# jcasal-homer/HomerHEVC

Hardware: AMD Instinct MI355X
Metric: encoded frames/sec, 1080p & 2160p YUV420 fixed-QP IPPP, 1/2/4/8 MI355X (higher is better)
Workload: dtype int16; 1 GPU; cfg2-1080p-encode; sequences_per_gpu=256, width=1920, height=1080, wfpp_num_threads=17, qp=32, gop=IPPP intra_period=100

## Files before the change

homerhevc_amd/csrc/enc/enc_platform.h:

```cpp
#pragma once
#include <stdint.h>
#include <string.h>
#include <math.h>

#if defined(__HIPCC__)
#include <hip/hip_runtime.h>
#define HENC_HD __device__
#if defined(HENC_PRIM_NOINLINE)
#define HENC_PRIM __device__ __attribute__((noinline))
#else
#define HENC_PRIM __device__
#endif
#define HENC_INLINE __host__ __device__ __forceinline__
#define HENC_TU_TABLES_IN_LDS 0
#define HENC_FT(e) ((const FastTables *)nullptr)
#else
#define HENC_HD
#define HENC_PRIM
#define HENC_INLINE inline
#define HENC_TU_TABLES_IN_LDS 1
#define HENC_FT(e) ((e).ft)
#endif

#if defined(__HIPCC__) && !defined(HENC_WALK_OUTLINE)
#define HENC_WALK_FN __attribute__((always_inline))
#else
#define HENC_WALK_FN
#endif

namespace henc {

#if defined(__HIPCC__)
struct WaveGrp {
	int tid;
	static constexpr int n = 64;
	static constexpr bool bg = false;
#if defined(HENC_NO_RDFULL)
	static constexpr bool rdfull = false;
#else
	static constexpr bool rdfull = true;
#endif
	__device__ __forceinline__ void sync() const
	{
		__builtin_amdgcn_fence(__ATOMIC_RELEASE, "wavefront");
		__builtin_amdgcn_wave_barrier();
		__builtin_amdgcn_fence(__ATOMIC_ACQUIRE, "wavefront");
	}
	__device__ __forceinline__ uint32_t sum(uint32_t v) const
	{
		int x = (int)v;
		x += __builtin_amdgcn_update_dpp(0, x, 0x111, 0xf, 0xf, true);
		x += __builtin_amdgcn_update_dpp(0, x, 0x112, 0xf, 0xf, true);
		x += __builtin_amdgcn_update_dpp(0, x, 0x114, 0xf, 0xf, true);
		x += __builtin_amdgcn_update_dpp(0, x, 0x118, 0xf, 0xf, true);
		return (uint32_t)(__builtin_amdgcn_readlane(x, 15) + __builtin_amdgcn_readlane(x, 31) + __builtin_amdgcn_readlane(x, 47) + __builtin_amdgcn_readlane(x, 63));
	}
	__device__ __forceinline__ int64_t sum64(int64_t v) const
	{
#pragma unroll
		for (int m = 32; m >= 1; m >>= 1) v += __shfl_xor(v, m, 64);
		return v;
	}
	__device__ __forceinline__ uint32_t any(bool p) const { return __ballot(p) != 0; }
	__device__ __forceinline__ uint64_t ballot(bool p) const { return __ballot(p); }
	__device__ __forceinline__ uint64_t min64(uint64_t v) const
	{
#pragma unroll
		for (int m = 32; m >= 1; m >>= 1) {
			const uint64_t o = __shfl_xor(v, m, 64);
			v = o < v ? o : v;
		}
		return v;
	}
};
struct WaveGrpLat : WaveGrp {
	static constexpr bool bg = true;
};
struct WaveGrpLean : WaveGrp {
	static constexpr bool rdfull = false;
};

template <class P>
struct PairGrpOf {
	int tid, half;
	static constexpr int n = 32;
	static constexpr bool bg = false;
	static constexpr bool rdfull = P::rdfull;
	__device__ __forceinline__ void sync() const
	{
		__builtin_amdgcn_fence(__ATOMIC_RELEASE, "wavefront");
		__builtin_amdgcn_wave_barrier();
		__builtin_amdgcn_fence(__ATOMIC_ACQUIRE, "wavefront");
	}
	__device__ __forceinline__ uint32_t sum(uint32_t v) const
	{
		int x = (int)v;
		x += __builtin_amdgcn_update_dpp(0, x, 0x111, 0xf, 0xf, true);
		x += __builtin_amdgcn_update_dpp(0, x, 0x112, 0xf, 0xf, true);
		x += __builtin_amdgcn_update_dpp(0, x, 0x114, 0xf, 0xf, true);
		x += __builtin_amdgcn_update_dpp(0, x, 0x118, 0xf, 0xf, true);
		const int lo = __builtin_amdgcn_readlane(x, 15) + __builtin_amdgcn_readlane(x, 31), hi = __builtin_amdgcn_readlane(x, 47) + __builtin_amdgcn_readlane(x, 63);
		return (uint32_t)(half ? hi : lo);
	}
	__device__ __forceinline__ uint64_t ballot(bool p) const { const uint64_t m = __ballot(p); return half ? m >> 32 : m & 0xffffffffull; }
	__device__ __forceinline__ uint32_t any(bool p) const { return ballot(p) != 0; }
};
using PairGrp = PairGrpOf<WaveGrp>;

#endif

template <class T>
HENC_INLINE T uni(T x)
{
#if defined(__HIP_DEVICE_COMPILE__)
	static_assert(sizeof(T) <= 4, "one scalar register");
	return (T)__builtin_amdgcn_readfirstlane((int)x);
#else
	return x;
#endif
}
template <class T>
HENC_INLINE T *uni_ptr(T *p)
{
#if defined(__HIP_DEVICE_COMPILE__)
	const uintptr_t v = (uintptr_t)p;
	const uint32_t lo = (uint32_t)__builtin_amdgcn_readfirstlane((int)(uint32_t)v), hi = (uint32_t)__builtin_amdgcn_readfirstlane((int)(uint32_t)(v >> 32));
	return (T *)(((uintptr_t)hi << 32) | (uintptr_t)lo);
#else
	return p;
#endif
}
template <class T>
HENC_INLINE T *in_fast_memory(T *p)
{
#if defined(__HIP_DEVICE_COMPILE__) && defined(HENC_CHECK_ADDRSPACE)
	if (p && !__builtin_amdgcn_is_shared((const void *)p)) __builtin_trap();
	return p;
#elif defined(__HIP_DEVICE_COMPILE__)
	__builtin_assume(__builtin_amdgcn_is_shared((const void *)p));
	return p;
#else
	return p;
#endif
}
#if defined(__HIP_DEVICE_COMPILE__) && defined(HENC_CHECK_ADDRSPACE)
#define HENC_ENC_IN_LDS(e) do { if (!__builtin_amdgcn_is_shared((const void *)&(e))) __builtin_trap(); } while (0)
#elif defined(__HIP_DEVICE_COMPILE__)
#define HENC_ENC_IN_LDS(e) __builtin_assume(__builtin_amdgcn_is_shared((const void *)&(e)))
#else
#define HENC_ENC_IN_LDS(e) do { } while (0)
#endif
#if defined(__HIP_DEVICE_COMPILE__) && defined(HENC_TU_OPERANDS_IN_LDS) && defined(HENC_CHECK_ADDRSPACE)
#define HENC_OP_IN_LDS(p) do { if (!__builtin_amdgcn_is_shared((const void *)(p))) __builtin_trap(); } while (0)
#elif defined(__HIP_DEVICE_COMPILE__) && defined(HENC_TU_OPERANDS_IN_LDS)
#define HENC_OP_IN_LDS(p) __builtin_assume(__builtin_amdgcn_is_shared((const void *)(p)))
#else
#define HENC_OP_IN_LDS(p) do { } while (0)
#endif
#if defined(__HIP_DEVICE_COMPILE__)
#define HENC_GLOBAL_PTR(T) __attribute__((address_space(1))) T *
#else
#define HENC_GLOBAL_PTR(T) T *
#endif
template <class T>
struct FastPtr {
	T *p;
	HENC_INLINE T *get() const { return in_fast_memory(p); }
	HENC_INLINE T *operator->() const { return get(); }
	HENC_INLINE T &operator*() const { return *get(); }
	HENC_INLINE T &operator[](int i) const { return get()[i]; }
	HENC_INLINE operator T *() const { return get(); }
	HENC_INLINE explicit operator bool() const { return p != nullptr; }
	HENC_INLINE FastPtr &operator=(T *q) { p = q; return *this; }
};

#if defined(__HIP_DEVICE_COMPILE__)
extern __shared__ __align__(16) unsigned char henc_lds_base[];
template <class T, int OFFSET>
struct LdsAt {
	HENC_INLINE T *get() const { return (T *)(henc_lds_base + OFFSET); }
	HENC_INLINE T *operator->() const { return get(); }
	HENC_INLINE T &operator*() const { return *get(); }
	HENC_INLINE T &operator[](int i) const { return get()[i]; }
	HENC_INLINE operator T *() const { return get(); }
	HENC_INLINE explicit operator bool() const { return true; }
	HENC_INLINE LdsAt &operator=(T *) { return *this; }
	HENC_INLINE LdsAt &operator=(decltype(nullptr)) { return *this; }
};
#endif

struct CpuGrp {
	static constexpr int tid = 0;
	static constexpr int n = 1;
	static constexpr bool bg = false;
	static constexpr bool rdfull = true;
	void sync() const {}
	uint32_t sum(uint32_t v) const { return v; }
	int64_t sum64(int64_t v) const { return v; }
	uint32_t any(bool p) const { return p; }
	uint64_t ballot(bool p) const { return p ? 1 : 0; }
	uint64_t min64(uint64_t v) const { return v; }
};

template <class T> HENC_INLINE T hmin(T a, T b) { return a < b ? a : b; }
template <class T> HENC_INLINE T hmax(T a, T b) { return a > b ? a : b; }
template <class T> HENC_INLINE T hclip(T v, T lo, T hi) { return v < lo ? lo : (v > hi ? hi : v); }
HENC_INLINE int habs(int v) { return v < 0 ? -v : v; }
HENC_INLINE double hsqrt(double v) { return ::sqrt(v); }
HENC_INLINE int16_t sat16(int v) { return (int16_t)hclip(v, -32768, 32767); }

}
```

homerhevc_amd/csrc/enc/enc_sched.h:

```cpp
#pragma once
#include "enc_ctu.h"

#if !defined(__HIPCC__) && defined(HENC_SCHED_CAUSES)
extern "C" int henc_sched_causes[8];
#define SCHED_CAUSE(k) (henc_sched_causes[k]++)
#else
#define SCHED_CAUSE(k) ((void)0)
#endif

namespace henc {

constexpr int MODE_STATE_BYTES = 2 * NDEPTH * NPART;

HENC_INLINE void sched_chain_step(uint8_t st[2][NDEPTH], const uint8_t *out_tokens, int k)
{
	uint8_t nx[2][NDEPTH];
	for (int comp = 0; comp < 2; comp++)
		for (int d = 0; d < NDEPTH; d++) {
			const uint8_t v = out_tokens[(comp * NDEPTH + d) * NPART + k];
			nx[comp][d] = (v & MODE_TOKEN) ? st[comp][v & 7] : v;
		}
	for (int comp = 0; comp < 2; comp++)
		for (int d = 0; d < NDEPTH; d++) st[comp][d] = nx[comp][d];
}

HENC_INLINE int sched_replay_search(const SearchLog &lg, const uint8_t *true_in, double sqrt_lambda, int *mode_g, int *bits_g, int *mode_t, int *bits_t)
{
	int td[2], pg[3], pt[3];
	double cg = 0, ct = 0;
	for (int k = 0; k < 2; k++) td[k] = (lg.src[k] & 0x8000) ? true_in[((lg.src[k] >> 8) & 7) * NPART + (lg.src[k] & 255)] : lg.used[k];
	mpm_from_dirs(lg.used[0], lg.used[1], pg);
	mpm_from_dirs(td[0], td[1], pt);
	auto table = [&](int mode) -> int64_t {
		for (int k = 0; k < lg.n; k++)
			if (lg.mode[k] == mode) return (int64_t)lg.sad[k];
		return -1;
	};
	*bits_g = intra_search_walk(pg, 1, sqrt_lambda, table, mode_g, &cg);
	*bits_t = intra_search_walk(pt, 1, sqrt_lambda, table, mode_t, &ct);
	return *bits_t >= 0;
}

template <class G>
HENC_HD int sched_guesses_hold(const G g, const CtuInfo &c, const FrameCtx &f, const uint8_t *true_in, const uint8_t *used_in, uint32_t intra_before,
			       uint32_t parts_before, uint32_t used_intra, uint32_t used_parts, int uses_ratio)
{
	int bad = 0;
	if (c.walk_intra != ctu_takes_intra_walk(f, c.ctu_number)) return 0;
	if (c.walk_intra) uses_ratio = 0;
	if (c.n_spec_reads > MAX_SEARCH_LOGS || c.n_ratio_cmp > MAX_RATIO_CMP) {
		for (int i = g.tid; i < NDEPTH * NPART; i += g.n) bad |= true_in[i] != used_in[i];
		if (uses_ratio) bad |= intra_ratio(intra_before, parts_before) != intra_ratio(used_intra, used_parts);
		return !g.any(bad);
	}
	for (int i = g.tid; i < c.n_spec_reads; i += g.n) {
		const SearchLog &lg = c.slog[i];
		if (lg.has_cmp) continue;
		int mg, bg, mt, bt;
		bad |= !sched_replay_search(lg, true_in, f.sqrt_lambda, &mg, &bg, &mt, &bt) || mg != mt || bg != bt;
	}
	if (uses_ratio) {
		const double ratio = intra_ratio(intra_before, parts_before), used_ratio = intra_ratio(used_intra, used_parts);
		const double correction = calc_mv_correction((uint32_t)f.qp, f.avg_dist);
		for (int i = g.tid; i < c.n_ratio_cmp; i += g.n) {
			const double *lg = c.ratio_cmp + 4 * i;
			double intra_dist = lg[0];
			int same_bits = 1;
			if (c.ratio_slog[i] >= 0) {
				const SearchLog &sl = c.slog[c.ratio_slog[i]];
				int mg, bg, mt, bt;
				if (!sched_replay_search(sl, true_in, f.sqrt_lambda, &mg, &bg, &mt, &bt) || mg != mt) { bad = 1; SCHED_CAUSE(bt < 0 ? 0 : 1); continue; }
				same_bits = bg == bt;
				intra_dist = (double)((uint32_t)lg[0] - intra_luma_cost(sl.tu_cost, bg, correction) + intra_luma_cost(sl.tu_cost, bt, correction));
			}
			const double ic = intra_cost_with_ratio(intra_dist, ratio, lg[1], lg[2]), ic_used = intra_cost_with_ratio(lg[0], used_ratio, lg[1], lg[2]);
			const int take = ic < lg[3];
			if (take != (c.ratio_out[i] != 0)) SCHED_CAUSE(c.ratio_slog[i] >= 0 && !same_bits ? 2 : 3);
			else if (take && (!same_bits || (uint32_t)ic != (uint32_t)ic_used)) SCHED_CAUSE(4);
			bad |= take != (c.ratio_out[i] != 0) || (take && (!same_bits || (uint32_t)ic != (uint32_t)ic_used));
		}
	}
	return !g.any(bad);
}

template <class G>
HENC_HD uint64_t sched_output_hash(const G g, const Seq &S, const FrameCtx &f, const CtuInfo &c)
{
	uint32_t h1 = 0, h2 = 0;
	const uint32_t *p = (const uint32_t *)(const CtuPublic *)&c;
	const int words = (int)(offsetof(CtuPublic, sao_recon) / 4);
	for (int i = g.tid; i < words; i += g.n) {
		h1 += p[i] * (2654435761u + 2u * (uint32_t)i);
		h2 += (p[i] ^ 0x9e3779b9u) * (40503u + 2u * (uint32_t)i + 1u);
	}
	for (int comp = 0; comp < 3; comp++) {
		const int sz = comp ? 32 : 64, px = comp ? c.x >> 1 : c.x, py = comp ? c.y >> 1 : c.y;
		const int pw = comp ? S.width >> 1 : S.width, ph = comp ? S.height >> 1 : S.height, rs = comp ? S.stride_c : S.stride_y;
		const int ww = (px + sz) < pw ? sz : pw - px, hh = (py + sz) < ph ? sz : ph - py;
		const int16_t *r = f.rec[comp] + py * rs + px;
		for (int i = g.tid; i < ww * hh; i += g.n) {
			const uint32_t v = (uint16_t)r[(i / ww) * rs + (i % ww)];
			h1 += v * (2246822519u + 2u * (uint32_t)(i + comp * 4096));
			h2 += (v + 0x632be5abu) * (3266489917u + 2u * (uint32_t)(i + comp * 4096));
		}
	}
	h1 = g.sum(h1);
	h2 = g.sum(h2);
	return ((uint64_t)h1 << 32) | h2;
}

HENC_INLINE void sched_known_intra(const uint32_t *prefix, int W, int row, int col, uint32_t *intra, uint32_t *parts)
{
	uint32_t ti = prefix[(size_t)row * (W + 1) + col], tp = (uint32_t)col;
	for (int k = 1; k <= row; k++) {
		const int have = col + 2 * k < W ? col + 2 * k : W;
		ti += prefix[(size_t)(row - k) * (W + 1) + have];
		tp += (uint32_t)have;
	}
	*intra = ti;
	*parts = tp * NPART;
}

}
```

homerhevc_amd/csrc/k_encode.hip:

```cpp
#define HENC_TU_OPERANDS_IN_LDS 1
#include <stddef.h>
#include <stdlib.h>
#include <algorithm>
#include <chrono>
#include <mutex>
#include <condition_variable>
#include <new>
#include <string>
#include <thread>
#include <vector>

#include <type_traits>
#include "common.h"
#include "enc/enc_sched.h"
#include "enc/enc_host.h"
#include "enc/enc_post.h"
#include "picture_io.h"

using namespace henc;

int hmr_subpel_plane_on(hipStream_t stream, int comp, const int16_t *pic, int stride, int rows, uint8_t *out);
int hmr_subpel_planes_on(hipStream_t stream, const int16_t *pic_y, const int16_t *pic_u, const int16_t *pic_v, int stride_y, int rows_y, int stride_c, int rows_c, uint8_t *out_y,
			 uint8_t *out_u, uint8_t *out_v);

struct EncDev {
	const Seq *seq;
	const FrameCtx *frame;
	const DevTables *tables;
	const Geo *geo;
	CtuInfo *ctus, *ctus_start;
	WorkSlow *work_slow;
	int16_t *coeff;
	int *progress;
	uint32_t *prefix;
	unsigned long long *prof;
	uint8_t *guess, *truth, *outtok;
	uint8_t *chain_start, *chain_end;
	int *valid, *dirty;
	unsigned long long *hash;
	uint32_t *intra_before, *used_intra, *used_parts;
	uint8_t *rowstate;
	int *thread_seen;
	int *row0_checked;
	int *counters;
	int threads;
	int dep, dep_full;
	int after, raster;
	FrameCtx *next_frame;
	double *fin;
	RcFrame *rc_dyn;
	const int *rd_src;
	const uint8_t *rd_init, *rd_ring;
	PostPic post;
};

__device__ __forceinline__ void wave_copy_words(void *dst, const void *src, int bytes, int tid)
{
	uint32_t *d = (uint32_t *)dst;
	const uint32_t *s = (const uint32_t *)src;
	for (int i = tid; i < bytes / 4; i += 64) d[i] = s[i];
}
__device__ __forceinline__ void wave_copy_quads(void *dst, const void *src, int bytes, int tid)
{
	uint4 *d = (uint4 *)dst;
	const uint4 *s = (const uint4 *)src;
#pragma unroll 4
	for (int i = tid; i < bytes / 16; i += 64) d[i] = s[i];
}
constexpr int PRED_STATE_BYTES = (64 * 64 + 2 * 32 * 32) * (int)sizeof(pred_t), ROW_STATE_BYTES = MODE_STATE_BYTES + PRED_STATE_BYTES;
static_assert(offsetof(Work, pred_c) == offsetof(Work, pred_y) + 64 * 64 * sizeof(pred_t) && sizeof(((Work *)nullptr)->pred_c) == 2 * 32 * 32 * sizeof(pred_t), "the prediction windows are one block of Work");
static_assert(MODE_STATE_BYTES % 16 == 0 && offsetof(Work, pred_y) % 16 == 0, "wave_copy_quads alignment");

constexpr size_t LDS_WORK = (sizeof(Work) + 15) & ~(size_t)15, LDS_NODES = (sizeof(Node) * NODE_SLOTS + 15) & ~(size_t)15,
		 LDS_GEO = NHELP * HSCRATCH_ELEMS * 2;
namespace henc { __constant__ Geo henc_geo_table[NNODES]; }
constexpr bool LDS_KEEPS_CTU_RECORD = false, LDS_KEEPS_TU_TABLES = false;
static_assert(LDS_KEEPS_TU_TABLES == (HENC_TU_TABLES_IN_LDS != 0), "enc_platform.h: HENC_FT");
constexpr size_t LDS_SEQ = (sizeof(Seq) + sizeof(FrameCtx) + 31) & ~(size_t)15, LDS_CTU = LDS_KEEPS_CTU_RECORD ? (sizeof(CtuPublic) + 15) & ~(size_t)15 : 0,
		 LDS_FT = LDS_KEEPS_TU_TABLES ? (sizeof(FastTables) + 15) & ~(size_t)15 : 0;
#if defined(HENC_PROFILE)
constexpr size_t LDS_BOX = LDS_BOX_BYTES + (1 + NHELP) * LDS_ENC_BYTES, LDS_HSCRATCH = 0, LDS_RD = (sizeof(WorkRd) + 15) & ~(size_t)15;
constexpr size_t LDS_BYTES = HENC_LDS_PROF_OFFSET + 2 * PP_COUNT * 8;
constexpr size_t LDS_FT_OFFSET = LDS_WORK + LDS_NODES + LDS_GEO + LDS_SEQ + LDS_CTU + LDS_BOX + LDS_HSCRATCH;
static_assert(LDS_WORK + LDS_NODES + LDS_GEO + LDS_SEQ + LDS_CTU + LDS_BOX + LDS_HSCRATCH + LDS_FT + LDS_RD <= HENC_LDS_PROF_OFFSET, "profile table overlaps the worker state");
#else
constexpr size_t LDS_BOX = LDS_BOX_BYTES + (1 + NHELP) * LDS_ENC_BYTES, LDS_HSCRATCH = 0, LDS_RD = (sizeof(WorkRd) + 15) & ~(size_t)15;
constexpr size_t LDS_BYTES = LDS_WORK + LDS_NODES + LDS_GEO + LDS_SEQ + LDS_CTU + LDS_BOX + LDS_HSCRATCH + LDS_FT + LDS_RD;
constexpr size_t LDS_FT_OFFSET = LDS_WORK + LDS_NODES + LDS_GEO + LDS_SEQ + LDS_CTU + LDS_BOX + LDS_HSCRATCH;
#endif
static_assert(sizeof(SubpelScratch) <= LDS_WORK + LDS_NODES + LDS_GEO, "task S works where the post stage does");
static_assert(sizeof(PostScratch) <= LDS_WORK + LDS_NODES + LDS_GEO, "the post stage works in what is idle between two CTUs: the worker's Work area, the CTU's partition nodes, the helpers' scratch");
#if !defined(HENC_PROFILE)
static_assert(LDS_OFF_RD == (int)(LDS_BYTES - LDS_RD), "the RD_FULL arrays are the tail of a worker's LDS");
#endif
static_assert(LDS_OFF_ENC == (int)(LDS_WORK + LDS_NODES + LDS_GEO + LDS_SEQ + LDS_CTU + LDS_BOX_BYTES) || LDS_FT != 0 || LDS_CTU != 0, "the RD_FULL arrays are the tail of a worker's LDS: launches without RD_FULL pictures leave them out");
static_assert(LDS_OFF_NODES == (int)LDS_WORK && LDS_OFF_SEQ == (int)(LDS_WORK + LDS_NODES + LDS_GEO) && LDS_OFF_BOX == (int)(LDS_WORK + LDS_NODES + LDS_GEO + LDS_SEQ + LDS_CTU),
	      "enc_common.h: the fixed places of Enc's LDS members");
#if !defined(HENC_WAVES_PER_EU)
#define HENC_WAVES_PER_EU 2
#endif
constexpr int ENC_THREADS = 64 * (1 + NHELP);
static_assert(LDS_BYTES <= 160 * 1024, "a workgroup has 160 KiB of LDS on gfx950");
constexpr int workers_per_cu(size_t lds_bytes)
{
	const int by_lds = (int)((160 * 1024) / ((lds_bytes + 1279) / 1280 * 1280)), by_waves = 4 * HENC_WAVES_PER_EU / (1 + NHELP);
	return by_lds < by_waves ? by_lds : by_waves;
}
constexpr int WORKERS_PER_CU = workers_per_cu(LDS_BYTES - LDS_RD);
#if !defined(HENC_PROFILE) && HENC_WAVES_PER_EU == 2 && HENC_NHELP == 1
static_assert(WORKERS_PER_CU == 4, "a worker's LDS (without the RD_FULL arrays) has to stay within a quarter of the CU's: 32 granules of 1280 bytes");
#endif
#if defined(HENC_PRINT_LDS)
static_assert(LDS_BYTES - LDS_RD == 0 && LDS_WORK == 0 && LDS_NODES == 0 && LDS_BOX == 0 && sizeof(PostScratch) == 0 && WORKERS_PER_CU == 0, "sizes");
#endif

template <class G>
__device__ __forceinline__ bool helper_serve(HelperBox *box, int h, int16_t *scratch, const G g, int seq)
{
	extern __shared__ __align__(16) uint8_t lds[];
	Enc &e = *(Enc *)(lds + LDS_OFF_ENC + (1 + h) * LDS_ENC_BYTES);
	HENC_ENC_IN_LDS(e);
	const Enc &worker = *(const Enc *)(lds + LDS_OFF_ENC);
	{
		const int job = box->job[h];
		if (job == HJOB_QUIT) return false;
		if (job == HJOB_NEW_CTU) {
			wave_copy_words(&e, &worker, (int)sizeof(Enc), g.tid);
			g.sync();
			e.box = nullptr;
			e.on_helper = 1 + h;
			e.scratch_a = scratch;
			e.scratch_b = scratch + 1024;
			e.adi_c = scratch + 2048;
			e.prof = nullptr;
		}
		const int *a = box->a[h];
		uint32_t r0 = 0, r1 = 0, r2 = 0, r3 = 0, r4 = 0, r5 = 0;
		switch (job) {
		case HJOB_INTER_TU: {
			int sum = 0;
			uint32_t raw = 0;
			if (NHELP == 1 && a[1] == COMP_UV && e.geo[a[0]].size_chroma <= 8) {
				const PairGrpOf<G> pg{g.tid & 31, g.tid >> 5};
				const uint32_t d = encode_inter_tu(pg, e, a[0], COMP_U + pg.half, a[2], a[3], &sum, &raw, pg.half * 512);
				r0 = (uint32_t)__builtin_amdgcn_readlane((int)d, 0); r1 = (uint32_t)__builtin_amdgcn_readlane(sum, 0); r2 = (uint32_t)__builtin_amdgcn_readlane((int)raw, 0);
				r3 = (uint32_t)__builtin_amdgcn_readlane((int)d, 32); r4 = (uint32_t)__builtin_amdgcn_readlane(sum, 32); r5 = (uint32_t)__builtin_amdgcn_readlane((int)raw, 32);
				break;
			}
			r0 = encode_inter_tu(g, e, a[0], a[1] == COMP_UV ? COMP_U : a[1], a[2], a[3], &sum, &raw);
			r1 = (uint32_t)sum;
			r2 = raw;
			if (a[1] == COMP_UV) {
				r3 = encode_inter_tu(g, e, a[0], COMP_V, a[2], a[3], &sum, &raw);
				r4 = (uint32_t)sum;
				r5 = raw;
			}
			break;
		}
		case HJOB_SYNC_CU:
			if (a[1] == COMP_UV) sync_cu_chroma_both(g, e, a[0], a[2], a[3], a[4], a[5]);
			else sync_cu_comp(g, e, a[0], a[2], a[3], a[4], a[5], a[1]);
			break;
		case HJOB_SSD: {
			const Geo &q = e.geo[a[0]];
			if (a[1] == COMP_UV) {
				const int n = q.size_chroma, l = ilog2i(n);
				uint32_t acc[2] = {0, 0};
				for (int i = g.tid * 4; i < n * n; i += 64 * 4) {
					const int o = q.yc * 32 + q.xc + (i >> l) * 32 + (i & (n - 1));
#pragma unroll
					for (int c = 0; c < 2; c++) {
						const S4 va = ld4(e.w->curr_c[c] + o), vb = ld4(e.w->pred_c[c] + o);
#pragma unroll
						for (int k = 0; k < 4; k++) { const int32_t dd = (int16_t)(va.v[k] - vb.v[k]); acc[c] += (uint32_t)(dd * dd); }
					}
				}
				r0 = g.sum(acc[0]);
				r1 = g.sum(acc[1]);
			} else {
				const int c = a[1] - 1;
				r0 = blk_ssd(g, e.w->curr_c[c] + q.yc * 32 + q.xc, 32, e.w->pred_c[c] + q.yc * 32 + q.xc, 32, q.size_chroma);
			}
			break;
		}
		case HJOB_CHROMA_SEARCH: {
			const int cand[5] = {a[2] & 255, (a[2] >> 8) & 255, (a[2] >> 16) & 255, (a[2] >> 24) & 255, a[3]};
			uint32_t sads[5];
			chroma_search_comp(g, e, a[0], a[1], cand, sads);
			g.sync();
			if (g.tid == 0)
				for (int k = 0; k < 5; k++) box->r[h][k] = sads[k];
			break;
		}
		case HJOB_CHROMA_TU: {
			int cs = 0;
			r0 = (uint32_t)chroma_tu_comp(g, e, a[0], a[1], a[2], a[3], a[4], a[5] & 255, a[5] >> 8, &cs);
			r1 = (uint32_t)cs;
			break;
		}
#if defined(HENC_QUAD)
// ... 89 lines not shown
	HelperBox *box = (HelperBox *)(lds + LDS_WORK + LDS_NODES + LDS_GEO + LDS_SEQ + LDS_CTU);
	const int wave = (int)(threadIdx.x >> 6);
	for (int i = (int)threadIdx.x; i < (int)(lds_bytes / 4); i += ENC_THREADS) ((uint32_t *)lds)[i] = 0;
	__syncthreads();
	if (wave > 0) {
		helper_loop<LAT, G>(box, wave - 1, (int16_t *)(lds + LDS_WORK + LDS_NODES) + (wave - 1) * HSCRATCH_ELEMS);
		return false;
	}
	return true;
}
__device__ __forceinline__ void release_helpers(int *hseq)
{
	extern __shared__ __align__(16) uint8_t lds[];
	HelperBox *box = (HelperBox *)(lds + LDS_WORK + LDS_NODES + LDS_GEO + LDS_SEQ + LDS_CTU);
	if ((threadIdx.x & 63) == 0)
		for (int h = 0; h < NHELP; h++) {
			box->job[h] = HJOB_QUIT;
			__hip_atomic_store(&box->cmd[h], ++hseq[h], __ATOMIC_RELEASE, __HIP_MEMORY_SCOPE_WORKGROUP);
		}
}
__device__ __forceinline__ void encode_row(const EncDev &d, int pass, int row, int *hseq)
{
	extern __shared__ __align__(16) uint8_t lds[];
	const Seq &S = *d.seq;
	const int W = S.wctu, H = S.hctu;
	WaveGrp g{(int)(threadIdx.x & 63)};
	Work *lw = (Work *)lds;
	HelperBox *box = (HelperBox *)(lds + LDS_WORK + LDS_NODES + LDS_GEO + LDS_SEQ + LDS_CTU);
	for (int i = g.tid; i < (int)(LDS_WORK / 4); i += 64) ((uint32_t *)lds)[i] = 0;
	g.sync();
	Seq *lseq = (Seq *)(lds + LDS_WORK + LDS_NODES + LDS_GEO);
	FrameCtx *lframe = (FrameCtx *)((uint8_t *)lseq + ((sizeof(Seq) + 15) & ~(size_t)15));
	for (int i = g.tid; i < (int)(sizeof(Seq) / 4); i += 64) ((uint32_t *)lseq)[i] = ((const uint32_t *)d.seq)[i];
	for (int i = g.tid; i < (int)(sizeof(FrameCtx) / 4); i += 64) ((uint32_t *)lframe)[i] = ((const uint32_t *)d.frame)[i];
	if (g.tid == 0) lw->slow = (HENC_GLOBAL_PTR(WorkSlow))(d.work_slow + row);
	g.sync();
	if (g.tid == 0) lframe->scene_cut_ctu = d.counters[2];
	FastTables *lft = LDS_KEEPS_TU_TABLES ? (FastTables *)(lds + LDS_FT_OFFSET) : nullptr;
	if (lft) fast_tables_fill(g, *lft, d.tables, lframe->qp % 6, chroma_qp_table(lframe->qp + S.chroma_qp_offset) % 6);
#if defined(HENC_PROFILE)
	if (g.tid < 2 * PP_COUNT) ((unsigned long long *)(lds + HENC_LDS_PROF_OFFSET))[g.tid] = 0;
#endif
	g.sync();
	Enc &e = *(Enc *)(lds + LDS_OFF_ENC);
	HENC_ENC_IN_LDS(e);
	e.seq = lseq;
	e.f = lframe;
	e.T = d.tables;
	e.ft = lft;
	e.geo.p = nullptr;
	e.ctus = d.ctus;
	e.ctu = nullptr;
	e.w = lw;
	e.nodes = nullptr;
	e.nodes_fast = (Node *)(lds + LDS_WORK);
	e.node_quad = -1;
	e.on_helper = 0;
	e.ctu_g = nullptr;
	e.ctu_fast = LDS_KEEPS_CTU_RECORD ? (CtuPublic *)(lds + LDS_WORK + LDS_NODES + LDS_GEO + LDS_SEQ) : nullptr;
	e.box = box;
	for (int h = 0; h < NHELP; h++) e.hseq[h] = hseq[h];
	e.bgseq = 0;
	e.bg_node = -1;
	e.prof = d.prof ? d.prof + (size_t)row * PF_COUNT : nullptr;
	e.timeline = nullptr;
	uint32_t *my_prefix = d.prefix + (size_t)row * (W + 1);
	if (pass <= 0 && g.tid == 0) my_prefix[0] = 0;
	int encodes = 0;
	if (g.tid == 0) lw->thread_seen_intra = 1;
	g.sync();
	for (int c = 0; c < W; c++) {
		if (row > 0) {
			HENC_PROF_T0();
			const int need = c + 2 < W ? c + 2 : W;
			while (__hip_atomic_load(&d.progress[row - 1], __ATOMIC_RELAXED, __HIP_MEMORY_SCOPE_AGENT) < need) __builtin_amdgcn_s_sleep(32);
			__builtin_amdgcn_fence(__ATOMIC_ACQUIRE, "agent");
			HENC_PROF_ADD(e, PF_WAIT);
		}
		const int n = row * W + c;
		const int redo = pass == 0 || !__hip_atomic_load(&d.valid[n], __ATOMIC_RELAXED, __HIP_MEMORY_SCOPE_AGENT) ||
				 __hip_atomic_load(&d.dirty[n], __ATOMIC_RELAXED, __HIP_MEMORY_SCOPE_AGENT);
		if (redo) {
			HENC_PROF_T0();
			uint8_t *gs = d.guess + (size_t)n * MODE_STATE_BYTES;
			uint32_t ui, up;
			if (pass > 0) {
				wave_copy_words(&d.ctus[n], &d.ctus_start[n], (int)offsetof(CtuInfo, n_spec_reads), g.tid);
				wave_copy_words(d.ctus[n].nodes, d.ctus_start[n].nodes, (int)sizeof(d.ctus[n].nodes), g.tid);
				wave_copy_words(gs, d.truth + (size_t)n * MODE_STATE_BYTES, MODE_STATE_BYTES, g.tid);
				ui = d.intra_before[n];
				up = (uint32_t)n * NPART;
			} else {
				if (n == 0) wave_copy_words(gs, d.chain_start, MODE_STATE_BYTES, g.tid);
				sched_known_intra(d.prefix, W, row, c, &ui, &up);
			}
			g.sync();
			if (g.tid == 0) e.w->mode_in = (const uint8_t (*)[NDEPTH][NPART])gs;
			if (g.tid == 0) { d.used_intra[n] = ui; d.used_parts[n] = up; }
			const unsigned long long old_hash = d.hash[n];
			e.total_intra_partitions = ui;
			e.total_partitions = up;
			e.coeff = d.coeff + (size_t)n * 6144;
			e.ctu_qp = lframe->qp;
			g.sync();
			encode_ctu(g, e, n);
			encodes++;
			wave_copy_words(d.outtok + (size_t)n * MODE_STATE_BYTES, e.w->intra_mode_buffs, MODE_STATE_BYTES, g.tid);
			const unsigned long long h = sched_output_hash(g, S, *lframe, d.ctus[n]);
			if (g.tid == 0) { d.hash[n] = h; d.dirty[n] = 0; }
			if (pass == 0) {
				const int snap = row + 1 < H && c == (W > 1 ? 1 : 0);
				if (c + 1 < W || snap) {
					const uint8_t *tok = &e.w->intra_mode_buffs[0][0][0];
					uint8_t *nx = gs + MODE_STATE_BYTES, *rs = d.guess + (size_t)(row + 1) * W * MODE_STATE_BYTES;
					for (int i = g.tid; i < MODE_STATE_BYTES; i += 64) {
						const uint8_t v = tok[i];
						const uint8_t r = (v & MODE_TOKEN) ? gs[(i / (NDEPTH * NPART)) * NDEPTH * NPART + (v & 7) * NPART + i % NPART] : v;
						if (c + 1 < W) nx[i] = r;
						if (snap) rs[i] = r;
					}
				}
				if (g.tid == 0) my_prefix[c + 1] = my_prefix[c] + d.ctus[n].intra_parts;
			} else if (h != old_hash && g.tid == 0) {
				if (c + 1 < W) d.dirty[n + 1] = 1;
				if (row + 1 < H) {
					if (c > 0) d.dirty[n + W - 1] = 1;
					d.dirty[n + W] = 1;
					if (c + 1 < W) d.dirty[n + W + 1] = 1;
				}
			}
			HENC_PROF_ADD(e, PF_TOTAL);
		}
		g.sync();
		if (g.tid == 0) __hip_atomic_store(&d.progress[row], c + 1, __ATOMIC_RELEASE, __HIP_MEMORY_SCOPE_AGENT);
	}
	for (int h = 0; h < NHELP; h++) hseq[h] = e.hseq[h];
	if (g.tid == 0 && encodes) atomicAdd(&d.counters[1], encodes);
#if defined(HENC_PROFILE)
	if (g.tid == 0 && e.prof) {
		const unsigned long long *pp = (const unsigned long long *)(lds + HENC_LDS_PROF_OFFSET);
		for (int k = 0; k < 2 * PP_COUNT; k++) e.prof[PF_PRIM0 + k] += pp[k];
	}
#endif
}

struct PoolSeq {
	int *cur_step;
	int *ticket;
	int *done;
};
constexpr int POOL_MAX_STEPS = HENC_MAX_STEPS;
constexpr int POOL_STRIDE = 1 + 2 * POOL_MAX_STEPS;
constexpr int BATCH_MAX = 512;

__device__ __forceinline__ void pool_step_rows(int t, int W, int H, int *r_lo, int *r_hi)
{
	const int lo = t - W + 1;
	*r_lo = lo <= 0 ? 0 : (lo + 1) >> 1;
	*r_hi = (t >> 1) < H - 1 ? (t >> 1) : H - 1;
}

template <class G>
__device__ void pool_encode_ctu(const EncDev &d, Enc &__restrict__ e, const G g, Seq *lseq, FrameCtx *lframe, FastTables *lft, int t, int row, int *cached_rem, const int *abort_flag)
{
	HENC_ENC_IN_LDS(e);
	const Seq &S = *lseq;
	const int W = S.wctu, H = S.hctu;
	const int raster = d.raster;
	const int T = d.threads, me = row % T, c = raster ? t - row * W : t - 2 * row, n = row * W + c;
	uint32_t ti = 0, tc = 0;
	for (int r2 = g.tid; r2 < H; r2 += 64) {
		const int have = raster ? (r2 < row ? W : (r2 == row ? c : 0)) : (t - 2 * r2 < 0 ? 0 : (t - 2 * r2 < W ? t - 2 * r2 : W));
		ti += d.prefix[(size_t)r2 * (W + 1) + have];
		tc += (uint32_t)have;
	}
	ti = g.sum(ti);
	tc = g.sum(tc);
	wave_copy_words(&e.w->intra_mode_buffs[0][0][0], d.rowstate + (size_t)me * ROW_STATE_BYTES, MODE_STATE_BYTES, g.tid);
	wave_copy_quads(e.w->pred_y, d.rowstate + (size_t)me * ROW_STATE_BYTES + MODE_STATE_BYTES, PRED_STATE_BYTES, g.tid);
	if (g.tid == 0) e.w->thread_seen_intra = d.thread_seen[me];
	if (rd_full(g, S)) {
		const int seen = d.thread_seen[me];
		for (int i = g.tid; i < NPART; i += 64) e.wrd->rd_pred_mode[i] = seen ? PM_INTRA : PM_INTER;
	}
	const int rem_y = lframe->qp % 6, rem_c = chroma_qp_table(lframe->qp + S.chroma_qp_offset) % 6;
	if (lft && (cached_rem[0] != rem_y || cached_rem[1] != rem_c)) {
		fast_tables_fill(g, *lft, d.tables, rem_y, rem_c);
		cached_rem[0] = rem_y; cached_rem[1] = rem_c;
	}
	g.sync();
	const int hrow = raster ? row : t / (2 * T) * T;
	uint32_t rc_bits = 0;
	int rc_ctus = 0;
	if (rd_full(g, S)) {
		const int code = d.rd_src[n], kind = code >> 28, slot = (code >> 24) & 15;
		const size_t off = (size_t)(code & 0x00ffffff) * RD_CTX_BYTES;
		e.rd_ctx = kind == 3 ? d.rd_ring + ((size_t)slot * S.nctu) * RD_CTX_BYTES + off : d.rd_init + (size_t)(kind ? 1 + slot : 0) * RD_CTX_BYTES;
	}
	if (lframe->rc.on) rc_consumed(g, d.post, W, H, t, &rc_bits, &rc_ctus);
	if (row == hrow) {
		if (g.tid == 0) {
			if (d.counters[2] < 0 && lframe->slice_type == SLICE_P && scene_cut_fires(S, *lframe, ti, tc * NPART)) {
				if (lframe->rc.on) {
					RcFrame nrc = lframe->rc;
					rc_change_pic_mode(nrc, S.reinit_gop, S.intra_period, S.nctu, nrc.sqrt_clipped_intra_period, rc_bits, rc_ctus);
					*d.rc_dyn = nrc;
				}
				d.counters[2] = n;
			}
			__hip_atomic_store(d.row0_checked, t + 1, __ATOMIC_RELEASE, __HIP_MEMORY_SCOPE_AGENT);
		}
	} else if (hrow < H && t - 2 * hrow < W) {
		while (__hip_atomic_load(d.row0_checked, __ATOMIC_RELAXED, __HIP_MEMORY_SCOPE_AGENT) < t + 1 && !__hip_atomic_load(abort_flag, __ATOMIC_RELAXED, __HIP_MEMORY_SCOPE_AGENT)) __builtin_amdgcn_s_sleep(8);
		__builtin_amdgcn_fence(__ATOMIC_ACQUIRE, "agent");
	}
	g.sync();
	if (g.tid == 0) lframe->scene_cut_ctu = __hip_atomic_load(&d.counters[2], __ATOMIC_RELAXED, __HIP_MEMORY_SCOPE_AGENT);
	g.sync();
	e.ctu_qp = lframe->qp;
	if (lframe->rc.on) {
		const int cut = lframe->scene_cut_ctu;
		const int is_sc = cut >= 0 && (raster ? n >= cut : t >= cut % W + 2 * (cut / W));
		if (is_sc) {
			wave_copy_words(&lframe->rc, d.rc_dyn, (int)sizeof(RcFrame), g.tid);
			g.sync();
		}
		e.ctu_qp = rc_calc_cu_qp(lframe->rc, (double)rc_bits, rc_ctus, lframe->slice_type, is_sc, S.reinit_gop, S.intra_period, lframe->avg_dist, lframe->num_encoded_frames);
	}
	if (g.tid == 0) e.w->mode_in = (const uint8_t (*)[NDEPTH][NPART])(d.rowstate + (size_t)me * ROW_STATE_BYTES);
	e.total_intra_partitions = ti;
	e.total_partitions = tc * NPART;
	e.coeff = d.coeff + (size_t)n * 6144;
	g.sync();
#if defined(HENC_PROFILE)
	e.prof = d.prof ? d.prof + (size_t)row * PF_COUNT : nullptr;
	{
		HENC_PROF_T0();
		encode_ctu(g, e, n);
		HENC_PROF_ADD(e, PF_TOTAL);
	}
	if (g.tid == 0 && e.prof) {
		unsigned long long *pp = (unsigned long long *)(henc_lds + HENC_LDS_PROF_OFFSET);
		for (int k = 0; k < 2 * PP_COUNT; k++) { e.prof[PF_PRIM0 + k] += pp[k]; pp[k] = 0; }
	}
#else
	encode_ctu(g, e, n);
#endif
	resolve_mode_tokens(g, *e.w, d.ctus[n]);
	wave_copy_words(d.outtok + (size_t)n * MODE_STATE_BYTES, e.w->intra_mode_buffs, MODE_STATE_BYTES, g.tid);
	wave_copy_words(d.rowstate + (size_t)me * ROW_STATE_BYTES, &e.w->intra_mode_buffs[0][0][0], MODE_STATE_BYTES, g.tid);
	wave_copy_quads(d.rowstate + (size_t)me * ROW_STATE_BYTES + MODE_STATE_BYTES, e.w->pred_y, PRED_STATE_BYTES, g.tid);
	if (g.tid == 0) {
		d.thread_seen[me] = e.w->thread_seen_intra;
		uint32_t *my_prefix = d.prefix + (size_t)row * (W + 1);
		my_prefix[c + 1] = my_prefix[c] + d.ctus[n].intra_parts;
		atomicAdd(&d.counters[1], 1);
	}
	g.sync();
	__builtin_amdgcn_fence(__ATOMIC_RELEASE, "agent");
	if (g.tid == 0) post_st_fenced(&d.post.rows[row].dec, c + 1);
}

__device__ __attribute__((noinline)) int pool_post_drain_run(const EncDev &d, const WaveGrp g, const Seq *lseq, const FrameCtx *lframe, Work *lw, WorkSlow *my_slow, int *finished);
__device__ __forceinline__ int pool_post_drain(const EncDev &d, const WaveGrp g, const Seq *lseq, const FrameCtx *lframe, Work *lw, WorkSlow *my_slow, int *finished)
{
	if (post_finished(*lseq, d.post)) return 0;
	PostCtx x;
	x.seq = lseq; x.f = lframe; x.T = d.tables; x.geo.p = nullptr; x.ctus = d.ctus; x.coeff = d.coeff; x.pic = &d.post;
	int r, c, k;
	if (!post_scan(g, x, r, c, k)) return 0;
	return pool_post_drain_run(d, g, lseq, lframe, lw, my_slow, finished);
}
__device__ __attribute__((noinline)) int pool_post_drain_run(const EncDev &d, const WaveGrp g, const Seq *lseq, const FrameCtx *lframe, Work *lw, WorkSlow *my_slow, int *finished)
{
	PostCtx x;
	x.seq = lseq; x.f = lframe; x.T = d.tables; x.geo.p = nullptr; x.ctus = d.ctus; x.coeff = d.coeff; x.pic = &d.post;
	PostScratch &sc = *(PostScratch *)in_fast_memory((uint8_t *)lw);
	const int ran = post_drain(g, x, sc);
	if (ran) {
		if (g.tid == 0) lw->slow = (HENC_GLOBAL_PTR(WorkSlow))my_slow;
		g.sync();
		if (post_finished(*lseq, d.post)) {
			int won = 0;
			if (g.tid == 0) won = atomicCAS(&d.post.errors[1], 0, 2) == 0;
			if (__builtin_amdgcn_readfirstlane(won)) {
				__builtin_amdgcn_fence(__ATOMIC_ACQUIRE, "agent");
				const int W = lseq->wctu, H = lseq->hctu, T = d.threads < 1 ? 1 : d.threads;
				int64_t part = 0;
				for (int t = g.tid; t < T && t < H; t += 64) {
					uint32_t acc = 0;
					for (int r = t; r < H; r += T)
						for (int c = 0; c < W; c++) acc += d.ctus[r * W + c].distortion;
					part += acc;
				}
				const double total = (double)g.sum64(part);
				if (g.tid == 0) {
					d.fin[0] = total;
					if (d.next_frame) {
						double a = total;
						a /= lseq->nctu * NPART;
						a = a < .1 ? .1 : a;
						if (lframe->slice_type == SLICE_I) a *= 1.5;
						else if (__hip_atomic_load(&d.counters[2], __ATOMIC_RELAXED, __HIP_MEMORY_SCOPE_AGENT) >= 0) a *= 1.375;
						d.next_frame->avg_dist = a;
					}
					__builtin_amdgcn_fence(__ATOMIC_RELEASE, "agent");
					post_st_release(&d.post.errors[1], 1);
					atomicAdd(finished, 1);
				}
			}
		}
	}
	return ran;
}

template <class G>
__device__ __forceinline__ void encode_pool_body(const EncDev *devs, int nseq, int *state, int *finished, WorkSlow *slow, unsigned long long watchdog_ticks, unsigned lds_bytes)
{
	unsigned long long t_start = wall_clock64();
	constexpr bool LAT = G::bg;
	if (!rows_enter<LAT, typename std::conditional<LAT, WaveGrp, G>::type>(lds_bytes)) return;
	extern __shared__ __align__(16) uint8_t lds[];
	G g{(int)(threadIdx.x & 63)};
	Work *lw = (Work *)lds;
	HelperBox *box = (HelperBox *)(lds + LDS_WORK + LDS_NODES + LDS_GEO + LDS_SEQ + LDS_CTU);
	Seq *lseq = (Seq *)(lds + LDS_WORK + LDS_NODES + LDS_GEO);
	FrameCtx *lframe = (FrameCtx *)((uint8_t *)lseq + ((sizeof(Seq) + 15) & ~(size_t)15));
	FastTables *lft = LDS_KEEPS_TU_TABLES ? (FastTables *)(lds + LDS_FT_OFFSET) : nullptr;
	if (g.tid == 0) lw->slow = (HENC_GLOBAL_PTR(WorkSlow))(slow + blockIdx.x);
#if defined(HENC_PROFILE)
	if (g.tid < 2 * PP_COUNT) ((unsigned long long *)(lds + HENC_LDS_PROF_OFFSET))[g.tid] = 0;
#endif
	g.sync();
	Enc &e = *(Enc *)(lds + LDS_OFF_ENC);
	HENC_ENC_IN_LDS(e);
	e.seq = lseq;
	e.f = lframe;
	e.ft = lft;
	e.geo.p = nullptr;
	e.ctu = nullptr;
	e.w = lw;
	e.nodes = nullptr;
	e.nodes_fast = (Node *)(lds + LDS_WORK);
	e.node_quad = -1;
	e.on_helper = 0;
	e.ctu_g = nullptr;
	e.ctu_fast = LDS_KEEPS_CTU_RECORD ? (CtuPublic *)(lds + LDS_WORK + LDS_NODES + LDS_GEO + LDS_SEQ) : nullptr;
	e.box = box;
	for (int h = 0; h < NHELP; h++) e.hseq[h] = 0;
	e.bgseq = 0;
	e.bg_node = -1;
	e.prof = nullptr;
	e.timeline = nullptr;
	int cached_rem[2] = {-1, -1}, cached_q = -1, idle_rounds = 0;
	int start = (int)(blockIdx.x % (unsigned)nseq);
	for (;;) {
		int q = -1, t = 0, k = 0;
		bool all_finished = true;
		for (int base = 0; base < nseq && q < 0; base += 64) {
			const int i = base + g.tid, cand = i < nseq ? (start + i) % nseq : -1;
			int ct = -1;
			bool open = false;
			if (cand >= 0) {
				const int *st = state + (size_t)cand * POOL_STRIDE;
				const EncDev &dd = devs[cand];
				const int W = dd.seq->wctu, H = dd.seq->hctu, steps = dd.raster ? W * H : W + 2 * (H - 1);
				ct = __hip_atomic_load(&st[0], __ATOMIC_RELAXED, __HIP_MEMORY_SCOPE_AGENT);
				if (ct < steps) {
					all_finished = false;
					if (dd.raster) open = __hip_atomic_load(&st[1], __ATOMIC_RELAXED, __HIP_MEMORY_SCOPE_AGENT) == ct;
					else {
						int r_lo, r_hi;
						pool_step_rows(ct, W, H, &r_lo, &r_hi);
						open = __hip_atomic_load(&st[1 + ct], __ATOMIC_RELAXED, __HIP_MEMORY_SCOPE_AGENT) < r_hi - r_lo + 1;
					}
				}
			}
			if (g.any(!all_finished)) all_finished = false;
			uint64_t m = g.ballot(open);
			while (m) {
				const int lane0 = __builtin_ctzll(m);
				const int q0 = __builtin_amdgcn_readlane(cand, lane0), t0 = __builtin_amdgcn_readlane(ct, lane0);
				const EncDev &d0 = devs[q0];
				bool ready = !d0.post.rc_need || rc_ready(g, d0.post, d0.seq->hctu, t0);
				if (ready && d0.dep >= 0) {
					const EncDev &dd = devs[d0.dep];
					const int H0 = dd.seq->hctu, W0 = dd.seq->wctu;
					for (int base2 = 0; base2 < H0 && ready; base2 += 64) {
						const int r2 = base2 + g.tid;
						bool miss = false;
						if (r2 < H0) {
							int need = t0 - 2 * r2 + 8;
							need = need < 0 ? 0 : (need > W0 ? W0 : need);
							if (d0.dep_full) need = W0;
							miss = post_ld(&dd.post.rows[r2].s_done) < need;
						}
						if (g.any(miss)) ready = false;
					}
				}
				if (ready && d0.after >= 0) ready = post_ld(&devs[d0.after].post.errors[1]) == 1;
				if (ready) break;
				m &= m - 1;
			}
			if (m) {
				const int lane = __builtin_ctzll(m);
				const int qq = __builtin_amdgcn_readlane(cand, lane), tt = __builtin_amdgcn_readlane(ct, lane);
				int kk = 0;
				const EncDev &dd = devs[qq];
				if (dd.raster) {
					if (g.tid == 0) kk = atomicCAS(&state[(size_t)qq * POOL_STRIDE + 1], tt, tt + 1) == tt ? 0 : 1;
					kk = __builtin_amdgcn_readfirstlane(kk);
					if (kk == 0) { q = qq; t = tt; k = 0; }
					else base -= 64;
					continue;
				}
				if (g.tid == 0) kk = atomicAdd(&state[(size_t)qq * POOL_STRIDE + 1 + tt], 1);
				kk = __builtin_amdgcn_readfirstlane(kk);
				int r_lo, r_hi;
				pool_step_rows(tt, dd.seq->wctu, dd.seq->hctu, &r_lo, &r_hi);
				if (kk < r_hi - r_lo + 1) { q = qq; t = tt; k = kk; }
				else base -= 64;
			}
		}
		if (q < 0) {
			if (__hip_atomic_load(finished, __ATOMIC_RELAXED, __HIP_MEMORY_SCOPE_AGENT) >= nseq) break;
			if (__hip_atomic_load(finished + 1, __ATOMIC_RELAXED, __HIP_MEMORY_SCOPE_AGENT)) break;
			if (wall_clock64() - t_start > watchdog_ticks) { if (g.tid == 0) __hip_atomic_store(finished + 1, 1, __ATOMIC_RELAXED, __HIP_MEMORY_SCOPE_AGENT); break; }
			int ran = 0;
			for (int i = 0; i < nseq; i++) {
				const int cand = (start + i) % nseq;
				const EncDev &dd = devs[cand];
				ran += pool_post_drain(dd, g, dd.seq, dd.frame, lw, slow + blockIdx.x, finished);
				if (ran) { start = cand; break; }
			}
			if (!ran) {
				idle_rounds = idle_rounds < 16 ? idle_rounds + 1 : 16;
				for (int i = 0; i < idle_rounds; i++) __builtin_amdgcn_s_sleep(127);
			} else {
				idle_rounds = 0;
				t_start = wall_clock64();
			}
			continue;
		}
		__builtin_amdgcn_fence(__ATOMIC_ACQUIRE, "agent");
		const EncDev &d = devs[q];
		if (q != cached_q) {
			for (int i = g.tid; i < (int)(sizeof(Seq) / 4); i += 64) ((uint32_t *)lseq)[i] = ((const uint32_t *)d.seq)[i];
			for (int i = g.tid; i < (int)(sizeof(FrameCtx) / 4); i += 64) ((uint32_t *)lframe)[i] = ((const uint32_t *)d.frame)[i];
			cached_q = q;
			g.sync();
		}
		e.T = d.tables;
		e.ctus = d.ctus;
		const int W = lseq->wctu, H = lseq->hctu;
		int r_lo, r_hi;
		pool_step_rows(t, W, H, &r_lo, &r_hi);
		const int hrow = t / (2 * d.threads) * d.threads;
		const bool hvalid = hrow >= r_lo && hrow <= r_hi;
		int row;
		if (d.raster) row = t / W;
		else if (hvalid) row = k == 0 ? hrow : (r_lo + k - 1 < hrow ? r_lo + k - 1 : r_lo + k);
		else row = r_lo + k;
		pool_encode_ctu(d, e, g, lseq, lframe, lft, t, row, cached_rem, finished + 1);
		if (g.tid == 0) {
			int *st = state + (size_t)q * POOL_STRIDE;
			const int dn = d.raster ? 1 : atomicAdd(&st[1 + POOL_MAX_STEPS + t], 1) + 1;
			if (dn == (d.raster ? 1 : r_hi - r_lo + 1)) {
				__builtin_amdgcn_fence(__ATOMIC_ACQUIRE, "agent");
				__hip_atomic_store(&st[0], t + 1, __ATOMIC_RELEASE, __HIP_MEMORY_SCOPE_AGENT);
			}
		}
		pool_post_drain(d, g, lseq, lframe, lw, slow + blockIdx.x, finished);
		idle_rounds = 0;
		t_start = wall_clock64();
		start = (q + 1) % nseq;
	}
	int hseq[NHELP];
	for (int h = 0; h < NHELP; h++) hseq[h] = e.hseq[h];
	release_helpers(hseq);
}
__global__ __launch_bounds__(ENC_THREADS) __attribute__((amdgpu_waves_per_eu(HENC_WAVES_PER_EU))) void k_encode_pool(const EncDev *devs, int nseq, int *state, int *finished, WorkSlow *slow, unsigned long long watchdog_ticks, unsigned lds_bytes)
{
	encode_pool_body<WaveGrpLean>(devs, nseq, state, finished, slow, watchdog_ticks, lds_bytes);
}
__global__ __launch_bounds__(ENC_THREADS) __attribute__((amdgpu_waves_per_eu(HENC_WAVES_PER_EU))) void k_encode_full(const EncDev *devs, int nseq, int *state, int *finished, WorkSlow *slow, unsigned long long watchdog_ticks, unsigned lds_bytes)
{
	encode_pool_body<WaveGrp>(devs, nseq, state, finished, slow, watchdog_ticks, lds_bytes);
}
__global__ __launch_bounds__(ENC_THREADS) __attribute__((amdgpu_waves_per_eu(HENC_WAVES_PER_EU))) void k_encode_pool_lat(const EncDev *devs, int nseq, int *state, int *finished, WorkSlow *slow, unsigned long long watchdog_ticks, unsigned lds_bytes)
{
	encode_pool_body<WaveGrpLat>(devs, nseq, state, finished, slow, watchdog_ticks, lds_bytes);
}

__global__ __launch_bounds__(320) void k_sched_scan(EncDev d)
{
	const int nctu = d.seq->nctu, k = threadIdx.x;
	if (k < NPART) {
		uint8_t st[2][NDEPTH];
		for (int comp = 0; comp < 2; comp++)
			for (int dd = 0; dd < NDEPTH; dd++) st[comp][dd] = d.chain_start[(comp * NDEPTH + dd) * NPART + k];
		for (int n = 0; n < nctu; n++) {
			uint8_t *t = d.truth + (size_t)n * MODE_STATE_BYTES;
			for (int comp = 0; comp < 2; comp++)
				for (int dd = 0; dd < NDEPTH; dd++) t[(comp * NDEPTH + dd) * NPART + k] = st[comp][dd];
			sched_chain_step(st, d.outtok + (size_t)n * MODE_STATE_BYTES, k);
		}
		for (int comp = 0; comp < 2; comp++)
			for (int dd = 0; dd < NDEPTH; dd++) d.chain_end[(comp * NDEPTH + dd) * NPART + k] = st[comp][dd];
	} else if (k == NPART) {
		uint32_t ib = 0;
		int cut = -1;
		const FrameCtx &f = *d.frame;
		for (int n = 0; n < nctu; n++) {
			d.intra_before[n] = ib;
			if (cut < 0 && f.slice_type == SLICE_P && scene_cut_fires(*d.seq, f, ib, (uint32_t)n * NPART)) cut = n;
			ib += d.ctus[n].intra_parts;
		}
		d.counters[0] = 0;
		d.counters[2] = cut;
	}
}

__global__ __launch_bounds__(64) void k_sched_check(EncDev d)
{
	const int n = blockIdx.x;
	WaveGrp g{(int)threadIdx.x};
	FrameCtx f = *d.frame;
	f.scene_cut_ctu = d.counters[2];
	const int uses_ratio = f.slice_type != SLICE_I;
	const int ok = sched_guesses_hold(g, d.ctus[n], f, d.truth + (size_t)n * MODE_STATE_BYTES, d.guess + (size_t)n * MODE_STATE_BYTES, d.intra_before[n], (uint32_t)n * NPART,
					  d.used_intra[n], d.used_parts[n], uses_ratio);
	if (g.tid == 0) {
		d.valid[n] = ok;
		if (!ok) atomicAdd(&d.counters[0], 1);
	}
}

__global__ __launch_bounds__(64) void k_sched_finish(EncDev d)
{
	const int n = blockIdx.x, tid = threadIdx.x;
	CtuInfo &c = d.ctus[n];
	const uint8_t *t = d.truth + (size_t)n * MODE_STATE_BYTES;
	for (int i = tid; i < 2 * NPART; i += 64) {
		uint8_t &v = (&c.intra_mode[0][0])[i];
		if (v & MODE_TOKEN) v = t[((i / NPART) * NDEPTH + (v & 7)) * NPART + i % NPART];
	}
}

struct SrcSlot {
	int16_t *p[3];
};

__global__ __launch_bounds__(ENC_THREADS) __attribute__((amdgpu_waves_per_eu(2))) void k_encode_ctus(EncDev d, int pass)
{
	if (!rows_enter((unsigned)LDS_BYTES)) return;
	int hseq[NHELP_MAX] = {0, 0, 0};
	encode_row(d, pass, (int)blockIdx.x, hseq);
	release_helpers(hseq);
}
__global__ __launch_bounds__(64) __attribute__((amdgpu_waves_per_eu(2))) void k_post_frame(EncDev d)
{
	extern __shared__ __align__(16) uint8_t lds[];
	WaveGrp g{(int)threadIdx.x};
	for (int r = (int)blockIdx.x * 64 + g.tid; r < d.seq->hctu; r += (int)gridDim.x * 64) d.post.rows[r].dec = d.seq->wctu;
	__builtin_amdgcn_fence(__ATOMIC_RELEASE, "agent");
	PostCtx x;
	x.seq = d.seq; x.f = d.frame; x.T = d.tables; x.geo.p = nullptr; x.ctus = d.ctus; x.coeff = d.coeff; x.pic = &d.post;
	PostScratch &sc = *(PostScratch *)in_fast_memory((uint8_t *)lds);
	const unsigned long long t_start = wall_clock64();
	while (!post_finished(*d.seq, d.post)) {
		if (!post_drain(g, x, sc)) {
			if (wall_clock64() - t_start > 3000000000ull) { if (g.tid == 0) d.post.errors[2] = 1; break; }
			__builtin_amdgcn_s_sleep(16);
		}
	}
}

#include "k_encode_object.inc"
#include "k_encode_batch.inc"
#include "k_encode_picture_io.inc"
#include "k_encode_walktest.inc"
```

homerhevc_amd/csrc/k_encode_batch.inc:

```
namespace {
__global__ __launch_bounds__(256) void k_pack_streams(const EncDev *devs, uint8_t *out, const size_t *offs)
{
	__shared__ uint32_t start[POST_MAX_ROWS + 1];
	const EncDev &d = devs[blockIdx.x];
	const int rows = d.seq->wpp ? d.seq->hctu : 1;
	if (threadIdx.x == 0) {
		uint32_t o = 0;
		for (int r = 0; r < rows; r++) { start[r] = o; o += (uint32_t)d.post.ent[r].bytecnt; }
		start[rows] = o;
	}
	__syncthreads();
	uint8_t *dst = out + offs[blockIdx.x];
	for (int r = 0; r < rows; r++) {
		const uint8_t *src = d.post.bs + (size_t)r * d.post.row_cap;
		const uint32_t n = start[r + 1] - start[r];
		for (uint32_t i = threadIdx.x; i < n; i += blockDim.x) dst[start[r] + i] = src[i];
	}
}

__global__ void k_batch_stage(const EncDev *h_devs, const FrameCtx *h_frames, EncDev *d_devs, FrameCtx *d_frames)
{
	const int i = blockIdx.x, t = threadIdx.x;
	for (int k = t; k < (int)(sizeof(EncDev) / 4); k += blockDim.x) ((uint32_t *)(d_devs + i))[k] = ((const uint32_t *)(h_devs + i))[k];
	for (int k = t; k < (int)(sizeof(FrameCtx) / 4); k += blockDim.x) ((uint32_t *)(d_frames + i))[k] = ((const uint32_t *)(h_frames + i))[k];
	const EncDev d = h_devs[i];
	const int H = d.seq->hctu, W = d.seq->wctu;
	if (t < 3) d.counters[t] = t == 2 ? -1 : 0;
	if (t == 3) *d.row0_checked = 0;
	if (t >= 4 && t < 8) d.post.errors[t - 4] = 0;
	for (int k = t; k < H * (int)(sizeof(PostRow) / 4); k += blockDim.x) ((int *)d.post.rows)[k] = 0;
	for (int k = t; k < H; k += blockDim.x) d.progress[k] = 0;
	for (int k = t; k < H * (W + 1); k += blockDim.x) d.prefix[k] = 0;
}

struct BatchTimes {
	std::chrono::steady_clock::time_point t[8];
	double ms(int a, int b) const { return std::chrono::duration<double, std::milli>(t[b] - t[a]).count(); }
};

template <class F>
void parallel_for(int n, int threads, F fn)
{
	const int T = n < threads ? n : threads;
	std::vector<std::thread> th;
	for (int t = 0; t < T; t++)
		th.emplace_back([=]() {
			for (int i = t; i < n; i += T) fn(i);
		});
	for (auto &x : th) x.join();
}
constexpr int QUEUE_THREADS = 16;
constexpr int CODING_THREADS = 32;

int batch_check(hmr_gpu_enc **encs, int n, const int *slots, uint8_t **streams, const long *caps, long *stream_bytes)
{
	if (!encs || n <= 0 || n > BATCH_MAX || !streams || !caps || !stream_bytes) return HMR_GPU_ERR_ARG;
	for (int i = 0; i < n; i++) {
		hmr_gpu_enc *e = encs[i];
		if (!e || !e->lockstep || e->ctx->device != encs[0]->ctx->device || (slots && (slots[i] < 0 || slots[i] >= (int)e->src.size())) || !streams[i]) {
			hmr_set_error("hmr_gpu_enc_encode_batch: encoder %d: needs the row-per-thread schedule (wfpp_num_threads > 1), the batch's device and a loaded picture slot", i);
			return HMR_GPU_ERR_ARG;
		}
		for (int j = 0; j < i; j++)
			if (encs[j] == e) return HMR_GPU_ERR_ARG;
	}
	return HMR_GPU_OK;
}

int batch_launch(hmr_gpu_enc **encs, int n, const int *slots, const int *image_types, int *pitch_out)
{
	hmr_gpu_enc *lead = encs[0];
	hipStream_t bst = lead->ctx->stream;
	int rc, rows_total = 0, max_ctus = 0;
	bool needs_rd = false;
	if (!lead->d_frames) {
		HIP_TRY(hipMalloc((void **)&lead->d_frames, BATCH_MAX * sizeof(FrameCtx)));
		HIP_TRY(hipHostMalloc((void **)&lead->h_frames, BATCH_MAX * sizeof(FrameCtx), hipHostMallocDefault));
		HIP_TRY(hipHostMalloc((void **)&lead->h_devs, BATCH_MAX * sizeof(EncDev), hipHostMallocDefault));
	}
	for (int i = 0; i < n; i++) {
		hmr_gpu_enc *e = encs[i];
		if ((rc = set_frame(e, slots[i], image_types ? image_types[i] : 0, -1.0, false))) return rc;
		e->pic_stream = bst;
		HIP_TRY(hipEventRecord(e->ev_ready, e->ctx->stream));
		if (i) HIP_TRY(hipStreamWaitEvent(bst, e->ev_ready, 0));
		lead->h_frames[i] = e->f;
		lead->h_devs[i] = e->d;
		lead->h_devs[i].frame = lead->d_frames + i;
		rows_total += pool_inflight(e->seq, e->raster);
		needs_rd = needs_rd || e->seq.rd_mode == RDM_FULL;
		if (e->seq.nctu > max_ctus) max_ctus = e->seq.nctu;
	}
	if (!lead->plane_stream[0]) {
		for (int k = 0; k < 2; k++) {
			HIP_TRY(hipStreamCreateWithFlags(&lead->plane_stream[k], hipStreamNonBlocking));
			HIP_TRY(hipEventCreateWithFlags(&lead->ev_plane[k], hipEventDisableTiming));
		}
		HIP_TRY(hipEventCreateWithFlags(&lead->ev_plane[2], hipEventDisableTiming));
	}
	HIP_TRY(hipEventRecord(lead->ev_plane[2], bst));
	for (int k = 0; k < 2; k++) HIP_TRY(hipStreamWaitEvent(lead->plane_stream[k], lead->ev_plane[2], 0));
	for (int i = 0; i < n; i++) {
		hmr_gpu_enc *e = encs[i];
		const Seq &s = e->seq;
		if (e->f.slice_type == SLICE_I) continue;
		if ((rc = hmr_subpel_plane_on(bst, 0, e->d_pic[e->cur ^ 1][0], s.stride_y, s.height + 2 * s.margin_y, e->planes.y))) return rc;
		for (int k = 0; k < 2; k++)
			if ((rc = hmr_subpel_plane_on(lead->plane_stream[k], 1 + k, e->d_pic[e->cur ^ 1][1 + k], s.stride_c, s.height / 2 + 2 * s.margin_c, e->planes.c[k]))) return rc;
	}
	for (int k = 0; k < 2; k++) {
		HIP_TRY(hipEventRecord(lead->ev_plane[k], lead->plane_stream[k]));
		HIP_TRY(hipStreamWaitEvent(bst, lead->ev_plane[k], 0));
	}
	if (!lead->d_batch) {
		HIP_TRY(hipMalloc((void **)&lead->d_batch, BATCH_MAX * sizeof(EncDev)));
		HIP_TRY(hipDeviceGetAttribute(&lead->n_cus, hipDeviceAttributeMultiprocessorCount, lead->ctx->device));
	}
	const int pitch = GATHER_HEAD + max_ctus + POST_MAX_ROWS;
	if ((size_t)pitch * n > lead->gather_words) {
		if (lead->d_gather) (void)hipFree(lead->d_gather);
		if (lead->h_gather) (void)hipHostFree(lead->h_gather);
		lead->d_gather = lead->h_gather = nullptr;
		lead->gather_words = 0;
		HIP_TRY(hipMalloc((void **)&lead->d_gather, (size_t)pitch * BATCH_MAX * 4));
		HIP_TRY(hipHostMalloc((void **)&lead->h_gather, (size_t)pitch * BATCH_MAX * 4, hipHostMallocDefault));
		lead->gather_words = (size_t)pitch * BATCH_MAX;
	}
	hipLaunchKernelGGL(k_batch_stage, dim3(n), dim3(256), 0, bst, (const EncDev *)lead->h_devs, (const FrameCtx *)lead->h_frames, (EncDev *)lead->d_batch, lead->d_frames);
	HIP_TRY(hipGetLastError());
	HIP_TRY(hipEventRecord(lead->ev_batch0, bst));
	if ((rc = launch_pool(lead, lead->h_devs, n, rows_total, needs_rd, bst))) return rc;
	(void)hipEventRecord(lead->ev_batch1, bst);
	hipLaunchKernelGGL(k_gather_results, dim3(n), dim3(256), 0, bst, (const EncDev *)lead->d_batch, lead->d_gather, pitch, (const int *)(lead->d_pool_state + BATCH_MAX * POOL_STRIDE));
	HIP_TRY(hipGetLastError());
	HIP_TRY(hipMemcpyAsync(lead->h_gather, lead->d_gather, (size_t)pitch * n * 4, hipMemcpyDeviceToHost, bst));
	*pitch_out = pitch;
	return HMR_GPU_OK;
}

int batch_finish(hmr_gpu_enc **encs, int n, const int *slots, int pitch, BatchTimes &bt)
{
	(void)slots;
	hmr_gpu_enc *lead = encs[0];
	hipStream_t bst = lead->ctx->stream;
	const hipError_t waited = hipStreamSynchronize(bst);
	if (waited != hipSuccess) {
		hmr_set_error("k_encode_pool: %s", hipGetErrorString(waited));
		return HMR_GPU_ERR_HIP;
	}
	bt.t[2] = std::chrono::steady_clock::now();
	float ms = 0;
	HIP_TRY(hipEventElapsedTime(&ms, lead->ev_batch0, lead->ev_batch1));
	if (!lead->h_offs) HIP_TRY(hipHostMalloc((void **)&lead->h_offs, BATCH_MAX * sizeof(size_t), hipHostMallocDefault));
	lead->pend_off.resize(n);
	lead->pend_rows.assign(n, std::vector<uint32_t>());
	size_t total = 0;
	for (int i = 0; i < n; i++) {
		hmr_gpu_enc *e = encs[i];
		const uint32_t *g = lead->h_gather + (size_t)i * pitch;
		if (g[3] & 2) {
			hmr_set_error("k_encode_pool: the launch was abandoned by its watchdog (a worker found nothing to do for too long: HENC_WATCHDOG_S)");
			return HMR_GPU_ERR_HIP;
		}
		if (g[3] & 1) {
			hmr_set_error("hmr_gpu_enc_encode_batch: sequence %d: a CTU row's sub-stream outgrew its buffer (%d bytes)", i, e->row_cap);
			return HMR_GPU_ERR_HIP;
		}
		e->note_stale_predictions(g[3] >> 8);
		const int rows = e->seq.wpp ? e->seq.hctu : 1;
		lead->pend_off[i] = total;
		lead->h_offs[i] = total;
		lead->pend_rows[i].assign(g + pitch - POST_MAX_ROWS, g + pitch - POST_MAX_ROWS + rows);
		for (int r = 0; r < rows; r++) total += lead->pend_rows[i][r];
		total = (total + 255) & ~(size_t)255;
		e->last_ms = e->last_total_ms = ms;
		e->last_encodes = (int)g[1];
		e->f.scene_cut_ctu = (int)g[2];
		e->last_passes = 1;
		release_planes(e);
		e->f_pending = e->f;
		e->awaiting_delivery = true;
		FrameRcOut ro;
		ro.sum_qp = (int)g[4]; ro.consumed_bits = (double)g[5];
		memcpy(&ro.target_pict_size, &g[6], 8);
		end_frame(e->seq, e->st, e->f, frame_acc_dist(e->seq, e->cfg.wfpp_num_threads, [&](int c) { return g[GATHER_HEAD + c]; }), &ro);
	}
	if (total > lead->stage_bytes) {
		if (lead->d_stage) (void)hipFree(lead->d_stage);
		if (lead->h_stage) (void)hipHostFree(lead->h_stage);
		lead->d_stage = lead->h_stage = nullptr;
		lead->stage_bytes = 0;
		const size_t want = total * 2 + (1 << 20);
		HIP_TRY(hipMalloc((void **)&lead->d_stage, want));
		HIP_TRY(hipHostMalloc((void **)&lead->h_stage, want, hipHostMallocDefault));
		lead->stage_bytes = want;
	}
	if (!lead->copy_stream) HIP_TRY(hipStreamCreateWithFlags(&lead->copy_stream, hipStreamNonBlocking));
	hipLaunchKernelGGL(k_pack_streams, dim3(n), dim3(256), 0, bst, (const EncDev *)lead->d_batch, lead->d_stage, (const size_t *)lead->h_offs);
	HIP_TRY(hipGetLastError());
	HIP_TRY(hipEventRecord(lead->ev_decided, bst));
	HIP_TRY(hipStreamWaitEvent(lead->copy_stream, lead->ev_decided, 0));
	if (total) HIP_TRY(hipMemcpyAsync(lead->h_stage, lead->d_stage, total, hipMemcpyDeviceToHost, lead->copy_stream));
	bt.t[3] = std::chrono::steady_clock::now();
	lead->pend_encs.assign(encs, encs + n);
	lead->pend_total = total;
	lead->pending = true;
	return HMR_GPU_OK;
}

int batch_deliver(hmr_gpu_enc *lead, uint8_t **streams, const long *caps, long *stream_bytes, BatchTimes &bt)
{
	const int n = (int)lead->pend_encs.size();
	bt.t[4] = std::chrono::steady_clock::now();
	lead->pending = false;
	for (int i = 0; i < n; i++) lead->pend_encs[i]->awaiting_delivery = false;
	HIP_TRY(hipStreamSynchronize(lead->copy_stream));
	bt.t[5] = std::chrono::steady_clock::now();
	std::vector<int> rcs(n, 0);
	std::vector<std::string> errs(n);
	parallel_for(n, CODING_THREADS, [&](int i) {
		hmr_gpu_enc *e = lead->pend_encs[i];
		rcs[i] = frame_assemble(e, e->f_pending, lead->h_stage + lead->pend_off[i], lead->pend_rows[i].data(), streams[i], caps[i], &stream_bytes[i]);
		if (rcs[i] < 0) errs[i] = hmr_gpu_last_error();
	});
	bt.t[6] = std::chrono::steady_clock::now();
	for (int i = 0; i < n; i++)
		if (rcs[i] < 0) { hmr_set_error("hmr_gpu_enc_encode_batch: sequence %d: %s", i, errs[i].c_str()); return rcs[i]; }
	return HMR_GPU_OK;
}

void batch_report(const BatchTimes &bt, hmr_gpu_enc *lead, bool pipelined)
{
	if (!getenv("HENC_BATCH_TIMING")) return;
	static std::chrono::steady_clock::time_point last_end;
	const auto now = std::chrono::steady_clock::now();
	fprintf(stderr, "batch step%s: launch %.1f ms, wait for the pool %.1f, queue device parts %.1f, download wait %.1f (%.0f MB), entropy coding %.1f; the call %.1f, since the last call %.1f\n",
		pipelined ? " (pipelined)" : "", bt.ms(0, 1), pipelined ? bt.ms(6, 2) : bt.ms(1, 2), bt.ms(2, 3), bt.ms(4, 5), lead->pend_total / 1e6, bt.ms(5, 6),
		std::chrono::duration<double, std::milli>(now - bt.t[0]).count(), std::chrono::duration<double, std::milli>(bt.t[0] - last_end).count());
	last_end = now;
}
}

extern "C" int hmr_gpu_enc_encode_batch(hmr_gpu_enc **encs, int n, const int *slots, const int *image_types, uint8_t **streams, const long *caps, long *stream_bytes)
{
	int rc = batch_check(encs, n, slots, streams, caps, stream_bytes);
	if (rc) return rc;
	if (!slots) return HMR_GPU_ERR_ARG;
	for (int i = 0; i < n; i++)
		if (encs[i]->awaiting_delivery || encs[i]->pending) {
			hmr_set_error("hmr_gpu_enc_encode_batch: encoder %d has an access unit outstanding from a pipelined call: flush first", i);
			return HMR_GPU_ERR_ARG;
		}
	hmr_gpu_enc *lead = encs[0];
	HIP_TRY(hipSetDevice(lead->ctx->device));
	BatchTimes bt;
	int pitch = 0;
	bt.t[0] = std::chrono::steady_clock::now();
	if ((rc = batch_launch(encs, n, slots, image_types, &pitch))) return rc;
	bt.t[1] = std::chrono::steady_clock::now();
	if ((rc = batch_finish(encs, n, slots, pitch, bt))) return rc;
	if ((rc = batch_deliver(lead, streams, caps, stream_bytes, bt))) return rc;
	batch_report(bt, lead, false);
	return HMR_GPU_OK;
}

extern "C" int hmr_gpu_enc_encode_batch_pipelined(hmr_gpu_enc **encs, int n, const int *slots, const int *image_types, uint8_t **streams, const long *caps, long *stream_bytes)
{
	int rc = batch_check(encs, n, slots, streams, caps, stream_bytes);
	if (rc) return rc;
	hmr_gpu_enc *lead = encs[0];
	HIP_TRY(hipSetDevice(lead->ctx->device));
	if (lead->pending) {
		if ((int)lead->pend_encs.size() != n || memcmp(lead->pend_encs.data(), encs, n * sizeof(hmr_gpu_enc *))) {
			hmr_set_error("hmr_gpu_enc_encode_batch_pipelined: the encoder list changed while access units are outstanding: flush (slots = NULL) with the previous list first");
			return HMR_GPU_ERR_ARG;
		}
	} else {
		for (int i = 0; i < n; i++)
			if (encs[i]->awaiting_delivery) {
				hmr_set_error("hmr_gpu_enc_encode_batch_pipelined: encoder %d has an access unit outstanding in another batch", i);
				return HMR_GPU_ERR_ARG;
			}
	}
	BatchTimes bt;
	for (auto &t : bt.t) t = std::chrono::steady_clock::now();
	int pitch = 0;
	if (slots && (rc = batch_launch(encs, n, slots, image_types, &pitch))) return rc;
	bt.t[1] = std::chrono::steady_clock::now();
	if (lead->pending) {
		if ((rc = batch_deliver(lead, streams, caps, stream_bytes, bt))) return rc;
	} else {
		for (int i = 0; i < n; i++) stream_bytes[i] = 0;
		bt.t[6] = bt.t[1];
	}
	if (slots && (rc = batch_finish(encs, n, slots, pitch, bt))) return rc;
	if (slots) batch_report(bt, lead, true);
	return HMR_GPU_OK;
}

extern "C" int hmr_gpu_enc_encode_chain(hmr_gpu_enc **encs, int n, hmr_gpu_enc *prev, const int *slots, const int *image_types, uint8_t **streams, const long *caps, long *stream_bytes)
{
	if (!encs || n <= 0 || n > CHAIN_MAX_FRAMES || !slots || !streams || !caps || !stream_bytes) return HMR_GPU_ERR_ARG;
	for (int j = 0; j < n; j++) {
		hmr_gpu_enc *e = encs[j];
		if (!e || !e->lockstep || e->ctx->device != encs[0]->ctx->device || slots[j] < 0 || slots[j] >= (int)e->src.size() || !streams[j] || e->awaiting_delivery || e->engine_index < 0 ||
		    e->seq.width != encs[0]->seq.width || e->seq.height != encs[0]->seq.height) {
			hmr_set_error("hmr_gpu_enc_encode_chain: frame %d: needs an engine object (hmr_gpu_enc_create_engine) of the chain's sequence on the chain's device with a loaded picture slot", j);
			return HMR_GPU_ERR_ARG;
		}
		if (n > 1 && (e->seq.bitrate_mode != 0 || e->seq.rd_mode == RDM_FULL)) {
			hmr_set_error("hmr_gpu_enc_encode_chain: frame %d: rate control and RD_FULL need the frames one at a time (a chain of %d frames starts them from a predicted state)", j, n);
			return HMR_GPU_ERR_ARG;
		}
		if (j >= e->st.engines && e->d_ctus_eng[0] != encs[j - e->st.engines]->d_ctus_eng[0]) {
			hmr_set_error("hmr_gpu_enc_encode_chain: frame %d: the object has to be a twin (hmr_gpu_enc_create_engine_twin) of the one that encodes frame %d, the engine's frame before it", j, j - e->st.engines);
			return HMR_GPU_ERR_ARG;
		}
		for (int i = 0; i < j; i++)
			if (encs[i] == e) return HMR_GPU_ERR_ARG;
	}
	hmr_gpu_enc *lead = encs[0];
	hipStream_t bst = lead->ctx->stream;
	HIP_TRY(hipSetDevice(lead->ctx->device));
	int rc, rows_total = 0;
	bool needs_rd = false;
	if (!lead->d_frames) {
		HIP_TRY(hipMalloc((void **)&lead->d_frames, BATCH_MAX * sizeof(FrameCtx)));
		HIP_TRY(hipHostMalloc((void **)&lead->h_frames, BATCH_MAX * sizeof(FrameCtx), hipHostMallocDefault));
		HIP_TRY(hipHostMalloc((void **)&lead->h_devs, BATCH_MAX * sizeof(EncDev), hipHostMallocDefault));
	}
	if (!lead->d_batch) HIP_TRY(hipMalloc((void **)&lead->d_batch, BATCH_MAX * sizeof(EncDev)));
	HostState st = prev ? prev->st : lead->st;
	const HostState start_state = st;
	struct Undo { hmr_gpu_enc *e; int cur; HostState st; FrameCtx f; PlaneSet planes, planes2; EncDev d; bool has_picture; hipStream_t pic_stream; };
	std::vector<Undo> undo;
	auto refuse = [&](int code) {
		for (size_t k = undo.size(); k-- > 0;) {
			Undo &u = undo[k];
			u.e->cur = u.cur; u.e->st = u.st; u.e->f = u.f; u.e->chain_planes = u.planes; u.e->chain_planes2 = u.planes2; u.e->d = u.d;
			u.e->has_picture = u.has_picture; u.e->pic_stream = u.pic_stream;
		}
		return code;
	};
	for (int j = 0; j < n; j++) {
		hmr_gpu_enc *e = encs[j];
		const Seq &s = e->seq;
		if (st.num_encoded_frames % e->st.engines != e->engine_index) {
			hmr_set_error("hmr_gpu_enc_encode_chain: frame %d of the sequence belongs to engine %d, not %d", st.num_encoded_frames, st.num_encoded_frames % e->st.engines, e->engine_index);
			return refuse(HMR_GPU_ERR_ARG);
		}
		for (int k = 0; k < 2; k++) {
			PlaneSet &ps = k ? e->chain_planes2 : e->chain_planes;
			if (ps.y) continue;
			PlaneSet p;
			p.device = e->ctx->device; p.bytes_y = (size_t)16 * s.plane_elems_y; p.bytes_c = (size_t)64 * s.plane_elems_c;
			HIP_TRY(hipMalloc((void **)&p.y, p.bytes_y));
			HIP_TRY(hipMalloc((void **)&p.c[0], p.bytes_c));
			HIP_TRY(hipMalloc((void **)&p.c[1], p.bytes_c));
			ps = p;
		}
		undo.push_back(Undo{e, e->cur, e->st, e->f, e->chain_planes, e->chain_planes2, e->d, e->has_picture, e->pic_stream});
		e->st = st;
		const hmr_gpu_enc *r = j ? encs[j - 1] : prev;
		const int16_t *ref_planes[3] = {nullptr, nullptr, nullptr};
		PlaneSet ref_set;
		if (r) {
			for (int c = 0; c < 3; c++) ref_planes[c] = plane0(const_cast<hmr_gpu_enc *>(r), r->cur, c);
			ref_set = r->chain_planes;
		}
		std::swap(e->chain_planes, e->chain_planes2);
		if (j == 0 && e == prev) ref_set = e->chain_planes2;
		if ((rc = set_frame(e, slots[j], image_types ? image_types[j] : 0, -1.0, false, true))) return refuse(rc);
		e->pic_stream = bst;
		st = e->st;
		st.num_encoded_frames++;
		if (e->f.slice_type != SLICE_I) {
			if (!r || !ref_set.y) {
				hmr_set_error("hmr_gpu_enc_encode_chain: frame %d is a P frame and there is no object that holds the picture before it with its phase planes", j);
				return refuse(HMR_GPU_ERR_ARG);
			}
			for (int c = 0; c < 3; c++) e->f.ref[c] = ref_planes[c];
			e->f.sub_y = ref_set.y + (size_t)s.margin_y * 16 * s.stride_y + s.margin_y;
			e->f.sub_c[0] = ref_set.c[0] + (size_t)s.margin_c * 64 * s.stride_c + s.margin_c;
			e->f.sub_c[1] = ref_set.c[1] + (size_t)s.margin_c * 64 * s.stride_c + s.margin_c;
			e->d.dep = j ? j - 1 : -1;
			e->d.dep_full = getenv("HENC_CHAIN_SERIAL") ? 1 : 0;
		}
		if (j >= e->st.engines) {
			const hmr_gpu_enc *b = encs[j - e->st.engines];
			if (b->f.slice_type == SLICE_I && b->f.num_encoded_frames != 0 && s.intra_period != 1) {
				hmr_set_error("hmr_gpu_enc_encode_chain: frame %d is an I frame inside the sequence and the same engine's next frame is in the chain: end the chain before frame %d", j - e->st.engines, j);
				return refuse(HMR_GPU_ERR_ARG);
			}
			e->d.after = j - e->st.engines;
			e->f.avg_dist = 0.0;
			lead->h_devs[j - e->st.engines].next_frame = lead->d_frames + j;
		}
		e->d.post.planes[0] = e->chain_planes.y; e->d.post.planes[1] = e->chain_planes.c[0]; e->d.post.planes[2] = e->chain_planes.c[1];
		HIP_TRY(hipEventRecord(e->ev_ready, e->ctx->stream));
		if (j) HIP_TRY(hipStreamWaitEvent(bst, e->ev_ready, 0));
		lead->h_frames[j] = e->f;
		lead->h_devs[j] = e->d;
		lead->h_devs[j].frame = lead->d_frames + j;
		rows_total += s.hctu;
		needs_rd = needs_rd || s.rd_mode == RDM_FULL;
	}
	const int nctu = lead->seq.nctu, pitch = GATHER_HEAD + nctu + POST_MAX_ROWS;
	if ((size_t)pitch * n > lead->gather_words) {
		if (lead->d_gather) (void)hipFree(lead->d_gather);
		if (lead->h_gather) (void)hipHostFree(lead->h_gather);
		lead->d_gather = lead->h_gather = nullptr;
		lead->gather_words = 0;
		HIP_TRY(hipMalloc((void **)&lead->d_gather, (size_t)pitch * BATCH_MAX * 4));
		HIP_TRY(hipHostMalloc((void **)&lead->h_gather, (size_t)pitch * BATCH_MAX * 4, hipHostMallocDefault));
		lead->gather_words = (size_t)pitch * BATCH_MAX;
	}
	hipLaunchKernelGGL(k_batch_stage, dim3(n), dim3(256), 0, bst, (const EncDev *)lead->h_devs, (const FrameCtx *)lead->h_frames, (EncDev *)lead->d_batch, lead->d_frames);
	HIP_TRY(hipGetLastError());
	HIP_TRY(hipEventRecord(lead->ev_batch0, bst));
	if ((rc = launch_pool(lead, lead->h_devs, n, rows_total, needs_rd, bst))) return rc;
	(void)hipEventRecord(lead->ev_batch1, bst);
	hipLaunchKernelGGL(k_gather_results, dim3(n), dim3(256), 0, bst, (const EncDev *)lead->d_batch, lead->d_gather, pitch, (const int *)(lead->d_pool_state + BATCH_MAX * POOL_STRIDE));
	HIP_TRY(hipGetLastError());
	HIP_TRY(hipMemcpyAsync(lead->h_gather, lead->d_gather, (size_t)pitch * n * 4, hipMemcpyDeviceToHost, bst));
	{
		const hipError_t waited = hipStreamSynchronize(bst);
		if (waited != hipSuccess) { hmr_set_error("k_encode_pool: %s", hipGetErrorString(waited)); return HMR_GPU_ERR_HIP; }
	}
	float ms = 0;
	HIP_TRY(hipEventElapsedTime(&ms, lead->ev_batch0, lead->ev_batch1));
	HostState seq_state = start_state;
	bool cut_before = false;
	for (int j = 0; j < n; j++) {
		hmr_gpu_enc *e = encs[j];
		const Seq &s = e->seq;
		const uint32_t *g = lead->h_gather + (size_t)j * pitch;
		if (g[3] & 2) { hmr_set_error("k_encode_pool: the launch was abandoned by its watchdog (HENC_WATCHDOG_S)"); return HMR_GPU_ERR_HIP; }
		if (g[3] & 1) { hmr_set_error("hmr_gpu_enc_encode_chain: frame %d: a CTU row's sub-stream outgrew its buffer (%d bytes)", j, e->row_cap); return HMR_GPU_ERR_HIP; }
		e->note_stale_predictions(g[3] >> 8);
		e->last_ms = e->last_total_ms = ms;
		e->last_encodes = (int)g[1];
		e->f.scene_cut_ctu = (int)g[2];
		e->last_passes = 1;
		const bool fired = (int)g[2] >= 0;
		if (fired && cut_before) {
			hmr_set_error("hmr_gpu_enc_encode_chain: two frames of the chain detected a scene change: in the sequential order the first one switches the detection off for the second; repeat the chain frame by frame");
			return HMR_GPU_ERR_ARG;
		}
		cut_before = cut_before || fired;
		FrameCtx replay;
		e->st = seq_state;
		begin_frame(s, e->st, image_types ? image_types[j] : 0, replay);
		double acc_dist;
		memcpy(&acc_dist, &g[8], 8);
		memcpy(&e->f.avg_dist, &g[10], 8);
		if (replay.slice_type != e->f.slice_type || replay.poc != e->f.poc || replay.avg_dist != e->f.avg_dist) {
			hmr_set_error("hmr_gpu_enc_encode_chain: frame %d started from a state the frames before it changed", j);
			return HMR_GPU_ERR_ARG;
		}
		FrameRcOut ro;
		ro.sum_qp = (int)g[4]; ro.consumed_bits = (double)g[5];
		memcpy(&ro.target_pict_size, &g[6], 8);
		end_frame(s, e->st, e->f, acc_dist, &ro);
		seq_state = e->st;
		const int rows = s.wpp ? s.hctu : 1;
		std::vector<uint32_t> row_bytes(g + pitch - POST_MAX_ROWS, g + pitch - POST_MAX_ROWS + rows);
		size_t total = 0;
		for (int r = 0; r < rows; r++) total += row_bytes[r];
		if (e->h_bs.size() < total) e->h_bs.resize(total);
		total = 0;
		for (int r = 0; r < rows; r++) {
			HIP_TRY(hipMemcpyAsync(e->h_bs.data() + total, e->d_bs + (size_t)r * e->row_cap, row_bytes[r], hipMemcpyDeviceToHost, bst));
			total += row_bytes[r];
		}
		HIP_TRY(hipStreamSynchronize(bst));
		if ((rc = frame_assemble(e, e->f, e->h_bs.data(), row_bytes.data(), streams[j], caps[j], &stream_bytes[j])) < 0) return rc;
	}
	return HMR_GPU_OK;
}

extern "C" int hmr_gpu_enc_encode(hmr_gpu_enc *e, const uint8_t *y, const uint8_t *u, const uint8_t *v, int image_type, uint8_t *stream, long cap, long *stream_bytes,
				  uint8_t *recon)
{
	const int rc = hmr_gpu_enc_load_source(e, 0, y, u, v);
	if (rc) return rc;
	return hmr_gpu_enc_encode_source(e, 0, image_type, stream, cap, stream_bytes, recon);
}
```

homerhevc_amd/csrc/k_encode_object.inc:

```
template <class T>
struct PinnedAlloc {
	typedef T value_type;
	PinnedAlloc() = default;
	template <class U> PinnedAlloc(const PinnedAlloc<U> &) {}
	T *allocate(size_t n)
	{
		void *p = nullptr;
		if (hipHostMalloc(&p, n * sizeof(T), hipHostMallocDefault) != hipSuccess) throw std::bad_alloc();
		return (T *)p;
	}
	void deallocate(T *p, size_t) { (void)hipHostFree(p); }
	template <class U> bool operator==(const PinnedAlloc<U> &) const { return true; }
	template <class U> bool operator!=(const PinnedAlloc<U> &) const { return false; }
};

struct PlaneSet { uint8_t *y = nullptr, *c[2] = {nullptr, nullptr}; size_t bytes_y = 0, bytes_c = 0; int device = 0; };
struct PlanePool {
	std::mutex m;
	std::vector<PlaneSet> free_sets;
	int acquire(int device, size_t by, size_t bc, PlaneSet *out)
	{
		{
			std::lock_guard<std::mutex> lk(m);
			for (size_t i = 0; i < free_sets.size(); i++)
				if (free_sets[i].device == device && free_sets[i].bytes_y == by && free_sets[i].bytes_c == bc) {
					*out = free_sets[i];
					free_sets.erase(free_sets.begin() + (long)i);
					return HMR_GPU_OK;
				}
		}
		PlaneSet p;
		p.device = device; p.bytes_y = by; p.bytes_c = bc;
		if (hipMalloc((void **)&p.y, by) != hipSuccess || hipMalloc((void **)&p.c[0], bc) != hipSuccess || hipMalloc((void **)&p.c[1], bc) != hipSuccess) {
			(void)hipGetLastError();
			if (p.y) (void)hipFree(p.y);
			if (p.c[0]) (void)hipFree(p.c[0]);
			if (p.c[1]) (void)hipFree(p.c[1]);
			hmr_set_error("phase planes: out of device memory (%zu bytes per picture)", by + 2 * bc);
			return HMR_GPU_ERR_HIP;
		}
		*out = p;
		return HMR_GPU_OK;
	}
	void release(const PlaneSet &p)
	{
		std::lock_guard<std::mutex> lk(m);
		free_sets.push_back(p);
	}
	int live = 0;
	void encoder_created() { std::lock_guard<std::mutex> lk(m); live++; }
	void encoder_destroyed()
	{
		std::lock_guard<std::mutex> lk(m);
		if (--live > 0) return;
		for (PlaneSet &p : free_sets) {
			(void)hipSetDevice(p.device);
			(void)hipFree(p.y); (void)hipFree(p.c[0]); (void)hipFree(p.c[1]);
		}
		free_sets.clear();
	}
};
PlanePool g_plane_pool;
struct hmr_gpu_enc {
	hmr_gpu_ctx *ctx;
	HostCfg cfg;
	long stale_last = -1, stale_total = 0;
	void note_stale_predictions(uint32_t n) { stale_last = (long)n; stale_total += (long)n; }
	Seq seq;
	HostState st;
	FrameCtx f;
	EncDev d;
	Seq *d_seq;
	FrameCtx *d_frame;
	Geo *d_geo;
	std::vector<Geo> geo;
	std::vector<SrcSlot> src;
	int16_t *d_pic[2][3], *d_pre[3], *d_rec[3];
	PostRow *d_rows = nullptr;
	RowEnt *d_ent = nullptr;
	uint8_t *d_bs = nullptr;
	uint32_t *d_cumbits = nullptr;
	double *d_sao_tab = nullptr;
	int *d_post_err = nullptr;
	RdCtxSim rdsim[MAX_ENGINES];
	uint8_t *d_ctx_ring = nullptr, *d_rd_init = nullptr;
	int *d_rd_src = nullptr;
	uint8_t h_rd_init[(1 + RD_RING) * RD_CTX_BYTES] = {0};
	uint16_t *d_rc_need = nullptr;
	RcFrame *d_rc_dyn = nullptr;
	int row_cap = 0;
	std::vector<RowEnt> h_ent;
	std::vector<uint8_t, PinnedAlloc<uint8_t>> h_bs;
	PlaneSet chain_planes2;
	PlaneSet chain_planes;
	PlaneSet planes;
	size_t src_elems[3], pic_elems[3];
	uint8_t *d_bytes;
	int units_stride, units_rows;
	int16_t *d_mvx, *d_mvy;
	int8_t *d_ref;
	uint8_t *d_qp, *d_flags;
	uint8_t *d_public;
	std::vector<uint8_t, PinnedAlloc<uint8_t>> h_public;
	std::vector<int16_t, PinnedAlloc<int16_t>> h_coeff;
	std::vector<int32_t> h_stats, h_params;
	std::vector<double> h_lambdas;
	hipEvent_t ev_frame = nullptr, ev_ready = nullptr, ev_batch0 = nullptr, ev_batch1 = nullptr;
	int n_cus = 0;
	uint8_t *d_stage = nullptr, *h_stage = nullptr;
	size_t stage_bytes = 0;
	void *d_batch = nullptr;
	bool pending = false, download_queued = false;
	std::vector<hmr_gpu_enc *> pend_encs;
	std::vector<size_t> pend_off;
	std::vector<std::vector<uint32_t>> pend_rows;
	size_t *h_offs = nullptr;
	size_t pend_total = 0;
	hipStream_t copy_stream = nullptr;
	uint32_t *d_gather = nullptr, *h_gather = nullptr;
	size_t gather_words = 0;
	bool awaiting_delivery = false;
	FrameCtx f_pending;
	double acc_pending = 0;
	hipEvent_t ev_packed = nullptr;
	hipEvent_t ev_decided = nullptr;
	FrameCtx *d_frames = nullptr, *h_frames = nullptr;
	EncDev *h_devs = nullptr;
	hipStream_t plane_stream[2] = {nullptr, nullptr};
	hipEvent_t ev_plane[3] = {nullptr, nullptr, nullptr};
	int *d_pool_state = nullptr;
	WorkSlow *d_pool_slow = nullptr;
	int pool_workers = 0;
	int last_pool_kernel = -1;
	JobRing<IngestJob> ingest;
	JobRing<RgbIngestJob> ingest_rgb;
	JobRing<ScaleJob> scale;
	JobRing<EgressJob> egress;
	JobRing<SsimJob> ssim;
	JobRing<RgbEgressJob> egress_rgb;
	JobRing<RgbScaleJob> scale_rgb;
	bool has_picture = false;
	hipStream_t pic_stream = nullptr;
	hipEvent_t ev_pic_done = nullptr, ev_own_done = nullptr;
	EntropyState es;
	CtuInfo *d_ctus_eng[MAX_ENGINES] = {nullptr};
	uint8_t *d_rowstate_eng[MAX_ENGINES] = {nullptr};
	int *d_seen_eng[MAX_ENGINES] = {nullptr};
	hmr_gpu_enc *twin_of = nullptr;
	int local_engines = 1, engine_index = -1;
	int cur, lockstep;
	int raster = 0;
	float last_ms, last_total_ms;
	int last_passes, last_encodes;
};

namespace {
void release_planes(hmr_gpu_enc *e);
constexpr int REC_BYTES = 32 + 3 * 256 + 2 * 256 + 9 * 256 + 256 + 256 + 2048 + 2048 + 6144 * 2 + 6144 * 2 + 2 * 5 * 256;

int16_t *plane0(hmr_gpu_enc *e, int which, int comp)
{
	const Seq &s = e->seq;
	const int st = comp ? s.stride_c : s.stride_y, m = comp ? s.margin_c : s.margin_y;
	return e->d_pic[which][comp] + (size_t)m * st + m;
}

template <class T>
int dev_alloc(T **p, size_t n, hipStream_t st)
{
	HIP_TRY(hipMalloc((void **)p, n * sizeof(T)));
	HIP_TRY(hipMemsetAsync(*p, 0, n * sizeof(T), st));
	HIP_TRY(hipStreamSynchronize(st));
	return HMR_GPU_OK;
}
#define DEV_ALLOC(p, n)                           \
	do {                                      \
		const int rc_ = dev_alloc(&(p), (n), e->ctx->stream); \
		if (rc_) return rc_;              \
	} while (0)

IngestJob ingest_job(const hmr_gpu_enc *e, const hmr_gpu_picture &pic, int16_t *const dst[3], int stride_y, int stride_c)
{
	IngestJob j;
	for (int c = 0; c < 3; c++) {
		j.src[c] = pic.plane[c];
		j.pitch[c] = pic.pitch[c];
		j.dst[c] = dst[c];
	}
	j.stride_y = stride_y; j.stride_c = stride_c;
	j.width = e->seq.width; j.height = e->seq.height;
	j.format = pic.format; j.reserved = 0;
	return j;
}
EgressJob egress_job(hmr_gpu_enc *e, const hmr_gpu_picture *pic, int16_t *const src[3], uint64_t *ssd)
{
	const Seq &s = e->seq;
	EgressJob j;
	for (int c = 0; c < 3; c++) {
		j.rec[c] = plane0(e, e->cur, c);
		j.src[c] = src ? src[c] : nullptr;
		j.dst[c] = pic ? const_cast<uint8_t *>(pic->plane[c]) : nullptr;
		j.pitch[c] = pic ? pic->pitch[c] : 0;
	}
	j.ssd = ssd;
	j.stride_y = s.stride_y; j.stride_c = s.stride_c;
	j.src_stride_y = s.src_stride_y; j.src_stride_c = s.src_stride_c;
	j.width = s.width; j.height = s.height;
	j.format = pic ? pic->format : HMR_GPU_PIC_I420; j.reserved = 0;
	return j;
}
hmr_gpu_picture packed_picture(const hmr_gpu_enc *e, const uint8_t *bytes)
{
	const int64_t w = e->seq.width, h = e->seq.height;
	return hmr_gpu_picture{HMR_GPU_PIC_I420, 0, {bytes, bytes + w * h, bytes + w * h + (w / 2) * (h / 2)}, {w, w / 2, w / 2}};
}
int widen_packed(hmr_gpu_enc *e, const uint8_t *bytes, int16_t *const dst[3], int stride_y, int stride_c)
{
	const IngestJob j = ingest_job(e, packed_picture(e, bytes), dst, stride_y, stride_c);
	return run_jobs(e->ingest, hmr_ingest_launch, e->ctx->stream, &j, 1, e->ctx->stream);
}
int narrow_packed(hmr_gpu_enc *e, uint8_t *bytes)
{
	const hmr_gpu_picture pic = packed_picture(e, bytes);
	const EgressJob j = egress_job(e, &pic, nullptr, nullptr);
	return run_jobs(e->egress, hmr_egress_launch, e->ctx->stream, &j, 1, e->ctx->stream);
}

int load_planes(hmr_gpu_enc *e, const uint8_t *y, const uint8_t *u, const uint8_t *v, int16_t *const dst[3], int stride_y, int stride_c)
{
	hipStream_t st = e->ctx->stream;
	const hmr_gpu_picture staged = packed_picture(e, e->d_bytes);
	const uint8_t *in[3] = {y, u, v};
	for (int c = 0; c < 3; c++)
		HIP_TRY(hipMemcpyAsync(const_cast<uint8_t *>(staged.plane[c]), in[c], (size_t)staged.pitch[c] * (c ? e->seq.height / 2 : e->seq.height), hipMemcpyHostToDevice, st));
	const int rc = widen_packed(e, e->d_bytes, dst, stride_y, stride_c);
	if (rc) return rc;
	HIP_TRY(hipStreamSynchronize(st));
	return HMR_GPU_OK;
}


int reference_planes(hmr_gpu_enc *e, hipStream_t st)
{
	const Seq &s = e->seq;
	if (e->f.slice_type == SLICE_I) return HMR_GPU_OK;
	return hmr_subpel_planes_on(st, e->d_pic[e->cur ^ 1][0], e->d_pic[e->cur ^ 1][1], e->d_pic[e->cur ^ 1][2], s.stride_y, s.height + 2 * s.margin_y, s.stride_c,
				    s.height / 2 + 2 * s.margin_c, e->planes.y, e->planes.c[0], e->planes.c[1]);
}
int ctu_stage_prepare(hmr_gpu_enc *e, bool planes_elsewhere = false)
{
	const Seq &s = e->seq;
	hipStream_t st = e->ctx->stream;
	if (!e->lockstep)
		HIP_TRY(hipMemcpyAsync(e->d.ctus_start, e->d.ctus, sizeof(CtuInfo) * s.nctu, hipMemcpyDeviceToDevice, st));
	if (!planes_elsewhere) {
		const int rc = reference_planes(e, st);
		if (rc) return rc;
	}
	{
		static const int zero_counters[3] = {0, 0, -1};
		HIP_TRY(hipMemcpyAsync(e->d.counters, zero_counters, sizeof zero_counters, hipMemcpyHostToDevice, st));
	}
	if (e->lockstep) {
		HIP_TRY(hipMemsetAsync(e->d.progress, 0, sizeof(int) * s.hctu, st));
		HIP_TRY(hipMemsetAsync(e->d.row0_checked, 0, sizeof(int), st));
		HIP_TRY(hipMemsetAsync(e->d.prefix, 0, sizeof(uint32_t) * s.hctu * (s.wctu + 1), st));
	}
	HIP_TRY(hipMemsetAsync(e->d_rows, 0, sizeof(PostRow) * s.hctu, st));
	HIP_TRY(hipMemsetAsync(e->d_post_err, 0, sizeof(int) * 4, st));
	return HMR_GPU_OK;
}
int lockstep_collect(hmr_gpu_enc *e)
{
	hipStream_t st = e->ctx->stream;
	int counters[3], aborted = 0;
	HIP_TRY(hipMemcpyAsync(counters, e->d.counters, sizeof counters, hipMemcpyDeviceToHost, st));
	HIP_TRY(hipMemcpyAsync(&aborted, e->d_pool_state + BATCH_MAX * POOL_STRIDE + 1, sizeof(int), hipMemcpyDeviceToHost, st));
	HIP_TRY(hipStreamSynchronize(st));
	e->last_encodes = counters[1];
	e->f.scene_cut_ctu = counters[2];
	e->last_passes = 1;
	release_planes(e);
	if (aborted) {
		hmr_set_error("k_encode_pool: the launch was abandoned by its watchdog (a worker found nothing to do for too long: HENC_WATCHDOG_S)");
		return HMR_GPU_ERR_HIP;
	}
	return HMR_GPU_OK;
}

static int pool_inflight(const Seq &s, int raster = 0)
{
	if (raster) return 3;
	const int by_step = s.hctu < (s.wctu + 1) / 2 ? s.hctu : (s.wctu + 1) / 2;
	return s.bitrate_mode != 0 ? (by_step + 1) / 2 : by_step;
}
int launch_pool(hmr_gpu_enc *lead, const EncDev *host, int n, int rows_total, bool needs_rd, hipStream_t st)
{
	if (!lead->n_cus) HIP_TRY(hipDeviceGetAttribute(&lead->n_cus, hipDeviceAttributeMultiprocessorCount, lead->ctx->device));
#if defined(HENC_PROFILE)
	const size_t lds_default = LDS_BYTES + (needs_rd ? 0 : 0);
#else
	const size_t lds_default = needs_rd ? LDS_BYTES : LDS_BYTES - LDS_RD;
#endif
	const size_t lds_bytes = getenv("HENC_LDS_BYTES") && (size_t)atoi(getenv("HENC_LDS_BYTES")) > lds_default ? (size_t)atoi(getenv("HENC_LDS_BYTES")) : lds_default;
	if (lds_bytes > 160 * 1024) {
		hmr_set_error("k_encode_pool: a worker's LDS request of %zu bytes (HENC_LDS_BYTES) is more than a CU has", lds_bytes);
		return HMR_GPU_ERR_ARG;
	}
	const int cap = lead->n_cus * workers_per_cu(lds_bytes);
	int workers = rows_total < cap ? rows_total : cap;
	if (workers < 1) workers = 1;
	if (getenv("HENC_POOL_WORKERS") && atoi(getenv("HENC_POOL_WORKERS")) > 0 && atoi(getenv("HENC_POOL_WORKERS")) < workers) workers = atoi(getenv("HENC_POOL_WORKERS"));
	const int kernel = workers <= lead->n_cus ? 0 : (needs_rd ? 2 : 1);
	if (kernel == 1)
		for (int i = 0; i < n; i++)
			if (host[i].rd_src) {
				hmr_set_error("k_encode_pool: picture %d of the launch is RD_FULL, and this kernel's walk is compiled without full RDO (needs_rd was not set)", i);
				return HMR_GPU_ERR_ARG;
			}
	if (!lead->d_pool_state) HIP_TRY(hipMalloc((void **)&lead->d_pool_state, sizeof(int) * (BATCH_MAX * POOL_STRIDE + 4)));
	if (lead->pool_workers < workers) {
		if (lead->d_pool_slow) (void)hipFree(lead->d_pool_slow);
		lead->d_pool_slow = nullptr;
		lead->pool_workers = 0;
		HIP_TRY(hipMalloc((void **)&lead->d_pool_slow, sizeof(WorkSlow) * workers));
		HIP_TRY(hipMemsetAsync(lead->d_pool_slow, 0, sizeof(WorkSlow) * workers, st));
		lead->pool_workers = workers;
	}
	HIP_TRY(hipMemsetAsync(lead->d_pool_state, 0, sizeof(int) * (BATCH_MAX * POOL_STRIDE + 4), st));
	double watchdog_s = getenv("HENC_WATCHDOG_S") ? atof(getenv("HENC_WATCHDOG_S")) : 120.0;
	if (!(watchdog_s > 0)) watchdog_s = 120.0;
	const unsigned long long watchdog = (unsigned long long)(watchdog_s * 1e8);
	auto *const fn = kernel == 0 ? k_encode_pool_lat : (kernel == 1 ? k_encode_pool : k_encode_full);
	hipLaunchKernelGGL(fn, dim3(workers), dim3(ENC_THREADS), lds_bytes, st, (const EncDev *)lead->d_batch, n, lead->d_pool_state, lead->d_pool_state + BATCH_MAX * POOL_STRIDE,
			   lead->d_pool_slow, watchdog, (unsigned)lds_default);
	const hipError_t launched = hipGetLastError();
	if (launched != hipSuccess) {
		hmr_set_error("k_encode_pool: %s", hipGetErrorString(launched));
		return HMR_GPU_ERR_HIP;
	}
	lead->last_pool_kernel = kernel;
	return HMR_GPU_OK;
}

int run_ctu_passes(hmr_gpu_enc *e)
{
	const Seq &s = e->seq;
	hipStream_t st = e->ctx->stream;
	int rc = ctu_stage_prepare(e);
	if (rc) return rc;
	HIP_TRY(hipEventRecord(e->ctx->ev0, st));
	if (e->lockstep) {
		if (!e->d_batch) HIP_TRY(hipMalloc((void **)&e->d_batch, BATCH_MAX * sizeof(EncDev)));
		HIP_TRY(hipMemcpyAsync(e->d_batch, &e->d, sizeof(EncDev), hipMemcpyHostToDevice, st));
		if ((rc = launch_pool(e, &e->d, 1, e->raster ? pool_inflight(s, 1) : s.hctu, s.rd_mode == RDM_FULL, st))) return rc;
		HIP_TRY(hipEventRecord(e->ctx->ev1, st));
		if ((rc = lockstep_collect(e))) return rc;
		HIP_TRY(hipEventElapsedTime(&e->last_ms, e->ctx->ev0, e->ctx->ev1));
		return HMR_GPU_OK;
	}
	int pass = 0;
	for (;; pass++) {
		HIP_TRY(hipMemsetAsync(e->d.progress, 0, sizeof(int) * s.hctu, st));
		{
			EncDev dd = e->d;
			int pp = pass;
			void *args[] = {&dd, &pp};
			const hipError_t launched = hipLaunchCooperativeKernel((const void *)k_encode_ctus, dim3(s.hctu), dim3(ENC_THREADS), args, (unsigned)LDS_BYTES, st);
			if (launched != hipSuccess) {
				hmr_set_error("k_encode_ctus (%d row workers, cooperative): %s", s.hctu, hipGetErrorString(launched));
				return HMR_GPU_ERR_HIP;
			}
		}
		hipLaunchKernelGGL(k_sched_scan, dim3(1), dim3(320), 0, st, e->d);
		hipLaunchKernelGGL(k_sched_check, dim3(s.nctu), dim3(64), 0, st, e->d);
		HIP_TRY(hipGetLastError());
		int counters[3];
		HIP_TRY(hipMemcpyAsync(counters, e->d.counters, sizeof counters, hipMemcpyDeviceToHost, st));
		HIP_TRY(hipStreamSynchronize(st));
		e->last_encodes = counters[1];
		e->f.scene_cut_ctu = counters[2];
		if (counters[0] == 0) break;
		if (pass > s.nctu + 2) {
			hmr_set_error("hmr_gpu_enc: the CTU schedule did not converge");
			return HMR_GPU_ERR_HIP;
		}
	}
	hipLaunchKernelGGL(k_sched_finish, dim3(s.nctu), dim3(64), 0, st, e->d);
	HIP_TRY(hipMemcpyAsync(e->d.chain_start, e->d.chain_end, MODE_STATE_BYTES, hipMemcpyDeviceToDevice, st));
	HIP_TRY(hipMemcpyAsync(e->d_frame, &e->f, sizeof(FrameCtx), hipMemcpyHostToDevice, st));
	HIP_TRY(hipFuncSetAttribute((const void *)k_post_frame, hipFuncAttributeMaxDynamicSharedMemorySize, (int)sizeof(PostScratch)));
	hipLaunchKernelGGL(k_post_frame, dim3(s.hctu < 32 ? s.hctu : 32), dim3(64), sizeof(PostScratch), st, e->d);
	HIP_TRY(hipGetLastError());
	HIP_TRY(hipEventRecord(e->ctx->ev1, st));
	HIP_TRY(hipStreamSynchronize(st));
	HIP_TRY(hipEventElapsedTime(&e->last_ms, e->ctx->ev0, e->ctx->ev1));
	e->last_passes = pass + 1;
	release_planes(e);
	return HMR_GPU_OK;
}

int set_frame(hmr_gpu_enc *e, int slot, int image_type, double avg_dist, bool upload = true, bool chain = false)
{
	const Seq &s = e->seq;
	e->cur ^= 1;
	e->has_picture = true;
	e->pic_stream = e->ctx->stream;
	{
		const int k = e->local_engines > 1 ? e->st.num_encoded_frames % e->local_engines : 0;
		e->d.ctus = e->d_ctus_eng[k];
		e->d.rowstate = e->d_rowstate_eng[k];
		e->d.thread_seen = e->d_seen_eng[k];
	}
	begin_frame(s, e->st, image_type, e->f);
	if (avg_dist >= 0) e->f.avg_dist = avg_dist;
	e->f.lockstep = e->lockstep && !e->raster;
	for (int c = 0; c < 3; c++) {
		e->f.src[c] = e->src[slot].p[c];
		e->f.ref[c] = plane0(e, e->cur ^ 1, c);
		e->f.rec[c] = e->d_rec[c] + (size_t)(c ? s.margin_c : s.margin_y) * (c ? s.stride_c : s.stride_y) + (c ? s.margin_c : s.margin_y);
		e->d.post.fin[c] = plane0(e, e->cur, c);
	}
	e->d.post.sao_lambda = e->d_sao_tab + (e->f.slice_type == SLICE_I ? 104 : 0);
	e->d.post.ctx_after = nullptr;
	if (s.rd_mode == RDM_FULL) {
		std::vector<RdCtxVersion> src;
		e->rdsim[e->local_engines > 1 ? e->f.num_encoded_frames % e->local_engines : 0].frame(e->f.num_encoded_frames, src, e->raster != 0);
		std::vector<int> codes(s.nctu);
		for (int n = 0; n < s.nctu; n++) {
			const RdCtxVersion v = src[n];
			if (v.frame > e->f.num_encoded_frames || (v.frame >= 0 && v.frame <= e->f.num_encoded_frames - RD_RING)) {
				hmr_set_error("RD_FULL: CTU %d copies coder states of frame %d in frame %d (the states of %d frames are kept)", n, v.frame, e->f.num_encoded_frames, RD_RING);
				return HMR_GPU_ERR_ARG;
			}
			const int slot = v.frame < 0 ? 0 : v.frame % RD_RING;
			codes[n] = v.frame < 0 ? 0 : (v.k == 0 ? (1 << 28) | (slot << 24) : (3 << 28) | (slot << 24) | (v.row * s.wctu + v.k - 1));
		}
		const int slot_now = e->f.num_encoded_frames % RD_RING;
		for (int i = 0; i < CTX_TOTAL; i++) e->h_rd_init[(1 + slot_now) * RD_CTX_BYTES + i] = Cabac::init_state(e->f.slice_type, e->f.qp, i);
		HIP_TRY(hipMemcpyAsync(e->d_rd_src, codes.data(), sizeof(int) * s.nctu, hipMemcpyHostToDevice, e->ctx->stream));
		HIP_TRY(hipMemcpyAsync(e->d_rd_init, e->h_rd_init, sizeof e->h_rd_init, hipMemcpyHostToDevice, e->ctx->stream));
		e->d.post.ctx_after = e->d_ctx_ring + (size_t)slot_now * s.nctu * RD_CTX_BYTES;
		e->d.rd_src = e->d_rd_src;
		e->d.rd_init = e->d_rd_init;
		e->d.rd_ring = e->d_ctx_ring;
	}
	e->d.dep = -1;
	e->d.dep_full = 0;
	e->d.after = -1;
	e->d.next_frame = nullptr;
	e->d.post.planes[0] = e->d.post.planes[1] = e->d.post.planes[2] = nullptr;
	if (e->f.slice_type != SLICE_I && !chain) {
		if (!e->planes.y) {
			const int rc = g_plane_pool.acquire(e->ctx->device, (size_t)16 * s.plane_elems_y, (size_t)64 * s.plane_elems_c, &e->planes);
			if (rc) return rc;
		}
		e->f.sub_y = e->planes.y + (size_t)s.margin_y * 16 * s.stride_y + s.margin_y;
		e->f.sub_c[0] = e->planes.c[0] + (size_t)s.margin_c * 64 * s.stride_c + s.margin_c;
		e->f.sub_c[1] = e->planes.c[1] + (size_t)s.margin_c * 64 * s.stride_c + s.margin_c;
	}
	if (upload) HIP_TRY(hipMemcpyAsync(e->d_frame, &e->f, sizeof(FrameCtx), hipMemcpyHostToDevice, e->ctx->stream));
	return HMR_GPU_OK;
}

void release_planes(hmr_gpu_enc *e)
{
	if (e->planes.y) g_plane_pool.release(e->planes);
	e->planes = PlaneSet();
}

__global__ __launch_bounds__(256) void k_copy_planes(const int16_t *s0, const int16_t *s1, const int16_t *s2, int16_t *d0, int16_t *d1, int16_t *d2, size_t n0, size_t n12)
{
	const int c = (int)blockIdx.y;
	const uint4 *s = (const uint4 *)(c == 0 ? s0 : (c == 1 ? s1 : s2));
	uint4 *d = (uint4 *)(c == 0 ? d0 : (c == 1 ? d1 : d2));
	const size_t n = (c == 0 ? n0 : n12) / 8;
	for (size_t i = (size_t)blockIdx.x * blockDim.x + threadIdx.x; i < n; i += (size_t)gridDim.x * blockDim.x) d[i] = s[i];
}

__global__ void k_pack_public(const CtuInfo *ctus, uint32_t *out)
{
	const uint32_t *src = (const uint32_t *)(const CtuPublic *)(ctus + blockIdx.x);
	uint32_t *dst = out + (size_t)blockIdx.x * (sizeof(CtuPublic) / 4);
	for (int i = threadIdx.x; i < (int)(sizeof(CtuPublic) / 4); i += blockDim.x) dst[i] = src[i];
}
__global__ void k_sum_stale(const CtuInfo *ctus, int nctu, int *out)
{
	int n = 0;
	for (int c = threadIdx.x; c < nctu; c += blockDim.x) n += ctus[c].n_stale_pred;
	if (n) atomicAdd(out, n);
}
int download_public(hmr_gpu_enc *e)
{
	const Seq &s = e->seq;
	hipLaunchKernelGGL(k_sum_stale, dim3(1), dim3(256), 0, e->ctx->stream, (const CtuInfo *)e->d.ctus, s.nctu, e->d_post_err + 3);
	hipLaunchKernelGGL(k_pack_public, dim3(s.nctu), dim3(256), 0, e->ctx->stream, e->d.ctus, (uint32_t *)e->d_public);
	HIP_TRY(hipGetLastError());
	HIP_TRY(hipMemcpyAsync(e->h_public.data(), e->d_public, sizeof(CtuPublic) * s.nctu, hipMemcpyDeviceToHost, e->ctx->stream));
	return HMR_GPU_OK;
}
}

extern "C" int hmr_gpu_enc_record_bytes(void) { return REC_BYTES; }

static thread_local int g_serial_pool = 0;
static int enc_create(hmr_gpu_ctx *ctx, const hmr_gpu_enc_cfg *cfg, int engine_index, hmr_gpu_enc **out)
{
	if (!ctx || !cfg || !out) return HMR_GPU_ERR_ARG;
	static_assert(sizeof(hmr_gpu_enc_cfg) == sizeof(HostCfg), "configuration layouts must match");
	static_assert(offsetof(CtuInfo, n_spec_reads) % 4 == 0 && sizeof(Node) % 4 == 0 && sizeof(Geo) % 2 == 0 && sizeof(Seq) % 4 == 0 && sizeof(FrameCtx) % 4 == 0 && sizeof(CtuPublic) % 4 == 0 && MODE_STATE_BYTES % 4 == 0, "word copies");
	hmr_gpu_enc *e = new hmr_gpu_enc();
	e->ctx = ctx;
	memcpy(&e->cfg, cfg, sizeof(HostCfg));
	const char *why = "";
	if (!make_seq(e->cfg, e->seq, &why)) {
		hmr_set_error("hmr_gpu_enc_create: configuration outside the built rows: %s", why);
		delete e;
		return HMR_GPU_ERR_ARG;
	}
	e->st.engines = clampi(e->cfg.num_enc_engines, 1, MAX_ENGINES);
	e->engine_index = engine_index;
	e->local_engines = engine_index >= 0 ? 1 : e->st.engines;
	if (e->st.engines > 1 && e->cfg.wfpp_num_threads < 2 && engine_index >= 0) {
		hmr_set_error("hmr_gpu_enc_create: configuration outside the built rows: num_enc_engines > 1 needs the row-per-thread schedule (wfpp_num_threads > 1)");
		delete e;
		return HMR_GPU_ERR_ARG;
	}
	if (engine_index >= e->st.engines) { delete e; return HMR_GPU_ERR_ARG; }
#if defined(HENC_NO_RDFULL)
	if (e->seq.rd_mode == RDM_FULL) {
		hmr_set_error("hmr_gpu_enc_create: this library was built with -DHENC_NO_RDFULL and cannot encode rd_mode RD_FULL");
		delete e;
		return HMR_GPU_ERR_ARG;
	}
#endif
	if (e->cfg.bitrate_mode != 0) host_rc_init(e->cfg, e->seq, e->st);
	g_plane_pool.encoder_created();
	struct Guard {
		hmr_gpu_enc *e;
		bool ok = false;
		~Guard() { if (!ok) hmr_gpu_enc_destroy(e); }
	} guard{e};
	e->seq.wide_min_n = 0;
	e->raster = e->cfg.wfpp_num_threads <= 1 && (e->cfg.bitrate_mode != 0 || e->seq.rd_mode == RDM_FULL || g_serial_pool || e->st.engines > 1);
	e->lockstep = e->cfg.wfpp_num_threads > 1 || e->raster;
	const Seq &s = e->seq;
	HIP_TRY(hipSetDevice(ctx->device));
	e->geo.resize(NNODES);
	make_geo(e->geo.data());
	DEV_ALLOC(e->d_seq, 1);
	HIP_TRY(hipMemcpy(e->d_seq, &s, sizeof(Seq), hipMemcpyHostToDevice));
	DEV_ALLOC(e->d_frame, 1);
	DEV_ALLOC(e->d_geo, NNODES);
	HIP_TRY(hipMemcpy(e->d_geo, e->geo.data(), sizeof(Geo) * NNODES, hipMemcpyHostToDevice));
	HIP_TRY(hipMemcpyToSymbol(HIP_SYMBOL(henc_geo_table), e->geo.data(), sizeof(Geo) * NNODES));
	DEV_ALLOC(e->d.ctus, s.nctu);
	if (e->cfg.wfpp_num_threads <= 1) DEV_ALLOC(e->d.ctus_start, s.nctu);
	{
		std::vector<CtuInfo> init(s.nctu);
		memset((void *)init.data(), 0, sizeof(CtuInfo) * s.nctu);
		for (auto &c : init) memset(c.mv_ref_idx, -1, sizeof c.mv_ref_idx);
		HIP_TRY(hipMemcpy(e->d.ctus, init.data(), sizeof(CtuInfo) * s.nctu, hipMemcpyHostToDevice));
		e->d_ctus_eng[0] = e->d.ctus;
		for (int k = 1; k < e->local_engines; k++) {
			DEV_ALLOC(e->d_ctus_eng[k], s.nctu);
			HIP_TRY(hipMemcpy(e->d_ctus_eng[k], init.data(), sizeof(CtuInfo) * s.nctu, hipMemcpyHostToDevice));
		}
	}
	if (e->cfg.wfpp_num_threads <= 1) DEV_ALLOC(e->d.work_slow, s.hctu);
	HIP_TRY(hipFuncSetAttribute((const void *)k_encode_ctus, hipFuncAttributeMaxDynamicSharedMemorySize, (int)LDS_BYTES));
	HIP_TRY(hipFuncSetAttribute((const void *)k_encode_pool, hipFuncAttributeMaxDynamicSharedMemorySize, 160 * 1024));
	HIP_TRY(hipFuncSetAttribute((const void *)k_encode_pool_lat, hipFuncAttributeMaxDynamicSharedMemorySize, 160 * 1024));
	HIP_TRY(hipFuncSetAttribute((const void *)k_encode_full, hipFuncAttributeMaxDynamicSharedMemorySize, 160 * 1024));
	HIP_TRY(hipEventCreate(&e->ev_frame));
	HIP_TRY(hipEventCreate(&e->ev_ready));
	HIP_TRY(hipEventCreate(&e->ev_batch0));
	HIP_TRY(hipEventCreate(&e->ev_batch1));
	HIP_TRY(hipEventCreateWithFlags(&e->ev_packed, hipEventDisableTiming));
	HIP_TRY(hipEventCreateWithFlags(&e->ev_decided, hipEventDisableTiming));
	DEV_ALLOC(e->d.coeff, (size_t)6144 * s.nctu);
	DEV_ALLOC(e->d.progress, s.hctu);
	DEV_ALLOC(e->d.prefix, (size_t)s.hctu * (s.wctu + 1));
	DEV_ALLOC(e->d.prof, (size_t)s.hctu * PF_COUNT + (size_t)s.nctu * 4);
	DEV_ALLOC(e->d.guess, (size_t)s.nctu * MODE_STATE_BYTES);
	DEV_ALLOC(e->d.truth, (size_t)s.nctu * MODE_STATE_BYTES);
	DEV_ALLOC(e->d.outtok, (size_t)s.nctu * MODE_STATE_BYTES);
	DEV_ALLOC(e->d.chain_start, MODE_STATE_BYTES);
	DEV_ALLOC(e->d.chain_end, MODE_STATE_BYTES);
	DEV_ALLOC(e->d.valid, s.nctu);
	DEV_ALLOC(e->d.dirty, s.nctu);
	DEV_ALLOC(e->d.hash, s.nctu);
	DEV_ALLOC(e->d.intra_before, s.nctu);
	DEV_ALLOC(e->d.used_intra, s.nctu);
	DEV_ALLOC(e->d.used_parts, s.nctu);
	DEV_ALLOC(e->d.counters, 4);
	DEV_ALLOC(e->d.rowstate, (size_t)s.hctu * ROW_STATE_BYTES);
	DEV_ALLOC(e->d.thread_seen, 64);
	e->d_rowstate_eng[0] = e->d.rowstate;
	e->d_seen_eng[0] = e->d.thread_seen;
	for (int k = 1; k < e->local_engines; k++) {
		DEV_ALLOC(e->d_rowstate_eng[k], (size_t)s.hctu * ROW_STATE_BYTES);
		DEV_ALLOC(e->d_seen_eng[k], 64);
	}
	DEV_ALLOC(e->d.row0_checked, 1);
	for (int c = 0; c < 3; c++) {
		e->src_elems[c] = (size_t)(c ? s.src_stride_c : s.src_stride_y) * (c ? s.height / 2 : s.height);
		e->pic_elems[c] = (size_t)(c ? s.stride_c : s.stride_y) * ((c ? s.height / 2 : s.height) + 2 * (c ? s.margin_c : s.margin_y));
		for (int k = 0; k < 2; k++) DEV_ALLOC(e->d_pic[k][c], e->pic_elems[c]);
		DEV_ALLOC(e->d_pre[c], e->pic_elems[c]);
		DEV_ALLOC(e->d_rec[c], e->pic_elems[c]);
	}
	{
		e->row_cap = s.wctu * CTU_STREAM_BOUND;
		DEV_ALLOC(e->d_rows, s.hctu);
		DEV_ALLOC(e->d_ent, s.hctu);
		DEV_ALLOC(e->d_bs, (size_t)e->row_cap * s.hctu);
		DEV_ALLOC(e->d_cumbits, s.nctu);
		DEV_ALLOC(e->d_sao_tab, 2 * 52 * 2);
		DEV_ALLOC(e->d_post_err, 4 + 2 * 16 + 4);
		double tab[2][104];
		sao_lambda_table(s, SLICE_P, tab[0]);
		sao_lambda_table(s, SLICE_I, tab[1]);
		HIP_TRY(hipMemcpy(e->d_sao_tab, tab, sizeof tab, hipMemcpyHostToDevice));
		e->h_ent.resize(s.hctu);
		DEV_ALLOC(e->d_rc_dyn, 1);
		if (s.rd_mode == RDM_FULL) {
			for (auto &sim : e->rdsim) sim.init(e->cfg.wfpp_num_threads > 1 ? e->cfg.wfpp_num_threads : 1, s.wctu, s.hctu, s.sao);
			DEV_ALLOC(e->d_ctx_ring, (size_t)RD_RING * s.nctu * RD_CTX_BYTES);
			HIP_TRY(hipMemset(e->d_ctx_ring, 0, (size_t)RD_RING * s.nctu * RD_CTX_BYTES));
			DEV_ALLOC(e->d_rd_init, (1 + RD_RING) * RD_CTX_BYTES);
			DEV_ALLOC(e->d_rd_src, s.nctu);
		}
		if (e->cfg.bitrate_mode != 0 || s.rd_mode == RDM_FULL) {
			std::vector<uint16_t> need;
			if (!rc_need_table(s.wctu, s.hctu, s.sao, e->cfg.wfpp_num_threads > 1, need)) {
				hmr_set_error("hmr_gpu_enc_create: rate control: the reference's entropy-coding lag is not row-monotone on a %d x %d CTU grid", s.wctu, s.hctu);
				return HMR_GPU_ERR_ARG;
			}
			DEV_ALLOC(e->d_rc_need, need.size());
			HIP_TRY(hipMemcpy(e->d_rc_need, need.data(), need.size() * sizeof(uint16_t), hipMemcpyHostToDevice));
		}
	}
	DEV_ALLOC(e->d_bytes, (size_t)s.width * s.height * 3 / 2);
	e->units_stride = s.wctu * 16;
	e->units_rows = s.hctu * 16;
	const size_t nu = (size_t)e->units_stride * e->units_rows;
	DEV_ALLOC(e->d_mvx, nu); DEV_ALLOC(e->d_mvy, nu); DEV_ALLOC(e->d_ref, nu); DEV_ALLOC(e->d_qp, nu);
	DEV_ALLOC(e->d_flags, nu);
	DEV_ALLOC(e->d_public, sizeof(CtuPublic) * s.nctu);
	e->h_public.resize(sizeof(CtuPublic) * s.nctu);
	e->h_coeff.resize((size_t)6144 * s.nctu);
	e->h_stats.resize((size_t)s.nctu * 3 * 5 * 2 * 32);
	e->h_params.resize((size_t)s.nctu * 3 * 34);
	e->d.seq = e->d_seq;
	e->d.frame = e->d_frame;
	e->d.tables = ctx->tables;
	e->d.geo = e->d_geo;
	e->d.rc_dyn = e->d_rc_dyn;
	{
		const size_t oy = (size_t)s.margin_y * s.stride_y + s.margin_y, oc = (size_t)s.margin_c * s.stride_c + s.margin_c;
		PostPic &P = e->d.post;
		memset(&P, 0, sizeof P);
		P.dbk[0] = e->d_pre[0] + oy; P.dbk[1] = e->d_pre[1] + oc; P.dbk[2] = e->d_pre[2] + oc;
		P.units_stride = e->units_stride;
		P.mvx = e->d_mvx; P.mvy = e->d_mvy; P.ref = e->d_ref; P.uqp = e->d_qp; P.flags = e->d_flags;
		P.rows = e->d_rows; P.ent = e->d_ent; P.bs = e->d_bs; P.row_cap = e->row_cap; P.cumbits = e->d_cumbits;
		P.sao_lambda = e->d_sao_tab; P.errors = e->d_post_err; P.rc_need = e->d_rc_need;
		P.prof = (unsigned long long *)(e->d_post_err + 4);
		e->d.fin = (double *)(e->d_post_err + 4 + 2 * 16);
	}
	e->cur = 0;
	e->d.raster = e->raster;
	e->d.threads = e->cfg.wfpp_num_threads > 1 ? e->cfg.wfpp_num_threads : 1;
	e->last_ms = e->last_total_ms = 0;
	e->last_passes = e->last_encodes = 0;
	HIP_TRY(hipStreamSynchronize(ctx->stream));
	guard.ok = true;
	*out = e;
	return HMR_GPU_OK;
}

extern "C" int hmr_gpu_enc_create(hmr_gpu_ctx *ctx, const hmr_gpu_enc_cfg *cfg, hmr_gpu_enc **out) { return enc_create(ctx, cfg, -1, out); }
extern "C" int hmr_gpu_enc_create_serial_pool(hmr_gpu_ctx *ctx, const hmr_gpu_enc_cfg *cfg, hmr_gpu_enc **out)
{
	if (!cfg || cfg->wfpp_num_threads > 1 || cfg->num_enc_engines > 1) {
		hmr_set_error("hmr_gpu_enc_create_serial_pool: wfpp_num_threads and num_enc_engines must be 1");
		return HMR_GPU_ERR_ARG;
	}
	g_serial_pool = 1;
	const int rc = enc_create(ctx, cfg, -1, out);
	g_serial_pool = 0;
	return rc;
}
extern "C" int hmr_gpu_enc_create_engine(hmr_gpu_ctx *ctx, const hmr_gpu_enc_cfg *cfg, int engine_index, hmr_gpu_enc **out)
{
	if (engine_index < 0) return HMR_GPU_ERR_ARG;
	return enc_create(ctx, cfg, engine_index, out);
}
extern "C" int hmr_gpu_enc_create_engine_twin(hmr_gpu_ctx *ctx, hmr_gpu_enc *of, hmr_gpu_enc **out)
{
	if (!ctx || !of || !out || of->engine_index < 0 || of->twin_of) return HMR_GPU_ERR_ARG;
	hmr_gpu_enc *t = nullptr;
	const int rc = enc_create(ctx, (const hmr_gpu_enc_cfg *)&of->cfg, of->engine_index, &t);
	if (rc) return rc;
	(void)hipFree(t->d_ctus_eng[0]);
	(void)hipFree(t->d_rowstate_eng[0]);
	(void)hipFree(t->d_seen_eng[0]);
	t->d_ctus_eng[0] = of->d_ctus_eng[0];
	t->d_rowstate_eng[0] = of->d_rowstate_eng[0];
	t->d_seen_eng[0] = of->d_seen_eng[0];
	t->d.ctus = t->d_ctus_eng[0]; t->d.rowstate = t->d_rowstate_eng[0]; t->d.thread_seen = t->d_seen_eng[0];
	t->twin_of = of;
	*out = t;
	return HMR_GPU_OK;
}
extern "C" int hmr_gpu_enc_state_bytes(void) { return (int)sizeof(HostState); }
extern "C" long hmr_gpu_enc_reference_elems(hmr_gpu_enc *e, int comp) { return e && comp >= 0 && comp < 3 ? (long)e->pic_elems[comp] : -1; }

extern "C" int hmr_gpu_enc_export_reference(hmr_gpu_enc *e, int16_t *dy, int16_t *du, int16_t *dv, void *state)
{
	if (!e || !dy || !du || !dv || !state) return HMR_GPU_ERR_ARG;
	hipStream_t st = e->ctx->stream;
	HIP_TRY(hipSetDevice(e->ctx->device));
	int16_t *dst[3] = {dy, du, dv};
	for (int c = 0; c < 3; c++) HIP_TRY(hipMemcpyAsync(dst[c], e->d_pic[e->cur][c], e->pic_elems[c] * 2, hipMemcpyDeviceToDevice, st));
	HIP_TRY(hipStreamSynchronize(st));
	memcpy(state, &e->st, sizeof(HostState));
	return HMR_GPU_OK;
}
extern "C" int hmr_gpu_enc_import_reference(hmr_gpu_enc *e, const int16_t *dy, const int16_t *du, const int16_t *dv, const void *state)
{
	if (!e || !dy || !du || !dv || !state) return HMR_GPU_ERR_ARG;
	HostState in;
	memcpy(&in, state, sizeof in);
	if (in.engines != e->st.engines || (e->engine_index >= 0 && in.num_encoded_frames % e->st.engines != e->engine_index)) {
		hmr_set_error("hmr_gpu_enc_import_reference: state of frame %d does not precede a frame of engine %d of %d", in.num_encoded_frames - 1, e->engine_index, e->st.engines);
		return HMR_GPU_ERR_ARG;
	}
	hipStream_t st = e->ctx->stream;
	HIP_TRY(hipSetDevice(e->ctx->device));
	const int16_t *src[3] = {dy, du, dv};
	for (int c = 0; c < 3; c++) HIP_TRY(hipMemcpyAsync(e->d_pic[e->cur][c], src[c], e->pic_elems[c] * 2, hipMemcpyDeviceToDevice, st));
	HIP_TRY(hipStreamSynchronize(st));
	e->st = in;
	return HMR_GPU_OK;
}

extern "C" long hmr_gpu_enc_reference_bytes(hmr_gpu_enc *e) { return e ? (long)e->seq.width * e->seq.height * 3 / 2 : -1; }
extern "C" int hmr_gpu_enc_export_references8(hmr_gpu_enc **encs, int n, uint8_t *dev_rows, long pitch, void *states)
{
	if (!encs || n <= 0 || !dev_rows || !states) return HMR_GPU_ERR_ARG;
	for (int i = 0; i < n; i++) {
		hmr_gpu_enc *e = encs[i];
		if (!e || pitch < hmr_gpu_enc_reference_bytes(e)) return HMR_GPU_ERR_ARG;
		HIP_TRY(hipSetDevice(e->ctx->device));
		const int rc = narrow_packed(e, dev_rows + (size_t)i * pitch);
		if (rc) return rc;
		memcpy((uint8_t *)states + (size_t)i * sizeof(HostState), &e->st, sizeof(HostState));
	}
	for (int i = 0; i < n; i++) HIP_TRY(hipStreamSynchronize(encs[i]->ctx->stream));
	return HMR_GPU_OK;
}
extern "C" int hmr_gpu_enc_import_references8(hmr_gpu_enc **encs, int n, const uint8_t *dev_rows, long pitch, const void *states)
{
	if (!encs || n <= 0 || !dev_rows || !states) return HMR_GPU_ERR_ARG;
	for (int i = 0; i < n; i++) {
		hmr_gpu_enc *e = encs[i];
		if (!e || pitch < hmr_gpu_enc_reference_bytes(e)) return HMR_GPU_ERR_ARG;
		HostState in;
		memcpy(&in, (const uint8_t *)states + (size_t)i * sizeof(HostState), sizeof in);
		if (in.engines != e->st.engines || (e->engine_index >= 0 && in.num_encoded_frames % e->st.engines != e->engine_index)) {
			hmr_set_error("hmr_gpu_enc_import_references8: engine %d: state of frame %d does not precede a frame of engine %d of %d", i, in.num_encoded_frames - 1, e->engine_index, e->st.engines);
			return HMR_GPU_ERR_ARG;
		}
		const Seq &s = e->seq;
		HIP_TRY(hipSetDevice(e->ctx->device));
		int16_t *dst[3] = {plane0(e, e->cur, 0), plane0(e, e->cur, 1), plane0(e, e->cur, 2)};
		int rc = widen_packed(e, dev_rows + (size_t)i * pitch, dst, s.stride_y, s.stride_c);
		if (rc) return rc;
		hmr_gpu_frame fr = {s.width, s.height, dst[0], dst[1], dst[2], s.stride_y, s.stride_c};
		rc = hmr_gpu_pad_frame(e->ctx, &fr, s.margin_y, s.margin_y);
		if (rc) return rc;
		e->st = in;
	}
	for (int i = 0; i < n; i++) HIP_TRY(hipStreamSynchronize(encs[i]->ctx->stream));
	return HMR_GPU_OK;
}

extern "C" void hmr_gpu_enc_destroy(hmr_gpu_enc *e)
{
	if (!e) return;
	(void)hipSetDevice(e->ctx->device);
	(void)hipStreamSynchronize(e->ctx->stream);
	release_planes(e);
	for (PlaneSet *ps : {&e->chain_planes, &e->chain_planes2})
		if (ps->y) { (void)hipFree(ps->y); (void)hipFree(ps->c[0]); (void)hipFree(ps->c[1]); }
	e->d.ctus = e->d_ctus_eng[0]; e->d.rowstate = e->d_rowstate_eng[0]; e->d.thread_seen = e->d_seen_eng[0];
	if (e->twin_of) e->d.ctus = nullptr, e->d.rowstate = nullptr, e->d.thread_seen = nullptr;
	for (int k = 1; k < MAX_ENGINES; k++) {
		if (e->d_ctus_eng[k]) (void)hipFree(e->d_ctus_eng[k]);
		if (e->d_rowstate_eng[k]) (void)hipFree(e->d_rowstate_eng[k]);
		if (e->d_seen_eng[k]) (void)hipFree(e->d_seen_eng[k]);
	}
	if (e->ev_frame) (void)hipEventDestroy(e->ev_frame);
	if (e->ev_ready) (void)hipEventDestroy(e->ev_ready);
	if (e->ev_batch0) (void)hipEventDestroy(e->ev_batch0);
	if (e->ev_batch1) (void)hipEventDestroy(e->ev_batch1);
	if (e->ev_packed) (void)hipEventDestroy(e->ev_packed);
	if (e->ev_decided) (void)hipEventDestroy(e->ev_decided);
	if (e->d_frames) (void)hipFree(e->d_frames);
	if (e->h_frames) (void)hipHostFree(e->h_frames);
	if (e->h_devs) (void)hipHostFree(e->h_devs);
	for (int k = 0; k < 2; k++) if (e->plane_stream[k]) { (void)hipStreamSynchronize(e->plane_stream[k]); (void)hipStreamDestroy(e->plane_stream[k]); }
	for (int k = 0; k < 3; k++) if (e->ev_plane[k]) (void)hipEventDestroy(e->ev_plane[k]);
	if (e->copy_stream) { (void)hipStreamSynchronize(e->copy_stream); (void)hipStreamDestroy(e->copy_stream); }
	if (e->d_gather) (void)hipFree(e->d_gather);
	if (e->h_gather) (void)hipHostFree(e->h_gather);
	if (e->h_offs) (void)hipHostFree(e->h_offs);
	e->ingest.release();
	e->ingest_rgb.release();
	e->scale.release();
	e->egress.release();
	e->ssim.release();
	e->egress_rgb.release();
	e->scale_rgb.release();
	if (e->ev_pic_done) (void)hipEventDestroy(e->ev_pic_done);
	if (e->ev_own_done) (void)hipEventDestroy(e->ev_own_done);
	if (e->d_batch) (void)hipFree(e->d_batch);
	if (e->d_pool_state) (void)hipFree(e->d_pool_state);
	if (e->d_pool_slow) (void)hipFree(e->d_pool_slow);
	if (e->d_stage) (void)hipFree(e->d_stage);
	if (e->h_stage) (void)hipHostFree(e->h_stage);
	void *p[] = {e->d_seq, e->d_frame, e->d_geo, e->d.ctus, e->d.ctus_start, e->d.work_slow, e->d.coeff, e->d.progress, e->d.prefix, e->d.prof, e->d.guess, e->d.truth, e->d.outtok,
		     e->d.chain_start, e->d.chain_end, e->d.valid, e->d.dirty, e->d.hash, e->d.intra_before, e->d.used_intra, e->d.used_parts, e->d.counters, e->d.rowstate, e->d.thread_seen, e->d.row0_checked, e->d_bytes, e->d_mvx,
		     e->d_mvy, e->d_ref, e->d_qp, e->d_flags, e->d_public};
	for (void *q : p) (void)hipFree(q);
	for (int c = 0; c < 3; c++) {
		(void)hipFree(e->d_pic[0][c]);
		(void)hipFree(e->d_pic[1][c]);
		(void)hipFree(e->d_pre[c]);
		(void)hipFree(e->d_rec[c]);
	}
	{
		void *pp[] = {e->d_rows, e->d_ent, e->d_bs, e->d_cumbits, e->d_sao_tab, e->d_post_err, e->d_rc_need, e->d_rc_dyn, e->d_ctx_ring, e->d_rd_init, e->d_rd_src};
		for (void *q : pp) (void)hipFree(q);
	}
	for (auto &sl : e->src)
		for (int c = 0; c < 3; c++) (void)hipFree(sl.p[c]);
	delete e;
	g_plane_pool.encoder_destroyed();
}

extern "C" int hmr_gpu_enc_post_profile(hmr_gpu_enc *e, unsigned long long *out)
{
	if (!e || !out) return HMR_GPU_ERR_ARG;
	HIP_TRY(hipMemcpy(out, e->d_post_err + 4, 16 * sizeof(unsigned long long), hipMemcpyDeviceToHost));
#if defined(HENC_POST_PROFILE)
	HIP_TRY(hipMemcpyFromSymbol(out + 10, HIP_SYMBOL(g_ent_prof), 6 * sizeof(unsigned long long)));
#endif
	return HMR_GPU_OK;
}

extern "C" float hmr_gpu_enc_last_ctu_ms(hmr_gpu_enc *e) { return e ? e->last_ms : 0.f; }

extern "C" int hmr_gpu_enc_stale_predictions(hmr_gpu_enc *e, long *last_picture, long *all_pictures)
{
	if (!e) return HMR_GPU_ERR_ARG;
	if (last_picture) *last_picture = e->stale_last;
	if (all_pictures) *all_pictures = e->stale_total;
	return HMR_GPU_OK;
}

extern "C" int hmr_gpu_enc_last_stats(hmr_gpu_enc *e, int *passes, int *ctu_encodes, float *ctu_ms, float *frame_ms)
{
	if (!e) return HMR_GPU_ERR_ARG;
	if (passes) *passes = e->last_passes;
	if (ctu_encodes) *ctu_encodes = e->last_encodes;
	if (ctu_ms) *ctu_ms = e->last_ms;
	if (frame_ms) *frame_ms = e->last_total_ms;
	return HMR_GPU_OK;
}

extern "C" int hmr_gpu_enc_last_pool_kernel(hmr_gpu_enc *e) { return e ? e->last_pool_kernel : -1; }

extern "C" int hmr_gpu_enc_timeline(hmr_gpu_enc *e, unsigned long long *out)
{
	if (!e || !out) return HMR_GPU_ERR_ARG;
	HIP_TRY(hipMemcpy(out, e->d.prof + (size_t)e->seq.hctu * PF_COUNT, sizeof(unsigned long long) * e->seq.nctu * 4, hipMemcpyDeviceToHost));
	return HMR_GPU_OK;
}

extern "C" int hmr_gpu_enc_profile(hmr_gpu_enc *e, unsigned long long *out, int reset)
{
	if (!e || !out) return HMR_GPU_ERR_ARG;
	HIP_TRY(hipMemcpy(out, e->d.prof, sizeof(unsigned long long) * e->seq.hctu * PF_COUNT, hipMemcpyDeviceToHost));
	if (reset) {
		HIP_TRY(hipMemsetAsync(e->d.prof, 0, sizeof(unsigned long long) * e->seq.hctu * PF_COUNT, e->ctx->stream));
		HIP_TRY(hipStreamSynchronize(e->ctx->stream));
	}
	return HMR_GPU_OK;
}

extern "C" int hmr_gpu_enc_load_source(hmr_gpu_enc *e, int slot, const uint8_t *y, const uint8_t *u, const uint8_t *v)
{
	if (!e || slot < 0 || slot > 4096 || !y || !u || !v) return HMR_GPU_ERR_ARG;
	HIP_TRY(hipSetDevice(e->ctx->device));
	while ((int)e->src.size() <= slot) {
		SrcSlot sl;
		for (int c = 0; c < 3; c++) DEV_ALLOC(sl.p[c], e->src_elems[c]);
		e->src.push_back(sl);
	}
	return load_planes(e, y, u, v, e->src[slot].p, e->seq.src_stride_y, e->seq.src_stride_c);
}

extern "C" int hmr_gpu_enc_frame_ctus(hmr_gpu_enc *e, const uint8_t *y, const uint8_t *u, const uint8_t *v, int image_type, const uint8_t *ref_y, const uint8_t *ref_u,
				      const uint8_t *ref_v, double avg_dist, uint8_t *records)
{
	if (!e || !y || !u || !v) return HMR_GPU_ERR_ARG;
	const Seq &s = e->seq;
	hipStream_t st = e->ctx->stream;
	HIP_TRY(hipSetDevice(e->ctx->device));
	int rc = hmr_gpu_enc_load_source(e, 0, y, u, v);
	if (rc) return rc;
	rc = set_frame(e, 0, image_type, avg_dist);
	if (rc) return rc;
	if (ref_y && ref_u && ref_v) {
		int16_t *dst[3] = {plane0(e, e->cur ^ 1, 0), plane0(e, e->cur ^ 1, 1), plane0(e, e->cur ^ 1, 2)};
		rc = load_planes(e, ref_y, ref_u, ref_v, dst, s.stride_y, s.stride_c);
		if (rc) return rc;
		hmr_gpu_frame fr = {s.width, s.height, dst[0], dst[1], dst[2], s.stride_y, s.stride_c};
		rc = hmr_gpu_pad_frame(e->ctx, &fr, s.margin_y, s.margin_y);
		if (rc) return rc;
	}
	rc = run_ctu_passes(e);
	if (rc) return rc;
	rc = download_public(e);
	if (rc) return rc;
	HIP_TRY(hipStreamSynchronize(st));
	end_frame(s, e->st, e->f, frame_acc_dist(s, e->cfg.wfpp_num_threads, [&](int n) { return ((const CtuPublic *)(e->h_public.data() + sizeof(CtuPublic) * n))->distortion; }));
	if (records) {
		std::vector<int16_t> rec[3];
		std::vector<uint8_t> truth((size_t)s.nctu * MODE_STATE_BYTES), chain_end(MODE_STATE_BYTES);
		std::vector<uint32_t> node0(3 * s.nctu);
		HIP_TRY(hipMemcpy(e->h_coeff.data(), e->d.coeff, e->h_coeff.size() * 2, hipMemcpyDeviceToHost));
		HIP_TRY(hipMemcpy(truth.data(), e->d.truth, truth.size(), hipMemcpyDeviceToHost));
		HIP_TRY(hipMemcpy(chain_end.data(), e->d.chain_end, MODE_STATE_BYTES, hipMemcpyDeviceToHost));
		for (int n = 0; n < s.nctu; n++) {
			Node nd;
			HIP_TRY(hipMemcpy(&nd, &e->d.ctus[n].nodes[0], sizeof(Node), hipMemcpyDeviceToHost));
			node0[3 * n] = nd.cost; node0[3 * n + 1] = nd.distortion; node0[3 * n + 2] = nd.sum;
		}
		for (int c = 0; c < 3; c++) {
			rec[c].resize(e->pic_elems[c]);
			HIP_TRY(hipMemcpy(rec[c].data(), e->d_rec[c], e->pic_elems[c] * 2, hipMemcpyDeviceToHost));
		}
		memset(records, 0, (size_t)REC_BYTES * s.nctu);
		for (int n = 0; n < s.nctu; n++) {
			uint8_t *o = records + (size_t)n * REC_BYTES;
			const CtuPublic &ci = *(const CtuPublic *)(e->h_public.data() + sizeof(CtuPublic) * n);
			int32_t hdr[8] = {0x43545544, e->f.num_encoded_frames, n, e->f.slice_type, (int32_t)node0[3 * n], (int32_t)node0[3 * n + 1], (int32_t)node0[3 * n + 2],
					  e->f.scene_cut_ctu >= 0 && n >= e->f.scene_cut_ctu};
			memcpy(o, hdr, 32); o += 32;
			for (int k = 0; k < 3; k++) { memcpy(o, ci.cbf[k], 256); o += 256; }
			memcpy(o, ci.intra_mode[0], 256); o += 256;
			memcpy(o, ci.intra_mode[1], 256); o += 256;
			const uint8_t *arrs[9] = {ci.inter_mode, ci.tr_idx, ci.pred_depth, ci.part_size_type, ci.pred_mode, ci.skipped, ci.merge, ci.merge_idx, ci.qp};
			for (int k = 0; k < 9; k++) { memcpy(o, arrs[k], 256); o += 256; }
			memcpy(o, ci.mv_ref_idx, 256); o += 256;
			memcpy(o, ci.mv_diff_ref_idx, 256); o += 256;
			memcpy(o, ci.mv_ref, 2048); o += 2048;
			memcpy(o, ci.mv_diff, 2048); o += 2048;
			memcpy(o, e->h_coeff.data() + (size_t)n * 6144, 12288); o += 12288;
			for (int c = 0; c < 3; c++) {
				const int nn = c ? 32 : 64, px = (ci.x >> (c ? 1 : 0)), py = (ci.y >> (c ? 1 : 0));
				const int pw = c ? s.width / 2 : s.width, ph = c ? s.height / 2 : s.height, rs = c ? s.stride_c : s.stride_y, m = c ? s.margin_c : s.margin_y;
				const int16_t *p = rec[c].data() + (size_t)m * rs + m;
				for (int yy = 0; yy < nn; yy++) {
					if (py + yy < ph) {
						const int ww = px + nn <= pw ? nn : pw - px;
						memcpy(o, p + (size_t)(py + yy) * rs + px, ww * 2);
					}
					o += nn * 2;
				}
			}
			memcpy(o, n + 1 < s.nctu ? truth.data() + (size_t)(n + 1) * MODE_STATE_BYTES : chain_end.data(), MODE_STATE_BYTES);
		}
	}
	return e->f.slice_type;
}

namespace {
constexpr int GATHER_HEAD = 12;
constexpr int CHAIN_MAX_FRAMES = 32;
__global__ void k_gather_results(const EncDev *devs, uint32_t *out, int pitch, const int *pool_flags)
{
	const EncDev &d = devs[blockIdx.x];
	uint32_t *o = out + (size_t)blockIdx.x * pitch;
	const int nctu = d.seq->nctu;
	if (threadIdx.x < 3) o[threadIdx.x] = (uint32_t)d.counters[threadIdx.x];
	__shared__ uint32_t s_qp, s_bits, s_stale;
	if (threadIdx.x == 0) { s_qp = 0; s_bits = 0; s_stale = 0; }
	__syncthreads();
	uint32_t q = 0, b = 0, stale = 0;
	for (int c = threadIdx.x; c < nctu; c += blockDim.x) { q += d.ctus[c].nodes[0].qp; stale += (uint32_t)d.ctus[c].n_stale_pred; }
	for (int r = threadIdx.x; r < d.seq->hctu; r += blockDim.x) b += d.post.cumbits[r * d.seq->wctu + d.seq->wctu - 1];
	atomicAdd(&s_qp, q);
	atomicAdd(&s_bits, b);
	atomicAdd(&s_stale, stale);
	__syncthreads();
	if (threadIdx.x == 0) o[3] = (uint32_t)(d.post.errors[0] != 0) | ((uint32_t)(pool_flags && pool_flags[1] != 0) << 1) | ((s_stale > 0xffffffu ? 0xffffffu : s_stale) << 8);
	if (threadIdx.x == 0) {
		o[4] = s_qp;
		o[5] = s_bits;
		const double tp = d.counters[2] >= 0 ? d.rc_dyn->target_pict_size : d.frame->rc.target_pict_size;
		memcpy(&o[6], &tp, 8);
		const double fin = d.fin[0], avg = d.frame->avg_dist;
		memcpy(&o[8], &fin, 8);
		memcpy(&o[10], &avg, 8);
	}
	for (int c = threadIdx.x; c < nctu; c += blockDim.x) o[GATHER_HEAD + c] = d.ctus[c].distortion;
	for (int r = threadIdx.x; r < d.seq->hctu; r += blockDim.x) o[pitch - POST_MAX_ROWS + r] = (uint32_t)d.post.ent[r].bytecnt;
}

}

namespace {
int frame_assemble(hmr_gpu_enc *e, const FrameCtx &f, const uint8_t *bytes, const uint32_t *row_bytes, uint8_t *stream, long cap, long *stream_bytes)
{
	const Seq &s = e->seq;
	const int rows = s.wpp ? s.hctu : 1;
	std::vector<const uint8_t *> data(rows);
	std::vector<int> nb(rows);
	size_t o = 0;
	for (int r = 0; r < rows; r++) { data[r] = bytes + o; nb[r] = (int)row_bytes[r]; o += row_bytes[r]; }
	std::vector<uint8_t> out;
	assemble_access_unit(e->es, s, f, e->cfg.profile, data.data(), nb.data(), out);
	*stream_bytes = (long)out.size();
	if ((long)out.size() > cap) {
		hmr_set_error("hmr_gpu_enc_encode: the access unit needs %ld bytes, the buffer holds %ld", (long)out.size(), cap);
		return HMR_GPU_ERR_ARG;
	}
	memcpy(stream, out.data(), out.size());
	return f.slice_type;
}
int frame_finish(hmr_gpu_enc *e, int slot, uint8_t *stream, long cap, long *stream_bytes, uint8_t *recon)
{
	(void)slot;
	const Seq &s = e->seq;
	hipStream_t st = e->ctx->stream;
	int rc, err[4];
	HIP_TRY(hipMemcpyAsync(e->h_ent.data(), e->d_ent, sizeof(RowEnt) * s.hctu, hipMemcpyDeviceToHost, st));
	const int pitch = GATHER_HEAD + s.nctu + POST_MAX_ROWS;
	if (e->lockstep) {
		if ((size_t)pitch > e->gather_words) {
			if (e->d_gather) (void)hipFree(e->d_gather);
			if (e->h_gather) (void)hipHostFree(e->h_gather);
			e->d_gather = e->h_gather = nullptr;
			e->gather_words = 0;
			HIP_TRY(hipMalloc((void **)&e->d_gather, (size_t)pitch * 4));
			HIP_TRY(hipHostMalloc((void **)&e->h_gather, (size_t)pitch * 4, hipHostMallocDefault));
			e->gather_words = (size_t)pitch;
		}
		hipLaunchKernelGGL(k_gather_results, dim3(1), dim3(256), 0, st, (const EncDev *)e->d_batch, e->d_gather, pitch, (const int *)nullptr);
		HIP_TRY(hipGetLastError());
		HIP_TRY(hipMemcpyAsync(e->h_gather, e->d_gather, (size_t)pitch * 4, hipMemcpyDeviceToHost, st));
	} else if ((rc = download_public(e))) return rc;
	HIP_TRY(hipMemcpyAsync(err, e->d_post_err, sizeof err, hipMemcpyDeviceToHost, st));
	HIP_TRY(hipStreamSynchronize(st));
	if (getenv("HENC_DEBUG_POST")) {
		std::vector<PostRow> rows(s.hctu);
		HIP_TRY(hipMemcpy(rows.data(), e->d_rows, sizeof(PostRow) * s.hctu, hipMemcpyDeviceToHost));
		for (int r = 0; r < s.hctu; r++)
			fprintf(stderr, "post row %d: dec %d D %d/%d P %d/%d F %d/%d\n", r, rows[r].dec, rows[r].d_claim, rows[r].d_done, rows[r].p_claim, rows[r].p_done, rows[r].f_claim, rows[r].f_done);
		fprintf(stderr, "post errors %d %d %d %d, sao %d\n", err[0], err[1], err[2], err[3], s.sao);
	}
	if (err[0]) {
		hmr_set_error("hmr_gpu_enc_encode: a CTU row's sub-stream outgrew its buffer (%d bytes)", e->row_cap);
		return HMR_GPU_ERR_HIP;
	}
	if (err[2]) {
		hmr_set_error("hmr_gpu_enc_encode: the post-decision stage was abandoned by its watchdog");
		return HMR_GPU_ERR_HIP;
	}
	const int rows = s.wpp ? s.hctu : 1;
	std::vector<uint32_t> row_bytes(rows);
	size_t total = 0;
	for (int r = 0; r < rows; r++) total += row_bytes[r] = (uint32_t)e->h_ent[r].bytecnt;
	if (e->h_bs.size() < total) e->h_bs.resize(total);
	total = 0;
	for (int r = 0; r < rows; r++) {
		HIP_TRY(hipMemcpyAsync(e->h_bs.data() + total, e->d_bs + (size_t)r * e->row_cap, row_bytes[r], hipMemcpyDeviceToHost, st));
		total += row_bytes[r];
	}
	if (recon) {
		if ((rc = narrow_packed(e, e->d_bytes))) return rc;
		HIP_TRY(hipMemcpyAsync(recon, e->d_bytes, (size_t)s.width * s.height * 3 / 2, hipMemcpyDeviceToHost, st));
	}
	HIP_TRY(hipStreamSynchronize(st));
	const uint32_t *gr = e->h_gather;
	e->note_stale_predictions(e->lockstep ? gr[3] >> 8 : (uint32_t)err[3]);
	const double acc = e->lockstep ? frame_acc_dist(s, e->cfg.wfpp_num_threads, [&](int n) { return gr[GATHER_HEAD + n]; })
				       : frame_acc_dist(s, e->cfg.wfpp_num_threads, [&](int n) { return ((const CtuPublic *)(e->h_public.data() + sizeof(CtuPublic) * n))->distortion; });
	rc = frame_assemble(e, e->f, e->h_bs.data(), row_bytes.data(), stream, cap, stream_bytes);
	if (rc < 0) return rc;
	FrameRcOut ro = {0, 0.0, 0.0};
	if (e->lockstep) {
		ro.sum_qp = (int)gr[4]; ro.consumed_bits = (double)gr[5];
		memcpy(&ro.target_pict_size, &gr[6], 8);
	}
	end_frame(s, e->st, e->f, acc, &ro);
	HIP_TRY(hipEventRecord(e->ctx->ev1, st));
	HIP_TRY(hipStreamSynchronize(st));
	HIP_TRY(hipEventElapsedTime(&e->last_total_ms, e->ev_frame, e->ctx->ev1));
	return e->f.slice_type;
}
}

extern "C" int hmr_gpu_enc_encode_source(hmr_gpu_enc *e, int slot, int image_type, uint8_t *stream, long cap, long *stream_bytes, uint8_t *recon)
{
	if (!e || slot < 0 || slot >= (int)e->src.size() || !stream || !stream_bytes) return HMR_GPU_ERR_ARG;
	if (e->awaiting_delivery) {
		hmr_set_error("hmr_gpu_enc_encode_source: the encoder has an access unit outstanding from a pipelined batch call: flush first");
		return HMR_GPU_ERR_ARG;
	}
	hipStream_t st = e->ctx->stream;
	HIP_TRY(hipSetDevice(e->ctx->device));
	HIP_TRY(hipEventRecord(e->ev_frame, st));
	int rc = set_frame(e, slot, image_type, -1.0);
	if (rc) return rc;
	rc = run_ctu_passes(e);
	if (rc) return rc;
	return frame_finish(e, slot, stream, cap, stream_bytes, recon);
}
```

include/homer_gpu.h:

```cpp
#ifndef HOMER_GPU_H
#define HOMER_GPU_H

#include <stddef.h>
#include <stdint.h>

#ifdef __cplusplus
extern "C" {
#endif

typedef struct hmr_gpu_ctx hmr_gpu_ctx;

enum hmr_gpu_status {
	HMR_GPU_OK = 0,
	HMR_GPU_ERR_NO_DEVICE = -1,
	HMR_GPU_ERR_HIP = -2,
	HMR_GPU_ERR_ARG = -3,
	HMR_GPU_ERR_NOMEM = -4
};


int hmr_gpu_create(hmr_gpu_ctx **out, int device, void *stream);
void hmr_gpu_destroy(hmr_gpu_ctx *ctx);
const char *hmr_gpu_last_error(void);
int hmr_gpu_sync(hmr_gpu_ctx *ctx);
// ... 200 lines not shown
	uint32_t p0;
	uint32_t p1;
} hmr_gpu_tu_job;
int hmr_gpu_tu_chain_batch(hmr_gpu_ctx *ctx, const hmr_gpu_tu_job *jobs, int njobs, int size, const int16_t *orig_base, const int16_t *pred_base,
			   int16_t *level_base, int16_t *recon_base, uint32_t *ssd, int32_t *ac_sum);
uint32_t hmr_gpu_tu_chain(int16_t *orig, int orig_stride, int16_t *pred, int pred_stride, int16_t *levels, int16_t *recon, int recon_stride, int size,
			  int is_dst, int scan_mode, int comp, int is_intra, int slice_is_intra, int sign_hiding, int per, int rem, int *ac_sum);

typedef struct hmr_gpu_itu_job {
	uint32_t orig_off, orig_stride;
	uint32_t pred_off, pred_stride;
	uint32_t rec_off, rec_stride;
	uint32_t lev_off;
	uint32_t p0, p1;
	uint32_t dec_off, dec_stride;
	uint32_t flags;
	uint32_t sizes;
	uint32_t mode;
} hmr_gpu_itu_job;
int hmr_gpu_intra_tu_chain_batch(hmr_gpu_ctx *ctx, const hmr_gpu_itu_job *jobs, int njobs, int size, const int16_t *orig_base, const int16_t *decoded_base,
				 int16_t *pred_base, int16_t *level_base, int16_t *recon_base, uint32_t *ssd, int32_t *ac_sum);
uint32_t hmr_gpu_intra_tu_chain(int16_t *orig, int orig_stride, int16_t *decoded_corner, int decoded_stride, int left, int top, int bottom_left, int top_right,
				int bl_size, int tr_size, int strong_enabled, int is_filtered, int mode, int is_luma, int16_t *pred, int pred_stride, int16_t *levels,
				int16_t *recon, int recon_stride, int size, int is_dst, int scan_mode, int comp, int slice_is_intra, int sign_hiding, int per, int rem,
				int *ac_sum);
#define HMR_GPU_ITU_MODE_FROM_SEARCH 0x100u
struct hmr_gpu_intra_result;
int hmr_gpu_intra_tu_chain_modes_batch(hmr_gpu_ctx *ctx, const hmr_gpu_itu_job *jobs, int njobs, int size, const int16_t *orig_base, const int16_t *decoded_base,
				       int16_t *pred_base, int16_t *level_base, int16_t *recon_base, uint32_t *ssd, int32_t *ac_sum,
				       const struct hmr_gpu_intra_result *modes);
int hmr_gpu_intra_tu_chain_rounds_batch(hmr_gpu_ctx *ctx, const hmr_gpu_itu_job *jobs, int njobs, int rounds, int size, const int16_t *orig_base,
					const int16_t *decoded_base, int16_t *pred_base, int16_t *level_base, int16_t *recon_base, uint32_t *ssd, int32_t *ac_sum,
					const struct hmr_gpu_intra_result *modes);
typedef struct hmr_gpu_inter_tu_job {
	uint32_t orig_off, orig_stride;
	uint32_t pred_off, pred_stride;
	uint32_t rec_off, rec_stride;
	uint32_t lev_off;
	uint32_t p0, p1;
	uint32_t reserved;
	double weight, zero_thr;
} hmr_gpu_inter_tu_job;
#define HMR_GPU_INTER_TU_FROM_SOURCE 1u
int hmr_gpu_inter_tu_chain_batch(hmr_gpu_ctx *ctx, const hmr_gpu_inter_tu_job *jobs, int njobs, int size, const int16_t *residual_base, const int16_t *pred_base,
				 int16_t *level_base, int16_t *recon_base, uint32_t *ssd, int32_t *ac_sum);
uint32_t hmr_gpu_inter_tu_chain(int16_t *residual, int residual_stride, int16_t *pred, int pred_stride, int16_t *levels, int16_t *recon, int recon_stride, int size,
				int scan_mode, int comp, int slice_is_intra, int sign_hiding, int per, int rem, double weight, double zero_thr, int *ac_sum);

typedef struct hmr_gpu_inter_tu_host {
	int16_t *residual; int residual_stride;
	int16_t *pred; int pred_stride;
	int16_t *levels;
	int16_t *recon; int recon_stride;
	int size, scan_mode, comp, slice_is_intra, sign_hiding, per, rem;
	double weight, zero_thr;
	uint32_t ssd;
	int ac_sum;
} hmr_gpu_inter_tu_host;
void hmr_gpu_inter_tu_chain_n(hmr_gpu_inter_tu_host *tus, int n);

typedef struct hmr_gpu_intra_job {
	double sqrt_lambda;
	uint32_t orig_off, orig_stride;
	uint32_t dec_off, dec_stride;
	uint32_t adi_off, adif_off;
	uint32_t pred_off, pred_stride;
	uint32_t flags;
	uint32_t sizes;
	int32_t preds[3];
	uint32_t pred_bits[3];
	uint32_t other_bits;
	uint32_t reserved;
} hmr_gpu_intra_job;
typedef struct hmr_gpu_intra_result {
	int32_t best_mode;
	int32_t bits;
	double cost;
} hmr_gpu_intra_result;
int hmr_gpu_intra_search_batch(hmr_gpu_ctx *ctx, const hmr_gpu_intra_job *jobs, int njobs, int size, const int16_t *orig_base,
			       const int16_t *decoded_base, int16_t *out_base, hmr_gpu_intra_result *out);
void hmr_gpu_intra_search(int16_t *orig, int orig_stride, int16_t *decoded_corner, int decoded_stride, int n, int left, int top, int bottom_left,
			  int top_right, int bl_size, int tr_size, int strong_enabled, const int32_t *preds, const int32_t *pred_bits, int other_bits,
			  double sqrt_lambda, int16_t *adi, int16_t *adi_filtered, int16_t *pred, int pred_stride, int32_t *out, double *best_cost);


#define HMR_GPU_TREE_NO_PARENT 0xffffffffu
typedef struct hmr_gpu_tree_job {
	uint32_t parent;
	uint32_t child[4];
	uint32_t par_rec_off, par_rec_stride;
	uint32_t chl_rec_off, chl_rec_stride;
	uint32_t par_lev_off, chl_lev_off;
	uint32_t size;
	uint32_t rule;
} hmr_gpu_tree_job;
typedef struct hmr_gpu_tree_result {
	uint32_t split;
	uint32_t cost, sum;
	uint8_t cbf[4];
} hmr_gpu_tree_result;
int hmr_gpu_tree_decide_batch(hmr_gpu_ctx *ctx, const hmr_gpu_tree_job *jobs, int njobs, const uint32_t *ssd, const int32_t *ac_sum, int16_t *recon_base,
			      int16_t *level_base, hmr_gpu_tree_result *out);
void hmr_gpu_intra_luma_cu(int16_t *orig, int orig_stride, int16_t *dec_par, int dec_par_stride, int16_t *dec_chl, int dec_chl_stride, const int32_t *nb,
			   int strong_enabled, const int32_t *preds, const int32_t *pred_bits, int other_bits, double sqrt_lambda, int16_t *adi, int16_t *adi_filtered,
			   int16_t *pred, int pred_stride, int16_t *lev_par, int16_t *lev_chl, int size, int slice_is_intra, int sign_hiding, int per, int rem, int rule,
			   int32_t *out, double *best_cost);


typedef struct hmr_gpu_chroma_job {
	double sqrt_lambda;
	uint32_t orig_u_off, orig_v_off, orig_stride;
	uint32_t dec_u_off, dec_v_off, dec_stride;
	uint32_t flags;
	uint32_t sizes;
	uint32_t luma_mode;
	uint32_t reserved;
} hmr_gpu_chroma_job;
int hmr_gpu_chroma_search_batch(hmr_gpu_ctx *ctx, const hmr_gpu_chroma_job *jobs, int njobs, int size, const int16_t *orig_base, const int16_t *decoded_base,
				const hmr_gpu_intra_result *luma_modes, hmr_gpu_intra_result *out);
void hmr_gpu_intra_chroma_cu(int16_t *orig_u, int16_t *orig_v, int orig_stride, int16_t *dec_u, int16_t *dec_v, int dec_stride, const int32_t *nb, int luma_mode,
			     int split, double sqrt_lambda, double weight, int16_t *pred_u, int16_t *pred_v, int pred_stride, int16_t *lev_u, int16_t *lev_v, int size,
			     int slice_is_intra, int sign_hiding, int per, int rem, int32_t *out);


int hmr_gpu_sao_offsets_frame(hmr_gpu_ctx *ctx, const int32_t *stats, int n_ctu, const double *lambdas, int32_t *offsets, int32_t *aux, int64_t *dist);
void hmr_gpu_sao_offsets_ctu(const int32_t *stats, const double *lambdas, int32_t *offsets, int32_t *aux, int64_t *dist);


typedef struct hmr_gpu_enc_cfg {
	int32_t size, profile, width, height;
	float frame_rate;
	int32_t cu_size, max_pred_partition_depth, max_intra_tr_depth, max_inter_tr_depth, intra_period, gop_size, num_b, num_ref_frames;
	int32_t motion_estimation_precision, qp, chroma_qp_offset, num_enc_engines, wfpp_enable, wfpp_num_threads, sign_hiding, sample_adaptive_offset;
	int32_t bitrate_mode, bitrate, vbv_size, vbv_init, reinit_gop_on_scene_change, rd_mode, performance_mode;
} hmr_gpu_enc_cfg;
typedef struct hmr_gpu_enc hmr_gpu_enc;

int hmr_gpu_enc_create(hmr_gpu_ctx *ctx, const hmr_gpu_enc_cfg *cfg, hmr_gpu_enc **out);
int hmr_gpu_enc_create_serial_pool(hmr_gpu_ctx *ctx, const hmr_gpu_enc_cfg *cfg, hmr_gpu_enc **out);
void hmr_gpu_enc_destroy(hmr_gpu_enc *enc);
int hmr_gpu_enc_record_bytes(void);
int hmr_gpu_enc_frame_ctus(hmr_gpu_enc *enc, const uint8_t *y, const uint8_t *u, const uint8_t *v, int image_type, const uint8_t *ref_y, const uint8_t *ref_u,
			   const uint8_t *ref_v, double avg_dist, uint8_t *records);
float hmr_gpu_enc_last_ctu_ms(hmr_gpu_enc *enc);

int hmr_gpu_enc_encode(hmr_gpu_enc *enc, const uint8_t *y, const uint8_t *u, const uint8_t *v, int image_type, uint8_t *stream, long cap, long *stream_bytes,
		       uint8_t *recon);
int hmr_gpu_enc_load_source(hmr_gpu_enc *enc, int slot, const uint8_t *y, const uint8_t *u, const uint8_t *v);
int hmr_gpu_enc_encode_source(hmr_gpu_enc *enc, int slot, int image_type, uint8_t *stream, long cap, long *stream_bytes, uint8_t *recon);
int hmr_gpu_enc_encode_batch(hmr_gpu_enc **encs, int n, const int *slots, const int *image_types, uint8_t **streams, const long *caps, long *stream_bytes);
int hmr_gpu_enc_encode_batch_pipelined(hmr_gpu_enc **encs, int n, const int *slots, const int *image_types, uint8_t **streams, const long *caps, long *stream_bytes);
int hmr_gpu_enc_last_stats(hmr_gpu_enc *enc, int *passes, int *ctu_encodes, float *ctu_ms, float *frame_ms);
int hmr_gpu_enc_last_pool_kernel(hmr_gpu_enc *enc);
int hmr_gpu_enc_stale_predictions(hmr_gpu_enc *enc, long *last_picture, long *all_pictures);
int hmr_gpu_enc_profile(hmr_gpu_enc *enc, unsigned long long *out, int reset);
int hmr_gpu_enc_timeline(hmr_gpu_enc *enc, unsigned long long *out);

int hmr_gpu_enc_create_engine(hmr_gpu_ctx *ctx, const hmr_gpu_enc_cfg *cfg, int engine_index, hmr_gpu_enc **out);
int hmr_gpu_enc_state_bytes(void);
long hmr_gpu_enc_reference_elems(hmr_gpu_enc *enc, int comp);
int hmr_gpu_enc_export_reference(hmr_gpu_enc *enc, int16_t *dev_y, int16_t *dev_u, int16_t *dev_v, void *state);
int hmr_gpu_enc_import_reference(hmr_gpu_enc *enc, const int16_t *dev_y, const int16_t *dev_u, const int16_t *dev_v, const void *state);
long hmr_gpu_enc_reference_bytes(hmr_gpu_enc *enc);
int hmr_gpu_enc_create_engine_twin(hmr_gpu_ctx *ctx, hmr_gpu_enc *of, hmr_gpu_enc **out);
int hmr_gpu_enc_encode_chain(hmr_gpu_enc **encs, int n, hmr_gpu_enc *prev, const int *slots, const int *image_types, uint8_t **streams, const long *caps, long *stream_bytes);
int hmr_gpu_enc_export_references8(hmr_gpu_enc **encs, int n, uint8_t *dev_rows, long pitch, void *states);
int hmr_gpu_enc_import_references8(hmr_gpu_enc **encs, int n, const uint8_t *dev_rows, long pitch, const void *states);

enum { HMR_GPU_PIC_I420 = 0, HMR_GPU_PIC_NV12 = 1 };
typedef struct hmr_gpu_picture {
	int32_t format, reserved;
	const uint8_t *plane[3];
	int64_t pitch[3];
} hmr_gpu_picture;
int hmr_gpu_picture_check(const hmr_gpu_picture *pic, int width, int height);
int hmr_gpu_enc_load_source_device(hmr_gpu_enc *enc, int slot, const hmr_gpu_picture *pic, void *producer_stream);
int hmr_gpu_enc_load_sources_device(hmr_gpu_enc **encs, int n, const int *slots, const hmr_gpu_picture *pics, void *producer_stream);

int hmr_gpu_enc_export_pictures_device(hmr_gpu_enc **encs, int n, const hmr_gpu_picture *pics, const int *slots, uint64_t *dev_ssd, void *consumer_stream);
int hmr_gpu_enc_export_picture_device(hmr_gpu_enc *enc, const hmr_gpu_picture *pic, int slot, uint64_t *dev_ssd, void *consumer_stream);
int hmr_gpu_psnr(const uint64_t ssd[3], int width, int height, double psnr[3]);

enum { HMR_GPU_RGB_PACKED8 = 0, HMR_GPU_RGB_PLANAR8 = 1, HMR_GPU_RGB_PLANAR_F16 = 2, HMR_GPU_RGB_PLANAR_F32 = 3 };
enum { HMR_GPU_MATRIX_BT601 = 0, HMR_GPU_MATRIX_BT709 = 1 };
typedef struct hmr_gpu_rgb_picture {
	int32_t format, matrix, full_range, reserved;
	int32_t pixel_bytes;
	int32_t offset[3];
	const void *plane[3];
	int64_t pitch[3];
} hmr_gpu_rgb_picture;
int hmr_gpu_rgb_picture_check(const hmr_gpu_rgb_picture *pic, int width, int height);
int hmr_gpu_rgb_convert_host(const hmr_gpu_rgb_picture *pic, int width, int height, uint8_t *y, uint8_t *u, uint8_t *v);
int hmr_gpu_enc_load_source_rgb_device(hmr_gpu_enc *enc, int slot, const hmr_gpu_rgb_picture *pic, void *producer_stream);
int hmr_gpu_enc_load_sources_rgb_device(hmr_gpu_enc **encs, int n, const int *slots, const hmr_gpu_rgb_picture *pics, void *producer_stream);
int hmr_gpu_enc_export_source_device(hmr_gpu_enc *enc, int slot, const hmr_gpu_picture *out, void *consumer_stream);
int hmr_gpu_enc_export_sources_device(hmr_gpu_enc **encs, int n, const int *slots, const hmr_gpu_picture *outs, void *consumer_stream);

typedef struct hmr_gpu_scaled_picture {
	hmr_gpu_picture pic;
	int32_t width, height;
} hmr_gpu_scaled_picture;
int hmr_gpu_scale_check(int src_w, int src_h, int dst_w, int dst_h);
int hmr_gpu_enc_load_sources_scaled_device(hmr_gpu_enc **encs, int n, const int *slots, const hmr_gpu_scaled_picture *pics, void *producer_stream);
int hmr_gpu_enc_load_source_scaled_device(hmr_gpu_enc *enc, int slot, const hmr_gpu_scaled_picture *pic, void *producer_stream);
int hmr_gpu_scale_host(const hmr_gpu_scaled_picture *pic, int dst_w, int dst_h, uint8_t *y, uint8_t *u, uint8_t *v);

int hmr_gpu_enc_ssim_device(hmr_gpu_enc **encs, int n, const int *slots, int64_t *dev_ssim, void *consumer_stream);
int hmr_gpu_enc_ssim_one_device(hmr_gpu_enc *enc, int slot, int64_t *dev_ssim, void *consumer_stream);
int hmr_gpu_ssim(const int64_t sums[3], int width, int height, double ssim[3]);
int hmr_gpu_ssim_host(const hmr_gpu_picture *a, const hmr_gpu_picture *b, int width, int height, int64_t sums[3]);

int hmr_gpu_enc_export_pictures_rgb_device(hmr_gpu_enc **encs, int n, const int *which, const hmr_gpu_rgb_picture *outs, const hmr_gpu_rgb_picture *refs, uint64_t *dev_ssd,
					   void *consumer_stream);
int hmr_gpu_enc_export_picture_rgb_device(hmr_gpu_enc *enc, int which, const hmr_gpu_rgb_picture *out, const hmr_gpu_rgb_picture *ref, uint64_t *dev_ssd, void *consumer_stream);
int hmr_gpu_rgb_from_yuv_host(const uint8_t *y, const uint8_t *u, const uint8_t *v, int width, int height, const hmr_gpu_rgb_picture *out);
int hmr_gpu_rgb_ssd_host(const hmr_gpu_rgb_picture *a, const hmr_gpu_rgb_picture *b, int width, int height, uint64_t ssd[3]);
int hmr_gpu_psnr_rgb(const uint64_t ssd[3], int width, int height, double psnr[4]);

typedef struct hmr_gpu_scaled_rgb_picture {
	hmr_gpu_rgb_picture pic;
	int32_t width, height;
} hmr_gpu_scaled_rgb_picture;
int hmr_gpu_enc_load_sources_scaled_rgb_device(hmr_gpu_enc **encs, int n, const int *slots, const hmr_gpu_scaled_rgb_picture *pics, void *producer_stream);
int hmr_gpu_enc_load_source_scaled_rgb_device(hmr_gpu_enc *enc, int slot, const hmr_gpu_scaled_rgb_picture *pic, void *producer_stream);
int hmr_gpu_scale_rgb_host(const hmr_gpu_scaled_rgb_picture *pic, int dst_w, int dst_h, uint8_t *y, uint8_t *u, uint8_t *v);

int hmr_gpu_subpel_planes(hmr_gpu_ctx *ctx, const int16_t *pic_y, const int16_t *pic_u, const int16_t *pic_v, int stride_y, int rows_y, int stride_c, int rows_c,
			  uint8_t *out_y, uint8_t *out_u, uint8_t *out_v);

int hmr_gpu_probe_valu_issue(hmr_gpu_ctx *ctx, int waves_per_simd, int dependent, double *wave_instr_per_s, double *ms);
int hmr_gpu_probe_issue(hmr_gpu_ctx *ctx, int op, int waves_per_simd, int dependent, double *wave_instr_per_s, double *ms);

void hmr_gpu_prim_bytes(int on);
uint32_t hmr_gpu_prim_sad(int16_t *src, uint32_t src_stride, int16_t *pred, uint32_t pred_stride, int size);
uint32_t hmr_gpu_prim_ssd16b(int16_t *src, uint32_t src_stride, int16_t *pred, uint32_t pred_stride, int size);
void hmr_gpu_prim_predict(int16_t *orig, int orig_stride, int16_t *pred, int pred_stride, int16_t *residual, int residual_stride, int size);
void hmr_gpu_prim_reconst(int16_t *pred, int pred_stride, int16_t *residual, int residual_stride, int16_t *decoded, int decoded_stride, int size);
uint32_t hmr_gpu_prim_modified_variance(int16_t *p, int size, int stride, int modif);
void hmr_gpu_prim_intra_planar(int16_t *prediction, int pred_stride, int16_t *adi_pred_buff, int adi_size, int cu_size);
void hmr_gpu_prim_intra_angular(int16_t *prediction, int pred_stride, int16_t *adi_pred_buff, int adi_size, int cu_size, int cu_mode, int is_luma);
void hmr_gpu_prim_fill_reference_samples(int16_t *decoded_corner, int stride, int n, int left, int top, int bottom_left, int top_right, int bl_size, int tr_size, int16_t *adi);
void hmr_gpu_prim_adi_filter(int16_t *adi, int16_t *out, int adi_size, int n, int strong_enabled);
void hmr_gpu_prim_transform(int16_t *block, int16_t *coeff, int block_stride, int n, int is_dst);
void hmr_gpu_prim_itransform(int16_t *block, int16_t *coeff, int block_stride, int n, int is_dst);
void hmr_gpu_prim_quant(int16_t *src, int16_t *dst, int16_t *delta_u, int scan_mode, int depth, int comp, int is_intra, int slice_is_intra, int sign_hiding, int *ac_sum,
			int cu_size, int per, int rem);
void hmr_gpu_prim_inv_quant(int16_t *src, int16_t *dst, int depth, int comp, int is_intra, int cu_size, int per, int rem);
int hmr_gpu_prim_multi_sad(int maxc, const uint8_t *src, const uint8_t *plane, size_t plane_bytes, const int64_t *cand_off, int ncalls, int stride, int n, uint32_t *out);

enum hmr_gpu_walk_step { HMR_GPU_WALK_QUAD8_Y = 1, HMR_GPU_WALK_QUAD8_C, HMR_GPU_WALK_QUAD16_Y, HMR_GPU_WALK_QUAD16_C, HMR_GPU_WALK_TU, HMR_GPU_WALK_TU_PAIR };
typedef struct hmr_gpu_walk_case {
	int32_t step, node, comp, one_slot;
	int32_t qp, ctu_x, ctu_y, slice_type;
	int32_t sign_hiding, chroma_qp_offset, stride_y, stride_c;
	int32_t mv[4][2];
	double avg_dist, chroma_weight;
	int64_t sub_y, sub_c[2], curr, pred;
} hmr_gpu_walk_case;
typedef struct hmr_gpu_walk_out {
	uint32_t dist[4][3];
	int32_t sum[4][3];
	uint32_t raw[4][3], cbf[4][3];
	uint32_t stray, reserved[15];
	uint8_t pred[4][256];
	int16_t rec[4][256], lv[4][256];
} hmr_gpu_walk_out;
int hmr_gpu_walk_forms(const hmr_gpu_walk_case *cases, int ncases, const uint8_t *arena, size_t arena_bytes, hmr_gpu_walk_out *out);

#ifdef __cplusplus
}
#endif
#endif
```

Measured before the change: 475.5 frames/s.

## Prioritize pool claims by remaining steps and add per-worker timeline instrumentation

```diff
diff --git a/homerhevc_amd/csrc/enc/enc_platform.h b/homerhevc_amd/csrc/enc/enc_platform.h
--- a/homerhevc_amd/csrc/enc/enc_platform.h
+++ b/homerhevc_amd/csrc/enc/enc_platform.h
@@ -71,6 +71,16 @@
 			v = o < v ? o : v;
 		}
 		return v;
+	}
+	__device__ __forceinline__ uint32_t max32(uint32_t v) const
+	{
+		auto up = [](uint32_t a, uint32_t b) { return a > b ? a : b; };
+		v = up(v, (uint32_t)__builtin_amdgcn_update_dpp(0, (int)v, 0x111, 0xf, 0xf, true));
+		v = up(v, (uint32_t)__builtin_amdgcn_update_dpp(0, (int)v, 0x112, 0xf, 0xf, true));
+		v = up(v, (uint32_t)__builtin_amdgcn_update_dpp(0, (int)v, 0x114, 0xf, 0xf, true));
+		v = up(v, (uint32_t)__builtin_amdgcn_update_dpp(0, (int)v, 0x118, 0xf, 0xf, true));
+		const int x = (int)v;
+		return up(up((uint32_t)__builtin_amdgcn_readlane(x, 15), (uint32_t)__builtin_amdgcn_readlane(x, 31)), up((uint32_t)__builtin_amdgcn_readlane(x, 47), (uint32_t)__builtin_amdgcn_readlane(x, 63)));
 	}
 };
 struct WaveGrpLat : WaveGrp {
diff --git a/homerhevc_amd/csrc/enc/enc_sched.h b/homerhevc_amd/csrc/enc/enc_sched.h
--- a/homerhevc_amd/csrc/enc/enc_sched.h
+++ b/homerhevc_amd/csrc/enc/enc_sched.h
@@ -121,4 +121,9 @@
 	*parts = tp * NPART;
 }
 
+HENC_INLINE uint32_t pool_claim_key(int steps_left, int pos) { return ((uint32_t)steps_left << 16) | (uint32_t)(0xffff - pos); }
+HENC_INLINE int pool_key_pos(uint32_t key) { return 0xffff - (int)(key & 0xffffu); }
+HENC_INLINE int pool_key_steps_left(uint32_t key) { return (int)(key >> 16); }
+HENC_INLINE int pool_pass_next(uint32_t pass_max, uint32_t best) { return pass_max > best ? pool_key_pos(pass_max) : -1; }
+
 }
diff --git a/homerhevc_amd/csrc/k_encode.hip b/homerhevc_amd/csrc/k_encode.hip
--- a/homerhevc_amd/csrc/k_encode.hip
+++ b/homerhevc_amd/csrc/k_encode.hip
@@ -46,6 +46,7 @@
 	int threads;
 	int dep, dep_full;
 	int after, raster;
+	int wctu, hctu, steps;
 	FrameCtx *next_frame;
 	double *fin;
 	RcFrame *rc_dyn;
@@ -441,6 +442,11 @@
 constexpr int POOL_MAX_STEPS = HENC_MAX_STEPS;
 constexpr int POOL_STRIDE = 1 + 2 * POOL_MAX_STEPS;
 constexpr int BATCH_MAX = 512;
+enum { POOL_T_FIRST_CLAIM = 1, POOL_T_STEPS_CLOSED = 2, POOL_T_FINISHED = 3 };
+enum { POOL_W_ENTERED = 0, POOL_W_LEFT = 1, POOL_W_BUSY = 2, POOL_W_POST = 3, POOL_W_WORDS = 4 };
+constexpr int POOL_TIME_WORKERS = 2048;
+constexpr int POOL_FLAG_INTS = 4, POOL_STATE_INTS = BATCH_MAX * POOL_STRIDE + POOL_FLAG_INTS + 2 * POOL_W_WORDS * POOL_TIME_WORKERS;
+static_assert((BATCH_MAX * POOL_STRIDE + POOL_FLAG_INTS) % 2 == 0, "the workers' records are 64-bit words");
 
 __device__ __forceinline__ void pool_step_rows(int t, int W, int H, int *r_lo, int *r_hi)
 {
@@ -450,7 +456,7 @@
 }
 
 template <class G>
-__device__ void pool_encode_ctu(const EncDev &d, Enc &__restrict__ e, const G g, Seq *lseq, FrameCtx *lframe, FastTables *lft, int t, int row, int *cached_rem, const int *abort_flag)
+__device__ unsigned long long pool_encode_ctu(const EncDev &d, Enc &__restrict__ e, const G g, Seq *lseq, FrameCtx *lframe, FastTables *lft, int t, int row, int *cached_rem, const int *abort_flag)
 {
 	HENC_ENC_IN_LDS(e);
 	const Seq &S = *lseq;
@@ -546,19 +552,24 @@
 		atomicAdd(&d.counters[1], 1);
 	}
 	g.sync();
+	const unsigned long long t_decided = wall_clock64();
 	__builtin_amdgcn_fence(__ATOMIC_RELEASE, "agent");
 	if (g.tid == 0) post_st_fenced(&d.post.rows[row].dec, c + 1);
+	return t_decided;
 }
 
 __device__ __attribute__((noinline)) int pool_post_drain_run(const EncDev &d, const WaveGrp g, const Seq *lseq, const FrameCtx *lframe, Work *lw, WorkSlow *my_slow, int *finished);
-__device__ __forceinline__ int pool_post_drain(const EncDev &d, const WaveGrp g, const Seq *lseq, const FrameCtx *lframe, Work *lw, WorkSlow *my_slow, int *finished)
-{
-	if (post_finished(*lseq, d.post)) return 0;
+__device__ __forceinline__ bool pool_post_look(const EncDev &d, const WaveGrp g, const Seq *lseq, const FrameCtx *lframe)
+{
+	if (post_finished(*lseq, d.post)) return false;
 	PostCtx x;
 	x.seq = lseq; x.f = lframe; x.T = d.tables; x.geo.p = nullptr; x.ctus = d.ctus; x.coeff = d.coeff; x.pic = &d.post;
 	int r, c, k;
-	if (!post_scan(g, x, r, c, k)) return 0;
-	return pool_post_drain_run(d, g, lseq, lframe, lw, my_slow, finished);
+	return post_scan(g, x, r, c, k);
+}
+__device__ __forceinline__ int pool_post_drain(const EncDev &d, const WaveGrp g, const Seq *lseq, const FrameCtx *lframe, Work *lw, WorkSlow *my_slow, int *finished)
+{
+	return pool_post_look(d, g, lseq, lframe) ? pool_post_drain_run(d, g, lseq, lframe, lw, my_slow, finished) : 0;
 }
 __device__ __attribute__((noinline)) int pool_post_drain_run(const EncDev &d, const WaveGrp g, const Seq *lseq, const FrameCtx *lframe, Work *lw, WorkSlow *my_slow, int *finished)
 {
@@ -585,6 +596,7 @@
 				const double total = (double)g.sum64(part);
 				if (g.tid == 0) {
 					d.fin[0] = total;
+					((unsigned long long *)d.fin)[POOL_T_FINISHED] = wall_clock64();
 					if (d.next_frame) {
 						double a = total;
 						a /= lseq->nctu * NPART;
@@ -603,11 +615,101 @@
 	return ran;
 }
 
+__device__ __forceinline__ int pool_step_open(const EncDev &d, const int *st, int *ct)
+{
+	const int W = d.wctu, H = d.hctu, steps = d.steps, raster = d.raster;
+	const int c = __hip_atomic_load(&st[0], __ATOMIC_RELAXED, __HIP_MEMORY_SCOPE_AGENT);
+	const int t1 = __hip_atomic_load(&st[1], __ATOMIC_RELAXED, __HIP_MEMORY_SCOPE_AGENT);
+	*ct = c;
+	if (c >= steps) return 0;
+	bool open;
+	if (raster) open = t1 == c;
+	else {
+		int r_lo, r_hi;
+		pool_step_rows(c, W, H, &r_lo, &r_hi);
+		open = (c == 0 ? t1 : __hip_atomic_load(&st[1 + c], __ATOMIC_RELAXED, __HIP_MEMORY_SCOPE_AGENT)) < r_hi - r_lo + 1;
+	}
+	return open ? steps - c : 0;
+}
+template <class G>
+__device__ __forceinline__ bool pool_step_ready(const G g, const EncDev *devs, int q0, int t0)
+{
+	const EncDev &d0 = devs[q0];
+	bool ready = !d0.post.rc_need || rc_ready(g, d0.post, d0.seq->hctu, t0);
+	if (ready && d0.dep >= 0) {
+		const EncDev &dd = devs[d0.dep];
+		const int H0 = dd.seq->hctu, W0 = dd.seq->wctu;
+		for (int base2 = 0; base2 < H0 && ready; base2 += 64) {
+			const int r2 = base2 + g.tid;
+			bool miss = false;
+			if (r2 < H0) {
+				int need = t0 - 2 * r2 + 8;
+				need = need < 0 ? 0 : (need > W0 ? W0 : need);
+				if (d0.dep_full) need = W0;
+				miss = post_ld(&dd.post.rows[r2].s_done) < need;
+			}
+			if (g.any(miss)) ready = false;
+		}
+	}
+	if (ready && d0.after >= 0) ready = post_ld(&devs[d0.after].post.errors[1]) == 1;
+	return ready;
+}
+template <class G>
+__device__ __forceinline__ int pool_claim(const G g, const EncDev &dd, int *st, int tt)
+{
+	int kk = 0;
+	if (dd.raster) {
+		if (g.tid == 0) kk = atomicCAS(&st[1], tt, tt + 1) == tt ? 0 : -1;
+		return __builtin_amdgcn_readfirstlane(kk);
+	}
+	if (g.tid == 0) kk = atomicAdd(&st[1 + tt], 1);
+	kk = __builtin_amdgcn_readfirstlane(kk);
+	int r_lo, r_hi;
+	pool_step_rows(tt, dd.seq->wctu, dd.seq->hctu, &r_lo, &r_hi);
+	return kk < r_hi - r_lo + 1 ? kk : -1;
+}
+
+__device__ __attribute__((noinline)) int pool_idle_pick(const EncDev *devs, const int *state, int nseq, int start, const WaveGrp g)
+{
+	uint32_t keys[BATCH_MAX / 64];
+#pragma unroll
+	for (int p = 0; p < BATCH_MAX / 64; p++) {
+		const int i = p * 64 + g.tid;
+		keys[p] = 0;
+		if (i < nseq) {
+			const int cand = (start + i) % nseq;
+			const EncDev &dd = devs[cand];
+			const int steps = dd.steps;
+			const int ct = __hip_atomic_load(&state[(size_t)cand * POOL_STRIDE], __ATOMIC_RELAXED, __HIP_MEMORY_SCOPE_AGENT);
+			keys[p] = pool_claim_key((ct < steps ? steps - ct : 0) + 1, i);
+		}
+	}
+	for (;;) {
+		uint32_t mine = 0;
+#pragma unroll
+		for (int p = 0; p < BATCH_MAX / 64; p++) mine = keys[p] > mine ? keys[p] : mine;
+		const uint32_t m = g.max32(mine);
+		const int pos = pool_pass_next(m, 0);
+		if (pos < 0) return -1;
+		const int cand = (start + pos) % nseq;
+		const EncDev &dd = devs[cand];
+		if (pool_post_look(dd, g, dd.seq, dd.frame)) return cand;
+#pragma unroll
+		for (int p = 0; p < BATCH_MAX / 64; p++)
+			if (p == pos >> 6 && g.tid == (pos & 63)) keys[p] = 0;
+	}
+}
+
 template <class G>
 __device__ __forceinline__ void encode_pool_body(const EncDev *devs, int nseq, int *state, int *finished, WorkSlow *slow, unsigned long long watchdog_ticks, unsigned lds_bytes)
 {
 	unsigned long long t_start = wall_clock64();
 	constexpr bool LAT = G::bg;
+#if defined(HENC_POOL_CLAIM_RR)
+	constexpr bool FIRST_OPEN = true;
+#else
+	constexpr bool FIRST_OPEN = LAT;
+#endif
 	if (!rows_enter<LAT, typename std::conditional<LAT, WaveGrp, G>::type>(lds_bytes)) return;
 	extern __shared__ __align__(16) uint8_t lds[];
 	G g{(int)(threadIdx.x & 63)};
@@ -643,84 +745,81 @@
 	e.timeline = nullptr;
 	int cached_rem[2] = {-1, -1}, cached_q = -1, idle_rounds = 0;
 	int start = (int)(blockIdx.x % (unsigned)nseq);
+	unsigned long long *const my_times = blockIdx.x < (unsigned)POOL_TIME_WORKERS ? (unsigned long long *)(finished + POOL_FLAG_INTS) + (size_t)blockIdx.x * POOL_W_WORDS : nullptr;
+	unsigned long long busy = 0, busy_post = 0;
+	if (g.tid == 0 && my_times) my_times[POOL_W_ENTERED] = t_start;
 	for (;;) {
 		int q = -1, t = 0, k = 0;
-		bool all_finished = true;
-		for (int base = 0; base < nseq && q < 0; base += 64) {
-			const int i = base + g.tid, cand = i < nseq ? (start + i) % nseq : -1;
-			int ct = -1;
-			bool open = false;
-			if (cand >= 0) {
-				const int *st = state + (size_t)cand * POOL_STRIDE;
-				const EncDev &dd = devs[cand];
-				const int W = dd.seq->wctu, H = dd.seq->hctu, steps = dd.raster ? W * H : W + 2 * (H - 1);
-				ct = __hip_atomic_load(&st[0], __ATOMIC_RELAXED, __HIP_MEMORY_SCOPE_AGENT);
-				if (ct < steps) {
-					all_finished = false;
-					if (dd.raster) open = __hip_atomic_load(&st[1], __ATOMIC_RELAXED, __HIP_MEMORY_SCOPE_AGENT) == ct;
-					else {
-						int r_lo, r_hi;
-						pool_step_rows(ct, W, H, &r_lo, &r_hi);
-						open = __hip_atomic_load(&st[1 + ct], __ATOMIC_RELAXED, __HIP_MEMORY_SCOPE_AGENT) < r_hi - r_lo + 1;
-					}
-				}
-			}
-			if (g.any(!all_finished)) all_finished = false;
-			uint64_t m = g.ballot(open);
-			while (m) {
-				const int lane0 = __builtin_ctzll(m);
-				const int q0 = __builtin_amdgcn_readlane(cand, lane0), t0 = __builtin_amdgcn_readlane(ct, lane0);
-				const EncDev &d0 = devs[q0];
-				bool ready = !d0.post.rc_need || rc_ready(g, d0.post, d0.seq->hctu, t0);
-				if (ready && d0.dep >= 0) {
-					const EncDev &dd = devs[d0.dep];
-					const int H0 = dd.seq->hctu, W0 = dd.seq->wctu;
-					for (int base2 = 0; base2 < H0 && ready; base2 += 64) {
-						const int r2 = base2 + g.tid;
-						bool miss = false;
-						if (r2 < H0) {
-							int need = t0 - 2 * r2 + 8;
-							need = need < 0 ? 0 : (need > W0 ? W0 : need);
-							if (d0.dep_full) need = W0;
-							miss = post_ld(&dd.post.rows[r2].s_done) < need;
-						}
-						if (g.any(miss)) ready = false;
-					}
-				}
-				if (ready && d0.after >= 0) ready = post_ld(&devs[d0.after].post.errors[1]) == 1;
-				if (ready) break;
-				m &= m - 1;
-			}
-			if (m) {
-				const int lane = __builtin_ctzll(m);
-				const int qq = __builtin_amdgcn_readlane(cand, lane), tt = __builtin_amdgcn_readlane(ct, lane);
-				int kk = 0;
-				const EncDev &dd = devs[qq];
-				if (dd.raster) {
-					if (g.tid == 0) kk = atomicCAS(&state[(size_t)qq * POOL_STRIDE + 1], tt, tt + 1) == tt ? 0 : 1;
-					kk = __builtin_amdgcn_readfirstlane(kk);
-					if (kk == 0) { q = qq; t = tt; k = 0; }
+		if constexpr (FIRST_OPEN) {
+			for (int base = 0; base < nseq && q < 0; base += 64) {
+				const int i = base + g.tid, cand = i < nseq ? (start + i) % nseq : -1;
+				int ct = -1;
+				const bool open = cand >= 0 && pool_step_open(devs[cand], state + (size_t)cand * POOL_STRIDE, &ct) > 0;
+				uint64_t m = g.ballot(open);
+				while (m) {
+					const int lane0 = __builtin_ctzll(m);
+					if (pool_step_ready(g, devs, __builtin_amdgcn_readlane(cand, lane0), __builtin_amdgcn_readlane(ct, lane0))) break;
+					m &= m - 1;
+				}
+				if (m) {
+					const int lane = __builtin_ctzll(m);
+					const int qq = __builtin_amdgcn_readlane(cand, lane), tt = __builtin_amdgcn_readlane(ct, lane);
+					const int kk = pool_claim(g, devs[qq], state + (size_t)qq * POOL_STRIDE, tt);
+					if (kk >= 0) { q = qq; t = tt; k = kk; }
 					else base -= 64;
+				}
+			}
+		} else {
+			uint32_t best = 0;
+			int best_q = -1, best_t = 0;
+			for (int base = 0; base < nseq; base += 64) {
+				const int i = base + g.tid, cand = i < nseq ? (start + i) % nseq : -1;
+				int ct = -1;
+				uint32_t key = 0;
+				if (cand >= 0) {
+					const int left = pool_step_open(devs[cand], state + (size_t)cand * POOL_STRIDE, &ct);
+					if (left > 0) key = pool_claim_key(left, i);
+				}
+				for (;;) {
+					const uint32_t m = g.max32(key);
+					const int pos = pool_pass_next(m, best);
+					if (pos < 0) break;
+					const int lane0 = pos - base;
+					const int q0 = __builtin_amdgcn_readlane(cand, lane0), t0 = __builtin_amdgcn_readlane(ct, lane0);
+					if (pool_step_ready(g, devs, q0, t0)) { best = m; best_q = q0; best_t = t0; break; }
+					if (g.tid == lane0) key = 0;
+				}
+			}
+			if (best_q >= 0) {
+				const int kk = pool_claim(g, devs[best_q], state + (size_t)best_q * POOL_STRIDE, best_t);
+				if (kk < 0) {
+					if (__hip_atomic_load(finished + 1, __ATOMIC_RELAXED, __HIP_MEMORY_SCOPE_AGENT)) break;
+					if (wall_clock64() - t_start > watchdog_ticks) { if (g.tid == 0) __hip_atomic_store(finished + 1, 1, __ATOMIC_RELAXED, __HIP_MEMORY_SCOPE_AGENT); break; }
 					continue;
 				}
-				if (g.tid == 0) kk = atomicAdd(&state[(size_t)qq * POOL_STRIDE + 1 + tt], 1);
-				kk = __builtin_amdgcn_readfirstlane(kk);
-				int r_lo, r_hi;
-				pool_step_rows(tt, dd.seq->wctu, dd.seq->hctu, &r_lo, &r_hi);
-				if (kk < r_hi - r_lo + 1) { q = qq; t = tt; k = kk; }
-				else base -= 64;
+				q = best_q; t = best_t; k = kk;
 			}
 		}
 		if (q < 0) {
 			if (__hip_atomic_load(finished, __ATOMIC_RELAXED, __HIP_MEMORY_SCOPE_AGENT) >= nseq) break;
 			if (__hip_atomic_load(finished + 1, __ATOMIC_RELAXED, __HIP_MEMORY_SCOPE_AGENT)) break;
-			if (wall_clock64() - t_start > watchdog_ticks) { if (g.tid == 0) __hip_atomic_store(finished + 1, 1, __ATOMIC_RELAXED, __HIP_MEMORY_SCOPE_AGENT); break; }
+			const unsigned long long t_idle = wall_clock64();
+			if (t_idle - t_start > watchdog_ticks) { if (g.tid == 0) __hip_atomic_store(finished + 1, 1, __ATOMIC_RELAXED, __HIP_MEMORY_SCOPE_AGENT); break; }
 			int ran = 0;
-			for (int i = 0; i < nseq; i++) {
-				const int cand = (start + i) % nseq;
-				const EncDev &dd = devs[cand];
-				ran += pool_post_drain(dd, g, dd.seq, dd.frame, lw, slow + blockIdx.x, finished);
-				if (ran) { start = cand; break; }
+			if constexpr (FIRST_OPEN) {
+				for (int i = 0; i < nseq; i++) {
+					const int cand = (start + i) % nseq;
+					const EncDev &dd = devs[cand];
+					ran += pool_post_drain(dd, g, dd.seq, dd.frame, lw, slow + blockIdx.x, finished);
+					if (ran) { start = cand; break; }
+				}
+			} else {
+				const int found = pool_idle_pick(devs, state, nseq, start, g);
+				if (found >= 0) {
+					const EncDev &dd = devs[found];
+					ran = pool_post_drain_run(dd, g, dd.seq, dd.frame, lw, slow + blockIdx.x, finished);
+					start = found;
+				}
 			}
 			if (!ran) {
 				idle_rounds = idle_rounds < 16 ? idle_rounds + 1 : 16;
@@ -728,11 +827,14 @@
 			} else {
 				idle_rounds = 0;
 				t_start = wall_clock64();
+				busy_post += t_start - t_idle;
 			}
 			continue;
 		}
+		const unsigned long long t_claim = wall_clock64();
 		__builtin_amdgcn_fence(__ATOMIC_ACQUIRE, "agent");
 		const EncDev &d = devs[q];
+		if (g.tid == 0 && t == 0) ((unsigned long long *)d.fin)[POOL_T_FIRST_CLAIM] = t_claim;
 		if (q != cached_q) {
 			for (int i = g.tid; i < (int)(sizeof(Seq) / 4); i += 64) ((uint32_t *)lseq)[i] = ((const uint32_t *)d.seq)[i];
 			for (int i = g.tid; i < (int)(sizeof(FrameCtx) / 4); i += 64) ((uint32_t *)lframe)[i] = ((const uint32_t *)d.frame)[i];
@@ -750,19 +852,26 @@
 		if (d.raster) row = t / W;
 		else if (hvalid) row = k == 0 ? hrow : (r_lo + k - 1 < hrow ? r_lo + k - 1 : r_lo + k);
 		else row = r_lo + k;
-		pool_encode_ctu(d, e, g, lseq, lframe, lft, t, row, cached_rem, finished + 1);
+		const unsigned long long t_decided = pool_encode_ctu(d, e, g, lseq, lframe, lft, t, row, cached_rem, finished + 1);
 		if (g.tid == 0) {
 			int *st = state + (size_t)q * POOL_STRIDE;
 			const int dn = d.raster ? 1 : atomicAdd(&st[1 + POOL_MAX_STEPS + t], 1) + 1;
 			if (dn == (d.raster ? 1 : r_hi - r_lo + 1)) {
 				__builtin_amdgcn_fence(__ATOMIC_ACQUIRE, "agent");
 				__hip_atomic_store(&st[0], t + 1, __ATOMIC_RELEASE, __HIP_MEMORY_SCOPE_AGENT);
+				if (t + 1 == (d.raster ? W * H : W + 2 * (H - 1))) ((unsigned long long *)d.fin)[POOL_T_STEPS_CLOSED] = t_decided;
 			}
 		}
 		pool_post_drain(d, g, lseq, lframe, lw, slow + blockIdx.x, finished);
 		idle_rounds = 0;
 		t_start = wall_clock64();
+		busy += t_start - t_claim;
 		start = (q + 1) % nseq;
+	}
+	if (g.tid == 0 && my_times) {
+		my_times[POOL_W_LEFT] = wall_clock64();
+		my_times[POOL_W_BUSY] = busy;
+		my_times[POOL_W_POST] = busy_post;
 	}
 	int hseq[NHELP];
 	for (int h = 0; h < NHELP; h++) hseq[h] = e.hseq[h];
diff --git a/homerhevc_amd/csrc/k_encode_batch.inc b/homerhevc_amd/csrc/k_encode_batch.inc
--- a/homerhevc_amd/csrc/k_encode_batch.inc
+++ b/homerhevc_amd/csrc/k_encode_batch.inc
@@ -131,7 +131,7 @@
 	HIP_TRY(hipEventRecord(lead->ev_batch0, bst));
 	if ((rc = launch_pool(lead, lead->h_devs, n, rows_total, needs_rd, bst))) return rc;
 	(void)hipEventRecord(lead->ev_batch1, bst);
-	hipLaunchKernelGGL(k_gather_results, dim3(n), dim3(256), 0, bst, (const EncDev *)lead->d_batch, lead->d_gather, pitch, (const int *)(lead->d_pool_state + BATCH_MAX * POOL_STRIDE));
+	hipLaunchKernelGGL(k_gather_results, dim3(n), dim3(256), 0, bst, (const EncDev *)lead->d_batch, lead->d_gather, pitch, (const int *)(lead->d_pool_state + BATCH_MAX * POOL_STRIDE), pool_times_of(lead));
 	HIP_TRY(hipGetLastError());
 	HIP_TRY(hipMemcpyAsync(lead->h_gather, lead->d_gather, (size_t)pitch * n * 4, hipMemcpyDeviceToHost, bst));
 	*pitch_out = pitch;
@@ -151,6 +151,7 @@
 	bt.t[2] = std::chrono::steady_clock::now();
 	float ms = 0;
 	HIP_TRY(hipEventElapsedTime(&ms, lead->ev_batch0, lead->ev_batch1));
+	pool_timeline_collect(lead, lead->h_gather, n, pitch);
 	if (!lead->h_offs) HIP_TRY(hipHostMalloc((void **)&lead->h_offs, BATCH_MAX * sizeof(size_t), hipHostMallocDefault));
 	lead->pend_off.resize(n);
 	lead->pend_rows.assign(n, std::vector<uint32_t>());
@@ -420,7 +421,7 @@
 	HIP_TRY(hipEventRecord(lead->ev_batch0, bst));
 	if ((rc = launch_pool(lead, lead->h_devs, n, rows_total, needs_rd, bst))) return rc;
 	(void)hipEventRecord(lead->ev_batch1, bst);
-	hipLaunchKernelGGL(k_gather_results, dim3(n), dim3(256), 0, bst, (const EncDev *)lead->d_batch, lead->d_gather, pitch, (const int *)(lead->d_pool_state + BATCH_MAX * POOL_STRIDE));
+	hipLaunchKernelGGL(k_gather_results, dim3(n), dim3(256), 0, bst, (const EncDev *)lead->d_batch, lead->d_gather, pitch, (const int *)(lead->d_pool_state + BATCH_MAX * POOL_STRIDE), pool_times_of(lead));
 	HIP_TRY(hipGetLastError());
 	HIP_TRY(hipMemcpyAsync(lead->h_gather, lead->d_gather, (size_t)pitch * n * 4, hipMemcpyDeviceToHost, bst));
 	{
@@ -429,6 +430,7 @@
 	}
 	float ms = 0;
 	HIP_TRY(hipEventElapsedTime(&ms, lead->ev_batch0, lead->ev_batch1));
+	pool_timeline_collect(lead, lead->h_gather, n, pitch);
 	HostState seq_state = start_state;
 	bool cut_before = false;
 	for (int j = 0; j < n; j++) {
diff --git a/homerhevc_amd/csrc/k_encode_object.inc b/homerhevc_amd/csrc/k_encode_object.inc
--- a/homerhevc_amd/csrc/k_encode_object.inc
+++ b/homerhevc_amd/csrc/k_encode_object.inc
@@ -132,6 +132,9 @@
 	WorkSlow *d_pool_slow = nullptr;
 	int pool_workers = 0;
 	int last_pool_kernel = -1;
+	int last_pool_workers = 0;
+	std::vector<unsigned long long> pool_timeline;
+	unsigned long long pool_busy = 0, pool_post = 0, pool_ticks = 0;
 	JobRing<IngestJob> ingest;
 	JobRing<RgbIngestJob> ingest_rgb;
 	JobRing<ScaleJob> scale;
@@ -318,7 +321,7 @@
 				hmr_set_error("k_encode_pool: picture %d of the launch is RD_FULL, and this kernel's walk is compiled without full RDO (needs_rd was not set)", i);
 				return HMR_GPU_ERR_ARG;
 			}
-	if (!lead->d_pool_state) HIP_TRY(hipMalloc((void **)&lead->d_pool_state, sizeof(int) * (BATCH_MAX * POOL_STRIDE + 4)));
+	if (!lead->d_pool_state) HIP_TRY(hipMalloc((void **)&lead->d_pool_state, sizeof(int) * POOL_STATE_INTS));
 	if (lead->pool_workers < workers) {
 		if (lead->d_pool_slow) (void)hipFree(lead->d_pool_slow);
 		lead->d_pool_slow = nullptr;
@@ -327,7 +330,7 @@
 		HIP_TRY(hipMemsetAsync(lead->d_pool_slow, 0, sizeof(WorkSlow) * workers, st));
 		lead->pool_workers = workers;
 	}
-	HIP_TRY(hipMemsetAsync(lead->d_pool_state, 0, sizeof(int) * (BATCH_MAX * POOL_STRIDE + 4), st));
+	HIP_TRY(hipMemsetAsync(lead->d_pool_state, 0, sizeof(int) * POOL_STATE_INTS, st));
 	double watchdog_s = getenv("HENC_WATCHDOG_S") ? atof(getenv("HENC_WATCHDOG_S")) : 120.0;
 	if (!(watchdog_s > 0)) watchdog_s = 120.0;
 	const unsigned long long watchdog = (unsigned long long)(watchdog_s * 1e8);
@@ -617,7 +620,7 @@
 		DEV_ALLOC(e->d_bs, (size_t)e->row_cap * s.hctu);
 		DEV_ALLOC(e->d_cumbits, s.nctu);
 		DEV_ALLOC(e->d_sao_tab, 2 * 52 * 2);
-		DEV_ALLOC(e->d_post_err, 4 + 2 * 16 + 4);
+		DEV_ALLOC(e->d_post_err, 4 + 2 * 16 + 8);
 		double tab[2][104];
 		sao_lambda_table(s, SLICE_P, tab[0]);
 		sao_lambda_table(s, SLICE_I, tab[1]);
@@ -671,6 +674,7 @@
 	}
 	e->cur = 0;
 	e->d.raster = e->raster;
+	e->d.wctu = s.wctu; e->d.hctu = s.hctu; e->d.steps = e->raster ? s.nctu : s.wctu + 2 * (s.hctu - 1);
 	e->d.threads = e->cfg.wfpp_num_threads > 1 ? e->cfg.wfpp_num_threads : 1;
 	e->last_ms = e->last_total_ms = 0;
 	e->last_passes = e->last_encodes = 0;
@@ -883,6 +887,23 @@
 
 extern "C" int hmr_gpu_enc_last_pool_kernel(hmr_gpu_enc *e) { return e ? e->last_pool_kernel : -1; }
 
+extern "C" int hmr_gpu_enc_last_pool_timeline(hmr_gpu_enc *e, int max_pictures, unsigned long long *first_claim, unsigned long long *steps_closed, unsigned long long *finished, int *workers,
+					      unsigned long long *busy_ticks, unsigned long long *post_ticks, unsigned long long *kernel_ticks)
+{
+	if (!e || max_pictures < 0) return HMR_GPU_ERR_ARG;
+	const int n = (int)(e->pool_timeline.size() / 3);
+	for (int i = 0; i < n && i < max_pictures; i++) {
+		if (first_claim) first_claim[i] = e->pool_timeline[(size_t)3 * i];
+		if (steps_closed) steps_closed[i] = e->pool_timeline[(size_t)3 * i + 1];
+		if (finished) finished[i] = e->pool_timeline[(size_t)3 * i + 2];
+	}
+	if (workers) *workers = e->last_pool_workers;
+	if (busy_ticks) *busy_ticks = e->pool_busy;
+	if (post_ticks) *post_ticks = e->pool_post;
+	if (kernel_ticks) *kernel_ticks = e->pool_ticks;
+	return n;
+}
+
 extern "C" int hmr_gpu_enc_timeline(hmr_gpu_enc *e, unsigned long long *out)
 {
 	if (!e || !out) return HMR_GPU_ERR_ARG;
@@ -990,9 +1011,10 @@
 }
 
 namespace {
-constexpr int GATHER_HEAD = 12;
+constexpr int GATHER_HEAD = 28;
+constexpr int GATHER_TIMES = 12;
 constexpr int CHAIN_MAX_FRAMES = 32;
-__global__ void k_gather_results(const EncDev *devs, uint32_t *out, int pitch, const int *pool_flags)
+__global__ void k_gather_results(const EncDev *devs, uint32_t *out, int pitch, const int *pool_flags, const unsigned long long *pool_times)
 {
 	const EncDev &d = devs[blockIdx.x];
 	uint32_t *o = out + (size_t)blockIdx.x * pitch;
@@ -1019,7 +1041,52 @@
 		memcpy(&o[10], &avg, 8);
 	}
 	for (int c = threadIdx.x; c < nctu; c += blockDim.x) o[GATHER_HEAD + c] = d.ctus[c].distortion;
+	if (threadIdx.x < 3) memcpy(&o[GATHER_TIMES + 2 * threadIdx.x], (const unsigned long long *)d.fin + 1 + threadIdx.x, 8);
+	if (blockIdx.x == 0 && pool_times) {
+		__shared__ unsigned long long s_w[4];
+		__shared__ uint32_t s_n;
+		if (threadIdx.x == 0) { s_w[0] = ~0ull; s_w[1] = 0; s_w[2] = 0; s_w[3] = 0; s_n = 0; }
+		__syncthreads();
+		unsigned long long first = ~0ull, last = 0, busy = 0, post = 0;
+		uint32_t nw = 0;
+		for (int w = threadIdx.x; w < POOL_TIME_WORKERS; w += blockDim.x) {
+			const unsigned long long *t = pool_times + (size_t)w * POOL_W_WORDS;
+			if (!t[POOL_W_ENTERED]) continue;
+			first = t[POOL_W_ENTERED] < first ? t[POOL_W_ENTERED] : first;
+			last = t[POOL_W_LEFT] > last ? t[POOL_W_LEFT] : last;
+			busy += t[POOL_W_BUSY];
+			post += t[POOL_W_POST];
+			nw++;
+		}
+		atomicAdd(&s_n, nw);
+		atomicMin(&s_w[0], first);
+		atomicMax(&s_w[1], last);
+		atomicAdd(&s_w[2], busy);
+		atomicAdd(&s_w[3], post);
+		__syncthreads();
+		if (threadIdx.x < 4) memcpy(&o[GATHER_TIMES + 6 + 2 * threadIdx.x], &s_w[threadIdx.x], 8);
+		if (threadIdx.x == 4) o[GATHER_TIMES + 14] = s_n;
+	}
 	for (int r = threadIdx.x; r < d.seq->hctu; r += blockDim.x) o[pitch - POST_MAX_ROWS + r] = (uint32_t)d.post.ent[r].bytecnt;
+}
+void pool_timeline_collect(hmr_gpu_enc *lead, const uint32_t *g, int n, int pitch)
+{
+	unsigned long long w[4];
+	memcpy(w, g + GATHER_TIMES + 6, sizeof w);
+	lead->pool_timeline.assign((size_t)3 * n, 0);
+	for (int i = 0; i < n; i++) {
+		unsigned long long t[3];
+		memcpy(t, g + (size_t)i * pitch + GATHER_TIMES, sizeof t);
+		for (int k = 0; k < 3; k++) lead->pool_timeline[(size_t)3 * i + k] = t[k] > w[0] ? t[k] - w[0] : 0;
+	}
+	lead->pool_ticks = w[1] > w[0] ? w[1] - w[0] : 0;
+	lead->pool_busy = w[2];
+	lead->pool_post = w[3];
+	lead->last_pool_workers = (int)g[GATHER_TIMES + 14];
+}
+const unsigned long long *pool_times_of(const hmr_gpu_enc *lead)
+{
+	return lead->d_pool_state ? (const unsigned long long *)(lead->d_pool_state + BATCH_MAX * POOL_STRIDE + POOL_FLAG_INTS) : nullptr;
 }
 
 }
@@ -1061,7 +1128,7 @@
 			HIP_TRY(hipHostMalloc((void **)&e->h_gather, (size_t)pitch * 4, hipHostMallocDefault));
 			e->gather_words = (size_t)pitch;
 		}
-		hipLaunchKernelGGL(k_gather_results, dim3(1), dim3(256), 0, st, (const EncDev *)e->d_batch, e->d_gather, pitch, (const int *)nullptr);
+		hipLaunchKernelGGL(k_gather_results, dim3(1), dim3(256), 0, st, (const EncDev *)e->d_batch, e->d_gather, pitch, (const int *)nullptr, pool_times_of(e));
 		HIP_TRY(hipGetLastError());
 		HIP_TRY(hipMemcpyAsync(e->h_gather, e->d_gather, (size_t)pitch * 4, hipMemcpyDeviceToHost, st));
 	} else if ((rc = download_public(e))) return rc;
@@ -1098,6 +1165,7 @@
 	}
 	HIP_TRY(hipStreamSynchronize(st));
 	const uint32_t *gr = e->h_gather;
+	if (e->lockstep) pool_timeline_collect(e, gr, 1, pitch);
 	e->note_stale_predictions(e->lockstep ? gr[3] >> 8 : (uint32_t)err[3]);
 	const double acc = e->lockstep ? frame_acc_dist(s, e->cfg.wfpp_num_threads, [&](int n) { return gr[GATHER_HEAD + n]; })
 				       : frame_acc_dist(s, e->cfg.wfpp_num_threads, [&](int n) { return ((const CtuPublic *)(e->h_public.data() + sizeof(CtuPublic) * n))->distortion; });
diff --git a/include/homer_gpu.h b/include/homer_gpu.h
--- a/include/homer_gpu.h
+++ b/include/homer_gpu.h
@@ -376,6 +376,9 @@
 int hmr_gpu_enc_encode_batch_pipelined(hmr_gpu_enc **encs, int n, const int *slots, const int *image_types, uint8_t **streams, const long *caps, long *stream_bytes);
 int hmr_gpu_enc_last_stats(hmr_gpu_enc *enc, int *passes, int *ctu_encodes, float *ctu_ms, float *frame_ms);
 int hmr_gpu_enc_last_pool_kernel(hmr_gpu_enc *enc);
+
+int hmr_gpu_enc_last_pool_timeline(hmr_gpu_enc *enc, int max_pictures, unsigned long long *first_claim, unsigned long long *steps_closed, unsigned long long *finished, int *workers,
+				   unsigned long long *busy_ticks, unsigned long long *post_ticks, unsigned long long *kernel_ticks);
 int hmr_gpu_enc_stale_predictions(hmr_gpu_enc *enc, long *last_picture, long *all_pictures);
 int hmr_gpu_enc_profile(hmr_gpu_enc *enc, unsigned long long *out, int reset);
 int hmr_gpu_enc_timeline(hmr_gpu_enc *enc, unsigned long long *out);
```

After: 486.5 frames/s (median of 6 runs). 2.3% higher.
